# zgchen33/MCGaze

Hardware: AMD Instinct MI355X
Metric: clips/sec (7x3x224x224) (higher is better)
Workload: dtype f16x3; 1 GPU; full multiclue_gaze_r50 forward (R-50 + FPN + 4 decoder stages + gaze head), 64 clips/GPU x 7 frames x 3x224x224, 64 clips/step; clips_per_gpu=64, clip_length=7, global_clips=64, chunk_frames=0, parallelism=single GPU, trunk_streams=2

## Files before the change

include/mcgaze_hip.h:

```cpp
#ifndef MCGAZE_HIP_H
#define MCGAZE_HIP_H

#include <stddef.h>
#include <stdint.h>

#ifdef __cplusplus
extern "C" {
#endif

#define MCG_ABI_VERSION 19

enum { MCG_OK = 0, MCG_ERR_ARG = 1, MCG_ERR_HIP = 2, MCG_ERR_UNSUPPORTED = 3, MCG_ERR_WORKSPACE = 4 };
typedef enum { MCG_F32 = 0, MCG_BF16 = 1, MCG_F16X3 = 2, MCG_F16 = 3 } mcg_dtype;
#define MCG_ELEM_BYTES(dt) (((dt) == MCG_BF16 || (dt) == MCG_F16) ? 2 : 4)
typedef void* mcg_stream;

int mcg_abi_version(void);
const char* mcg_build_id(void);
const char* mcg_last_error(void);
int mcg_device_info(int* cu_count, size_t* hbm_bytes, char* arch, int arch_len);

int mcg_nchw_to_nhwc(mcg_stream s, mcg_dtype dt, const float* src, void* dst, int N, int C, int H, int W);
int mcg_nhwc_to_nchw(mcg_stream s, mcg_dtype dt, const void* src, float* dst, int N, int C, int H, int W);

enum { MCG_RES_NONE = 0, MCG_RES_ADD = 1, MCG_RES_UPSAMPLE_ADD = 2 };
enum {
  MCG_FLAG_STAGED_GEMM = 1,
  MCG_FLAG_NO_SPECIALISED = 2,
  MCG_FLAG_NO_ATTN_BLOCK = 4
};
typedef struct {
  const void* x;
  const void* w;
  const float* bias;
  const void* residual;
  void* y;
  int N, H, W, Cin, Cout, KH, KW, stride, pad;
  int relu;
  int residual_mode;
  int Hr, Wr;
  const void* x2;
  int Cin2, stride2, H2, W2;
  int tile;
  int flags;
  float wscale;
} mcg_conv_desc;
int mcg_conv2d(mcg_stream s, mcg_dtype dt, const mcg_conv_desc* d);

int mcg_bottleneck_x3(mcg_stream s, const float* x, const float* src2, const void* wstream, const float* bias, float* y, float* z,
                      int frames, int H, int W, int cm, int nsrc, int cn, void* trace);

size_t mcg_conv3x3_wino_x3_weight_bytes(int Cin, int Cout, int g);
int mcg_conv3x3_wino_x3(mcg_stream s, const float* x, const void* u, const float* bias, float* y, int frames, int H, int W,
                        int Cin, int Cout, int relu, int tile, float wscale, int g);

int mcg_pointwise_stream(mcg_stream s, mcg_dtype dt, const void* a, const void* wf, const float* bias, const void* res, void* y,
                         int M, int K, int N, int relu, int res_mode, int Ho, int Wo, int Hr, int Wr, float wscale,
                         const int* block_list, const int* block_count, int grid_cap);
int mcg_pointwise_dyn(mcg_stream s, mcg_dtype dt, const void* a, const void* wf, const float* bias, void* y, int M, float wscale, int grid_cap);
int mcg_pointwise_pair(mcg_stream s, mcg_dtype dt, const void* a1, const void* a2, const void* res, const void* w3f, const float* b3,
                       void* y, const void* w1f, const float* b1, void* z, int M, int K2, int C2, int grid_cap);

size_t mcg_stem_workspace_bytes(mcg_dtype dt, int N, int H, int W);
int mcg_stem_forward(mcg_stream s, mcg_dtype dt, const float* img, const void* w_stem, const float* bias,
                     void* y, int N, int H, int W, void* ws, size_t ws_bytes, int flags);

int mcg_roi_align(mcg_stream s, mcg_dtype dt, const void* const feats[4], const int feat_h[4], const int feat_w[4],
                  const int strides[4], int C, const float* boxes, int num_boxes, int boxes_per_frame,
                  void* out, int32_t* levels_out);
int mcg_roi_align_indexed(mcg_stream s, mcg_dtype dt, const void* const feats[4], const int feat_h[4], const int feat_w[4],
                          const int strides[4], int C, const float* boxes, int num_boxes, int boxes_per_frame,
                          const int32_t* frame_of, int pyramid_frames, void* out, int32_t* levels_out);

enum {
  MCG_SW_IN_PROJ_W = 0, MCG_SW_IN_PROJ_B, MCG_SW_OUT_PROJ_W, MCG_SW_OUT_PROJ_B, MCG_SW_ATTN_LN_G, MCG_SW_ATTN_LN_B,
  MCG_SW_DYN_W,
  MCG_SW_DYN_B,
  MCG_SW_NORM_IN_G, MCG_SW_NORM_IN_B, MCG_SW_NORM_OUT_G, MCG_SW_NORM_OUT_B,
  MCG_SW_FC_W, MCG_SW_FC_B, MCG_SW_FC_LN_G, MCG_SW_FC_LN_B, MCG_SW_IIC_LN_G, MCG_SW_IIC_LN_B,
  MCG_SW_FFN1_W, MCG_SW_FFN1_B, MCG_SW_FFN2_W, MCG_SW_FFN2_B, MCG_SW_FFN_LN_G, MCG_SW_FFN_LN_B,
  MCG_SW_CLS_FC_W, MCG_SW_CLS_LN_G, MCG_SW_CLS_LN_B,
  MCG_SW_REG_FC_W,
  MCG_SW_REG_LN_G,
  MCG_SW_REG_LN_B,
  MCG_SW_HEAD_CLS_W,
  MCG_SW_HEAD_CLS_B,
  MCG_SW_HEAD_REG_W,
  MCG_SW_HEAD_REG_B,
  MCG_SW_OUT_PROJ_WF, MCG_SW_CLS_FC_WF,
  MCG_SW_REG_FC_WF,
  MCG_SW_IN_PROJ_WF,
  MCG_SW_DYN_WF,
  MCG_SW_COUNT
};
enum {
  MCG_GW_FC_W = 0,
  MCG_GW_LN_G,
  MCG_GW_LN_B,
  MCG_GW_OUT_W,
  MCG_GW_OUT_B,
  MCG_GW_FUSE_W,
  MCG_GW_FUSE_B,
  MCG_GW_COUNT
};

size_t mcg_stage_workspace_bytes(mcg_dtype dt, int num_frames);
int mcg_stage_forward(mcg_stream s, mcg_dtype dt, const void* const weights[MCG_SW_COUNT], const void* roi_feat,
                      const void* obj_in, const float* boxes_in, int num_frames, int clip_length,
                      void* obj_out, float* boxes_out, float* cls_out, const float bbox_stds[4],
                      void* ws, size_t ws_bytes, int flags);
int mcg_stage_forward_ragged(mcg_stream s, mcg_dtype dt, const void* const weights[MCG_SW_COUNT], const void* roi_feat,
                             const void* obj_in, const float* boxes_in, int num_frames, const int* clip_start, int num_clips,
                             int max_clip_length, void* obj_out, float* boxes_out, float* cls_out, const float bbox_stds[4],
                             void* ws, size_t ws_bytes, int flags);

size_t mcg_gaze_head_workspace_bytes(mcg_dtype dt, int num_frames);
int mcg_gaze_head(mcg_stream s, mcg_dtype dt, const void* const weights[MCG_GW_COUNT], const void* obj,
                  int num_frames, float* gaze_out, void* ws, size_t ws_bytes);

typedef struct {
  const void* w;
  const float* bias;
  int cin, cout, k, stride, pad;
  const void* wf;
  float wscale;
  const void* wf4;
} mcg_conv_weights;

typedef struct {
  const void* wstream;
  const float* bias;
  int conv2_index;
  int cm, c, cn;
  int nsrc;
} mcg_fused_block;

typedef struct {
  int blocks[4];
  mcg_conv_weights stem;
  const mcg_conv_weights* convs;
  int num_convs;
  mcg_conv_weights lateral[4];
  mcg_conv_weights fpn_out[4];
  mcg_conv_weights c3_ds[4];
  const float* init_boxes;
  const void* init_feats;
  int num_stages;
  const void* const* stage_weights;
  const void* const* gaze_weights;
  float bbox_stds[4];
  const mcg_fused_block* fused;
  int num_fused;
} mcg_model_weights;

typedef struct mcg_engine mcg_engine;
int mcg_engine_create(mcg_engine** out, const mcg_model_weights* w, mcg_dtype dt);
void mcg_engine_destroy(mcg_engine* e);
int mcg_engine_set_option(mcg_engine* e, const char* name, int value);
int mcg_engine_range_audit(mcg_engine* e, unsigned long long* counts, const char** names, int capacity, int* n_out);
size_t mcg_engine_workspace_bytes(const mcg_engine* e, int num_frames, int H, int W, int chunk_frames);
int mcg_backbone_fpn_forward(mcg_engine* e, mcg_stream s, const float* img, int num_frames, int H, int W,
                             int chunk_frames, void* const pyramid[4], void* ws, size_t ws_bytes);
size_t mcg_trunk_workspace_bytes(const mcg_engine* e, int num_frames, int H, int W, int chunk_frames);
size_t mcg_decoder_workspace_bytes(const mcg_engine* e, int num_frames);
int mcg_decoder_forward(mcg_engine* e, mcg_stream s, const void* const pyramid[4], int num_frames, int clip_length, int H, int W,
                        const int* img_hw, float* gaze_out, float* boxes_out, float* scores_out, void* ws, size_t ws_bytes);
int mcg_decoder_forward_indexed(mcg_engine* e, mcg_stream s, const void* const pyramid[4], int pyramid_frames, const int32_t* frame_of,
                                int num_frames, int clip_length, int H, int W, const int* img_hw, float* gaze_out, float* boxes_out,
                                float* scores_out, void* ws, size_t ws_bytes);
int mcg_decoder_forward_ragged(mcg_engine* e, mcg_stream s, const void* const pyramid[4], int pyramid_frames, const int32_t* frame_of,
                               int num_frames, const int* clip_start, int num_clips, int max_clip_length, int H, int W, const int* img_hw,
                               float* gaze_out, float* boxes_out, float* scores_out, void* ws, size_t ws_bytes);
size_t mcg_deferred_pyramid_bytes(const mcg_engine* e, int num_frames, int H, int W);
int mcg_deferred_pyramid_levels(const mcg_engine* e, void* slot, int num_frames, int H, int W, void* levels[4], int* deferred);
int mcg_deferred_pyramid_state(const mcg_engine* e, void* slot, int num_frames, int H, int W, void** inner, int** flags, int** counts,
                               int** lists, int* blocks, int* lateral_deferred);
int mcg_inner_block_neighbours(int id, int H, int W, int out[9]);
int mcg_backbone_fpn_forward_deferred(mcg_engine* e, mcg_stream s, const float* img, int num_frames, int H, int W, int chunk_frames,
                                      void* slot, size_t slot_bytes, void* ws, size_t ws_bytes);
int mcg_decoder_forward_deferred(mcg_engine* e, mcg_stream s, void* slot, size_t slot_bytes, int num_frames, int clip_length, int H, int W,
                                 const int* img_hw, float* gaze_out, float* boxes_out, float* scores_out, void* ws, size_t ws_bytes);
int mcg_decoder_forward_deferred_ragged(mcg_engine* e, mcg_stream s, void* slot, size_t slot_bytes, int num_frames, const int* clip_start,
                                        int num_clips, int max_clip_length, int H, int W, const int* img_hw, float* gaze_out,
                                        float* boxes_out, float* scores_out, void* ws, size_t ws_bytes);
int mcg_clip_forward(mcg_engine* e, mcg_stream s, const float* img, int num_frames, int clip_length, int H, int W,
                     const int* img_hw, int chunk_frames, float* gaze_out, float* boxes_out, float* scores_out,
                     void* ws, size_t ws_bytes);
int mcg_clip_forward_ragged(mcg_engine* e, mcg_stream s, const float* img, int num_frames, const int* clip_start, int num_clips,
                            int max_clip_length, int H, int W, const int* img_hw, int chunk_frames, float* gaze_out, float* boxes_out,
                            float* scores_out, void* ws, size_t ws_bytes);
int mcg_pyramid_scatter_rows(mcg_stream s, mcg_dtype dt, const void* const src[4], void* const dst[4],
                             int num_frames, int store_rows, int H, int W, const int32_t* row_of);
int mcg_merge_windows(mcg_stream s, const float* gaze, const float* boxes, const float* scores, int num_frames, const float* scale,
                      int scale_per_frame, const int32_t* plan, int num_dst, int max_src, float* store, int store_rows,
                      float person_threshold);
int mcg_smooth_gaze(mcg_stream s, const float* store, int store_rows, const int32_t* plan, int num_out, double alpha, float* out);

typedef struct mcg_frame_desc {
  const void* src;
  int src_h, src_w, src_pitch;
  int crop_y, crop_x, crop_h, crop_w;
  int out_h, out_w;
} mcg_frame_desc;
int mcg_preprocess_frames(mcg_stream stream, const mcg_frame_desc* frames_dev, int num_frames, float* dst, int pad_h, int pad_w,
                          const float mean[3], const float stdinv[3], int to_rgb);
typedef struct mcg_image_desc {
  const void* src;
  int h, w, pitch;
} mcg_image_desc;
int mcg_preprocess_head_crops(mcg_stream s, const mcg_image_desc* images_dev, int num_images, const float* boxes_dev,
                              const int32_t* image_of_dev, int n, double expand, int scale_w, int scale_h, mcg_frame_desc* desc_out_dev,
                              int32_t* img_hw_dev, float* scale_factor_dev, int32_t* flags_dev, float* dst, int pad_h, int pad_w,
                              const float mean[3], const float stdinv[3], int to_rgb);
typedef struct mcg_yuv_coef {
  int y_off, cy, cub, cug, cvg, cvr;
} mcg_yuv_coef;
typedef struct mcg_nv12_image_desc {
  const void* y;
  const void* uv;
  int h, w, pitch_y, pitch_uv;
} mcg_nv12_image_desc;
typedef struct mcg_nv12_frame_desc {
  const void* src;
  int src_h, src_w, src_pitch;
  int crop_y, crop_x, crop_h, crop_w;
  int out_h, out_w;
  const void* uv;
  int uv_pitch;
} mcg_nv12_frame_desc;
int mcg_preprocess_frames_nv12(mcg_stream stream, const mcg_nv12_frame_desc* frames_dev, int num_frames, float* dst, int pad_h, int pad_w,
                               const float mean[3], const float stdinv[3], int to_rgb, const mcg_yuv_coef* coef);
int mcg_preprocess_head_crops_nv12(mcg_stream s, const mcg_nv12_image_desc* images_dev, int num_images, const float* boxes_dev,
                                   const int32_t* image_of_dev, int n, double expand, int scale_w, int scale_h,
                                   mcg_nv12_frame_desc* desc_out_dev, int32_t* img_hw_dev, float* scale_factor_dev, int32_t* flags_dev,
                                   float* dst, int pad_h, int pad_w, const float mean[3], const float stdinv[3], int to_rgb,
                                   const mcg_yuv_coef* coef);

typedef struct mcg_arrow_desc {
  int seg[3][2][2];
  int thickness;
  int x0, y0, x1, y1;
  int image, flag;
  int reserved;
} mcg_arrow_desc;
int mcg_draw_gaze_arrows(mcg_stream s, const mcg_image_desc* images_dev, int num_images, int max_h, int max_w, const float* boxes_dev,
                         const float* gaze_dev, int gaze_stride, const int32_t* image_of_dev, int n, double length, int min_thickness,
                         double thickness_ratio, double tip_length, const unsigned char* color, const unsigned char* colors_dev,
                         mcg_arrow_desc* plan_out_dev, int32_t* flags_dev);
int mcg_draw_gaze_arrows_nv12(mcg_stream s, const mcg_nv12_image_desc* images_dev, int num_images, int max_h, int max_w, const float* boxes_dev,
                              const float* gaze_dev, int gaze_stride, const int32_t* image_of_dev, int n, double length, int min_thickness,
                              double thickness_ratio, double tip_length, const unsigned char* yuv, const unsigned char* yuvs_dev,
                              mcg_arrow_desc* plan_out_dev, int32_t* flags_dev);

size_t mcg_detect_heads_workspace_bytes(int num_images, int num_anchors);
int mcg_detect_heads(mcg_stream s, const float* pred_dev, int num_images, int num_anchors, int num_classes, long long image_stride, int row_stride,
                     int in_h, int in_w, const int32_t* frame_hw_dev , double conf_thres, double iou_thres,
                     int only_class , int agnostic, int max_nms, int max_det,
                     float* boxes_dev , float* scores_dev , int32_t* classes_dev ,
                     int32_t* image_of_dev , int32_t* counts_dev , int32_t* flags_dev ,
                     void* ws_dev, size_t ws_bytes);

enum { MCG_LETTERBOX_U8 = 0, MCG_LETTERBOX_F16 = 1, MCG_LETTERBOX_F32 = 2 };
typedef struct mcg_letterbox_desc {
  mcg_frame_desc frame;
  int top, left;
} mcg_letterbox_desc;
typedef struct mcg_nv12_letterbox_desc {
  mcg_nv12_frame_desc frame;
  int top, left;
} mcg_nv12_letterbox_desc;
int mcg_letterbox_frames(mcg_stream stream, const mcg_letterbox_desc* frames_dev, int num_frames, void* dst, int out_h, int out_w, int out_type,
                         int swap_rb);
int mcg_letterbox_frames_nv12(mcg_stream stream, const mcg_nv12_letterbox_desc* frames_dev, int num_frames, void* dst, int out_h, int out_w,
                              int out_type, int swap_rb, const mcg_yuv_coef* coef);

typedef struct mcg_track_header {
  int32_t next_id;
  int32_t frames_seen;
  int32_t reserved[2];
} mcg_track_header;
typedef struct mcg_track_slot {
  float box[4];
  int32_t id;
  int32_t age;
  int32_t reserved[2];
} mcg_track_slot;
size_t mcg_track_state_bytes(int num_sequences, int slots);
int mcg_track_heads(mcg_stream s, const float* boxes_dev, long long frame_stride, const int32_t* counts_dev, int num_sequences, int num_frames,
                    int max_det, int slots, double match_iou, int max_age, void* state_dev,
                    float* slot_boxes_dev , int32_t* image_of_dev , int32_t* track_id_dev ,
                    int32_t* age_dev , int32_t* det_of_dev , int32_t* flags_dev );

int mcg_track_heads_motion(mcg_stream s, const float* boxes_dev, long long frame_stride, const int32_t* counts_dev, int num_sequences,
                           int num_frames, int max_det, int slots, double match_iou, int max_age, double velocity_gain, double coast_decay,
                           void* state_dev, float* slot_boxes_dev , int32_t* image_of_dev ,
                           int32_t* track_id_dev , int32_t* age_dev , int32_t* det_of_dev ,
                           int32_t* flags_dev , float* state_boxes_dev );

int mcg_live_slots(mcg_stream s, const void* state_dev, int num_cameras, int slots, int tick, int ring_depth, float* crop_boxes_dev,
                   int32_t* image_of_dev, int32_t* ring_id_dev, float* ring_box_dev, int32_t* matched_dev);
int mcg_live_gate(mcg_stream s, const int32_t* ring_id_dev, const float* ring_box_dev, int ring_depth, int num_cameras, int slots, int tick,
                  const int32_t* table_dev, int num_entries, int first_out, int num_out, const float* fused_dev, const float* others_dev,
                  float* fused_smooth_dev, float* others_smooth_dev, int32_t* track_id_dev, int32_t* valid_dev, float* head_box_dev,
                  int32_t* image_of_dev, int32_t* smooth_valid_dev);

int mcg_live_lanes(mcg_stream s, const void* state_dev, int num_cameras, int slots, int lanes, int tick, int ring_depth,
                   int32_t* lane_state_dev, float* crop_boxes_dev, int32_t* image_of_dev, int32_t* ring_id_dev, float* ring_box_dev,
                   int32_t* ring_col_dev, int32_t* lane_of_dev, int32_t* matched_dev, int32_t* overflow_dev);
int mcg_live_gate_lanes(mcg_stream s, const int32_t* ring_id_dev, const float* ring_box_dev, const int32_t* ring_col_dev, int ring_depth,
                        int num_cameras, int slots, int lanes, int tick, const int32_t* table_dev, int num_entries, int first_out, int num_out,
                        const float* fused_dev, const float* others_dev, float* fused_smooth_dev, float* others_smooth_dev,
                        int32_t* track_id_dev, int32_t* valid_dev, int32_t* camera_dev, int32_t* slot_dev, float* head_box_dev,
                        int32_t* image_of_dev, int32_t* smooth_valid_dev);

int mcg_gaze_targets(mcg_stream s, const float* boxes_dev, const float* gaze_dev, int gaze_stride, const int32_t* image_of_dev, int n,
                     const float* regions_dev, const int32_t* region_image_dev, int m, int region_period, double expand, double camera_cos2,
                     int32_t* kind_dev, int32_t* target_dev, float* t_dev, float* hit_dev, int32_t* mutual_dev, int32_t* flags_dev);

int mcg_gaze_dwell(mcg_stream s, const int32_t* person_dev, const int32_t* tag_dev, const int32_t* kind_dev, const int32_t* ident_dev,
                   const int32_t* mutual_dev, int num_frames, int columns, int frame0, int enter, int exit_frames, int32_t* state_dev,
                   int32_t* region_frames_dev, int num_regions, int32_t* dwell_dev, int32_t* ended_dev, int32_t* events_dev, int max_events,
                   int32_t* num_events_dev);

#define MCG_ATTEND_POLY_VERTS 32
int mcg_gaze_targets_poly(mcg_stream s, const float* boxes_dev, const float* gaze_dev, int gaze_stride, const int32_t* image_of_dev, int n,
                          const float* region_xy_dev, int num_vertices, const int32_t* region_start_dev, const int32_t* region_image_dev, int m,
                          int region_period, double expand, double camera_cos2, int32_t* kind_dev, int32_t* target_dev, float* t_dev,
                          float* hit_dev, int32_t* mutual_dev, int32_t* flags_dev);

typedef struct mcg_stroke_desc {
  int seg[3][2][2];
  int thickness;
  int x0, y0, x1, y1;
  int image, flag;
  int layer, count;
  unsigned color, color_active;
  int reserved;
} mcg_stroke_desc;
int mcg_draw_attention(mcg_stream s, const mcg_image_desc* images_dev, int num_images, int max_h, int max_w, const float* boxes_dev,
                       const float* gaze_dev, int gaze_stride, const int32_t* image_of_dev, int n, const int32_t* kind_dev, const int32_t* target_dev,
                       const float* hit_dev, const int32_t* mutual_dev, const float* region_xy_dev, int num_vertices,
                       const int32_t* region_start_dev, const int32_t* region_image_dev, int m, int region_period, const unsigned char* palette,
                       double length, int min_thickness, double thickness_ratio, double tip_length, int line_thickness, int region_thickness,
                       void* workspace_dev, size_t workspace_bytes, int32_t* flags_dev, int32_t* region_flags_dev, int32_t* region_active_dev);
int mcg_draw_attention_nv12(mcg_stream s, const mcg_nv12_image_desc* images_dev, int num_images, int max_h, int max_w, const float* boxes_dev,
                            const float* gaze_dev, int gaze_stride, const int32_t* image_of_dev, int n, const int32_t* kind_dev,
                            const int32_t* target_dev, const float* hit_dev, const int32_t* mutual_dev, const float* region_xy_dev, int num_vertices,
                            const int32_t* region_start_dev, const int32_t* region_image_dev, int m, int region_period, const unsigned char* palette,
                            double length, int min_thickness, double thickness_ratio, double tip_length, int line_thickness, int region_thickness,
                            void* workspace_dev, size_t workspace_bytes, int32_t* flags_dev, int32_t* region_flags_dev, int32_t* region_active_dev);

#define MCG_LABEL_CHARS 24
typedef struct mcg_label_desc {
  int x, y;
  int x0, y0, x1, y1;
  int image, flag;
  int len;
  unsigned color;
  unsigned char text[MCG_LABEL_CHARS];
} mcg_label_desc;
int mcg_format_labels(mcg_stream s, const int32_t* id_dev, const int32_t* value_dev, int n, int num, int den, unsigned char* text_out_dev);
int mcg_draw_labels(mcg_stream s, const mcg_image_desc* images_dev, int num_images, int max_h, int max_w, const float* boxes_dev,
                    const int32_t* image_of_dev, const unsigned char* text_dev, const int32_t* place_dev, int n, const unsigned char* font_dev,
                    int scale, int advance, int pad, const unsigned char* color, const unsigned char* colors_dev, const unsigned char* background,
                    mcg_label_desc* plan_out_dev, int32_t* flags_dev);
int mcg_draw_labels_nv12(mcg_stream s, const mcg_nv12_image_desc* images_dev, int num_images, int max_h, int max_w, const float* boxes_dev,
                         const int32_t* image_of_dev, const unsigned char* text_dev, const int32_t* place_dev, int n, const unsigned char* font_dev,
                         int scale, int advance, int pad, const unsigned char* yuv, const unsigned char* yuvs_dev, const unsigned char* background,
                         mcg_label_desc* plan_out_dev, int32_t* flags_dev);

int mcg_gaze_heat_add(mcg_stream s, const float* hit_dev, const int32_t* kind_dev, const int32_t* image_of_dev, const int32_t* flags_dev,
                      const int32_t* mask_dev, int n, int32_t* heat_dev, int32_t* peak_dev, int C, int GH, int GW, int cell_shift, int radius,
                      int kinds, int period, int decay_shift, void* workspace_dev, size_t workspace_bytes);
int mcg_draw_heat(mcg_stream s, const mcg_image_desc* images_dev, int num_images, int max_h, int max_w, const int32_t* heat_dev,
                  const int32_t* full_dev, int C, int GH, int GW, int cell_shift, int period, const unsigned char* lut_dev, int min_level);
int mcg_draw_heat_nv12(mcg_stream s, const mcg_nv12_image_desc* images_dev, int num_images, int max_h, int max_w, const int32_t* heat_dev,
                       const int32_t* full_dev, int C, int GH, int GW, int cell_shift, int period, const unsigned char* lut_dev, int min_level);

typedef struct mcg_anon_desc {
  int image, flag;
  int x0, y0, x1, y1;
  int cx2, cy2;
  int W, H;
  int shift, shape;
} mcg_anon_desc;
int mcg_anonymize_heads(mcg_stream s, const mcg_image_desc* images_dev, int num_images, int max_h, int max_w, const float* boxes_dev,
                        const int32_t* image_of_dev, int n, double expand, int shape, int cell_shift, int blocks, int mode,
                        const unsigned char* color, mcg_anon_desc* plan_out_dev, int32_t* flags_dev);
int mcg_anonymize_heads_nv12(mcg_stream s, const mcg_nv12_image_desc* images_dev, int num_images, int max_h, int max_w, const float* boxes_dev,
                             const int32_t* image_of_dev, int n, double expand, int shape, int cell_shift, int blocks, int mode,
                             const unsigned char* yuv, mcg_anon_desc* plan_out_dev, int32_t* flags_dev);

int mcg_engine_profile_start(mcg_engine* e, int capacity);
int mcg_engine_profile_stop(mcg_engine* e, int* count, float* ms, double* flops, double* algo_bytes, int* cfg, int* shape_mnk, int capacity);
int mcg_bench_backbone_forward(mcg_engine* e, mcg_stream s, const float* img, int num_frames, int H, int W, void* ws, size_t ws_bytes);
int mcg_bench_backbone_levels(const mcg_engine* e, void* ws, int num_frames, int H, int W, void* levels[4]);

#ifdef __cplusplus
}
#endif
#endif
```

mcgaze_amd/csrc/check_resources.py:

```python
#!/usr/bin/env python3
import re
import sys

RULES = {
    'wino_x3w_kernel': dict(scratch=0, vgpr_spill=0, unit='engine'),
    'wino_x3w_blocks_kernel': dict(scratch=0, vgpr_spill=0, unit='engine'),
    'gaze_targets_kernel': dict(scratch=0, vgpr_spill=0, unit='attend'),
    'gaze_targets_poly_kernel': dict(scratch=0, vgpr_spill=0, unit='attend'),
    'gaze_mutual_kernel': dict(scratch=0, vgpr_spill=0, unit='attend'),
    'gaze_dwell_kernel': dict(scratch=0, vgpr_spill=0, unit='dwell'),
    'gaze_dwell_events_kernel': dict(scratch=0, vgpr_spill=0, unit='dwell'),
    'label_raster_kernel': dict(scratch=0, vgpr_spill=0, unit='labels'),
    'heat_render_kernel': dict(scratch=0, vgpr_spill=0, unit='heat'),
    'anonymize_render_kernel': dict(scratch=0, vgpr_spill=0, unit='anonymize'),
}


def parse(path):
    kernels, cur = [], None
    for line in open(path, errors='replace'):
        m = re.search(r'remark: (?:\s*)Function Name: (\S+)', line)
        if m:
            cur = dict(name=m.group(1))
            kernels.append(cur)
            continue
        m = re.search(r'remark:\s+([A-Za-z \[\]/]+): (\S+) \[-Rpass-analysis', line)
        if m and cur is not None:
            cur[m.group(1).strip()] = m.group(2)
    return kernels


def main():
    path = sys.argv[1]
    kernels = parse(path)
    other = [l.rstrip() for l in open(path, errors='replace') if 'Rpass-analysis=kernel-resource-usage' not in l and not re.match(r'\s+\d* *\|', l) and l.strip()
             and not l.startswith('In file included from') and not re.match(r'\d+ (warning|remark)s? generated', l.strip())]
    for l in other:
        print(l, file=sys.stderr)
    bad = []
    import os
    unit = os.path.basename(path).split('.')[0]
    for prefix, lim in RULES.items():
        if lim.get('unit') == unit and not any(prefix in k['name'] and 'VGPRs Spill' in k and 'ScratchSize [bytes/lane]' in k for k in kernels):
            bad.append(f'{prefix}: no resource remarks found in {path} (expected -Rpass-analysis=kernel-resource-usage output for it)')
    for k in kernels:
        for prefix, lim in RULES.items():
            if prefix in k['name']:
                scratch = int(k.get('ScratchSize [bytes/lane]', '0'))
                spill = int(k.get('VGPRs Spill', '0'))
                if scratch > lim['scratch'] or spill > lim['vgpr_spill']:
                    bad.append(f"{k['name']}: scratch {scratch} B/lane, {spill} spilled VGPRs (limits {lim['scratch']}, {lim['vgpr_spill']})")
    if '--table' in sys.argv:
        print('| kernel | VGPRs | AGPRs | SGPRs | scratch B/lane | VGPR spill | waves/SIMD |\n|---|---|---|---|---|---|---|')
        for k in kernels:
            print(f"| `{k['name']}` | {k.get('VGPRs')} | {k.get('AGPRs')} | {k.get('TotalSGPRs')} | {k.get('ScratchSize [bytes/lane]')} | {k.get('VGPRs Spill')} | {k.get('Occupancy [waves/SIMD]')} |")
    if bad:
        print('check_resources: kernels that must not spill (RULES):\n  ' + '\n  '.join(bad), file=sys.stderr)
        return 1
    return 0


if __name__ == '__main__':
    sys.exit(main())
```

mcgaze_amd/csrc/engine.hip:

```cpp
#include "igemm.hpp"
#include "pw_pair.hpp"
#include "pw_single.hpp"
#include "bneck_x3.hpp"
#include "pw_single_x3.hpp"
#include "wino_x3.hpp"

#include <stdarg.h>
#include <stdlib.h>
#include <string.h>

#include <map>
#include <mutex>
#include <string>
#include <vector>

int launch_roi_align(hipStream_t s, mcg_dtype dt, const void* const feats[4], const int feat_h[4], const int feat_w[4],
                     const int strides[4], int C, const float* boxes, int num_boxes, int boxes_per_frame, const int32_t* frame_of,
                     int pyramid_frames, void* out, int32_t* levels_out);
int launch_init_queries(hipStream_t s, mcg_dtype dt, const float* init_boxes, const void* init_feats, const int* img_hw,
                        const int32_t* frame_of, int pyramid_frames, int H, int W, float* boxes, void* obj, int N);
bool roi_mark_supported(int H, int W);
int launch_defer_clear(hipStream_t s, int* p, int n);
int launch_roi_mark(hipStream_t s, const float* boxes, int num_boxes, int boxes_per_frame, int level, int H, int W, int stride, int* state,
                    int* list, int* count);
int launch_inner_mark(hipStream_t s, const int* out_list, const int* out_count, int H, int W, int nblk, int* state, int* list, int* count);

struct mcg_engine {
  mcg_dtype dt;
  int blocks[4];
  mcg_conv_weights stem;
  std::vector<mcg_conv_weights> convs;
  mcg_conv_weights lateral[4], fpn_out[4], c3_ds[4];
  std::vector<mcg_fused_block> fused;
  bool bneck_fused = true;
  bool bneck_blocked = true;
  int winograd = 1;
  int wino_tile = -1;
  int fpn_deferred = 1;
  int fpn_lateral_deferred = 1;
  static constexpr int kAuditCap = 256;
  unsigned long long* audit_dev = nullptr;
  std::vector<std::string> audit_names;
  const float* init_boxes;
  const void* init_feats;
  int num_stages;
  std::vector<const void*> stage_w;
  const void* gaze_w[MCG_GW_COUNT];
  float stds[4];
  static constexpr int kMaxSplit = 4, kCandidates = 8;
  struct StreamPool* pool = nullptr;
  hipStream_t* cand = nullptr;
  hipEvent_t ev_fork = nullptr, ev_join[kMaxSplit - 1] = {};
  McgCtx ctx;
  Prof prof;
  int trunk_streams = 2;
  int max_range_frames = 0;
  bool pw_single = true;
  bool pw_pair = true;
  std::mutex mu;
};
struct StreamPool {
  hipStream_t cand[mcg_engine::kCandidates] = {};
  hipEvent_t ev_probe[3] = {};
  std::map<hipStream_t, std::vector<int>> side_of;
  std::mutex mu;
  bool ok = false;
};
static StreamPool* stream_pool_for_current_device() {
  static std::mutex g_mu;
  static std::map<int, StreamPool*> g_pools;
  int dev = 0;
  if (hipGetDevice(&dev) != hipSuccess) return nullptr;
  std::lock_guard<std::mutex> lock(g_mu);
  auto it = g_pools.find(dev);
  if (it != g_pools.end()) return it->second;
  StreamPool* p = new StreamPool();
  bool ok = true;
  for (int i = 0; i < mcg_engine::kCandidates; ++i) ok = ok && hipStreamCreateWithFlags(&p->cand[i], hipStreamNonBlocking) == hipSuccess;
  for (int i = 0; i < 3; ++i) ok = ok && hipEventCreate(&p->ev_probe[i]) == hipSuccess;
  p->ok = ok;
  g_pools[dev] = p;
  return p;
}
__global__ void probe_spin_kernel(long long ticks) {
  const long long t0 = wall_clock64();
  while (wall_clock64() - t0 < ticks) {}
}
static const std::vector<int>& side_streams_for(mcg_engine* e, hipStream_t s) {
  StreamPool* p = e->pool;
  std::lock_guard<std::mutex> lock(p->mu);
  auto it = p->side_of.find(s);
  if (it != p->side_of.end()) return it->second;
  std::vector<int> good, rest;
  const long long ticks = 15000;
  for (int c = 0; c < mcg_engine::kCandidates; ++c) {
    bool concurrent = false;
    if (hipEventRecord(p->ev_probe[0], s) == hipSuccess) {
      hipLaunchKernelGGL(probe_spin_kernel, dim3(1), dim3(64), 0, s, ticks);
      hipLaunchKernelGGL(probe_spin_kernel, dim3(1), dim3(64), 0, p->cand[c], ticks);
      float ms = 0.f;
      if (hipEventRecord(p->ev_probe[1], s) == hipSuccess && hipEventRecord(p->ev_probe[2], p->cand[c]) == hipSuccess &&
          hipEventSynchronize(p->ev_probe[1]) == hipSuccess && hipEventSynchronize(p->ev_probe[2]) == hipSuccess &&
          hipEventElapsedTime(&ms, p->ev_probe[0], p->ev_probe[2]) == hipSuccess)
        concurrent = ms < 0.15f * 1.6f;
    }
    (concurrent ? good : rest).push_back(c);
  }
  (void)hipGetLastError();
  good.insert(good.end(), rest.begin(), rest.end());
  return p->side_of.emplace(s, good).first->second;
}
static int range_frame_cap(const mcg_engine* e, int H, int W) {
  const long long per_frame = (long long)(H / 4) * (W / 4) * 256 * (mcg_is16(e->dt) ? 2 : 4);
  long long cap = 0x7FFFFF00ll / (per_frame > 0 ? per_frame : 1);
  if (e->max_range_frames > 0 && e->max_range_frames < cap) cap = e->max_range_frames;
  return cap < 1 ? 1 : (cap > 0x7fffffff ? 0x7fffffff : (int)cap);
}
static const int kMinFramesPerRange = 56;
static int trunk_ranges(const mcg_engine* e, int frames) {
  int k = e->trunk_streams;
  if (k > mcg_engine::kMaxSplit) k = mcg_engine::kMaxSplit;
  while (k > 1 && frames / k < kMinFramesPerRange) --k;
  return k < 1 ? 1 : k;
}

static inline size_t al256(size_t b) { return (b + 255) / 256 * 256; }
static inline size_t esize(mcg_dtype dt) { return mcg_is16(dt) ? 2 : 4; }

extern "C" void mcg_engine_destroy(mcg_engine* e);
extern "C" int mcg_engine_create(mcg_engine** out, const mcg_model_weights* w, mcg_dtype dt) {
  MCG_CHECK_ARG(out && w, "mcg_engine_create: null pointer");
  MCG_CHECK_ARG(dt == MCG_F32 || dt == MCG_BF16 || dt == MCG_F16X3 || dt == MCG_F16, "mcg_engine_create: unknown dtype %d", (int)dt);
  int expect = 0;
  for (int l = 0; l < 4; ++l) {
    MCG_CHECK_ARG(w->blocks[l] > 0, "mcg_engine_create: blocks[%d]=%d", l, w->blocks[l]);
    expect += 3 * w->blocks[l] + 1;
  }
  MCG_CHECK_ARG(w->num_convs == expect && w->convs, "mcg_engine_create: expected %d bottleneck convs, got %d", expect, w->num_convs);
  MCG_CHECK_ARG(w->num_stages > 0 && w->stage_weights && w->gaze_weights && w->init_boxes && w->init_feats, "mcg_engine_create: decoder tables missing");
  for (int i = 0; i < w->num_convs; ++i)
    MCG_CHECK_ARG(w->convs[i].w && w->convs[i].bias, "mcg_engine_create: conv %d has a null pointer", i);
  mcg_engine* e = new mcg_engine();
  e->dt = dt;
  memcpy(e->blocks, w->blocks, sizeof(e->blocks));
  e->stem = w->stem;
  e->convs.assign(w->convs, w->convs + w->num_convs);
  memcpy(e->lateral, w->lateral, sizeof(e->lateral));
  memcpy(e->fpn_out, w->fpn_out, sizeof(e->fpn_out));
  memcpy(e->c3_ds, w->c3_ds, sizeof(e->c3_ds));
  if (w->fused && w->num_fused > 0 && dt == MCG_F16X3) e->fused.assign(w->fused, w->fused + w->num_fused);
  e->init_boxes = w->init_boxes;
  e->init_feats = w->init_feats;
  e->num_stages = w->num_stages;
  e->stage_w.assign(w->stage_weights, w->stage_weights + (size_t)w->num_stages * MCG_SW_COUNT);
  memcpy(e->gaze_w, w->gaze_weights, sizeof(e->gaze_w));
  memcpy(e->stds, w->bbox_stds, sizeof(e->stds));
  bool ok = hipEventCreateWithFlags(&e->ev_fork, hipEventDisableTiming) == hipSuccess;
  e->pool = stream_pool_for_current_device();
  ok = ok && e->pool && e->pool->ok;
  if (e->pool) e->cand = e->pool->cand;
  for (int i = 0; i < mcg_engine::kMaxSplit - 1; ++i) ok = ok && hipEventCreateWithFlags(&e->ev_join[i], hipEventDisableTiming) == hipSuccess;
  if (!ok) {
    mcg_engine_destroy(e);
    mcg_set_error("mcg_engine_create: could not create the side streams / events");
    return MCG_ERR_HIP;
  }
  *out = e;
  return MCG_OK;
}

extern "C" int mcg_engine_set_option(mcg_engine* e, const char* name, int value) {
  MCG_CHECK_ARG(e && name, "mcg_engine_set_option: null pointer");
  std::lock_guard<std::mutex> lock(e->mu);
  if (!strcmp(name, "trunk_streams")) { MCG_CHECK_ARG(value >= 1 && value <= mcg_engine::kMaxSplit, "trunk_streams must be 1..%d", mcg_engine::kMaxSplit); e->trunk_streams = value; }
  else if (!strcmp(name, "max_range_frames")) { MCG_CHECK_ARG(value >= 0, "max_range_frames must be >= 0"); e->max_range_frames = value; }
  else if (!strcmp(name, "tile")) e->ctx.tile = value > 0 ? value : -1;
  else if (!strcmp(name, "staged_gemm")) e->ctx.staged = value != 0;
  else if (!strcmp(name, "conv3x3_c64")) e->ctx.c64 = value != 0;
  else if (!strcmp(name, "stem_fused")) e->ctx.stem_fused = value != 0;
  else if (!strcmp(name, "decoder_chain")) e->ctx.chain = value != 0;
  else if (!strcmp(name, "decoder_attn_block")) e->ctx.attn_block = value != 0;
  else if (!strcmp(name, "pointwise_pair")) e->pw_pair = value != 0;
  else if (!strcmp(name, "pointwise_stream")) e->pw_single = value != 0;
  else if (!strcmp(name, "bottleneck_fused")) e->bneck_fused = value != 0;
  else if (!strcmp(name, "bottleneck_blocked")) e->bneck_blocked = value != 0;
  else if (!strcmp(name, "winograd")) { MCG_CHECK_ARG(value >= 0 && value <= 2, "winograd must be 0, 1 or 2"); e->winograd = value; }
  else if (!strcmp(name, "fpn_deferred")) e->fpn_deferred = value != 0;
  else if (!strcmp(name, "fpn_lateral_deferred")) e->fpn_lateral_deferred = value != 0;
  else if (!strcmp(name, "wino_tile")) { MCG_CHECK_ARG(value >= -1 && value <= 3, "wino_tile must be -1 (by grid size) .. 3"); e->wino_tile = value; }
  else if (!strcmp(name, "range_audit")) {
    MCG_CHECK_ARG(!mcg_is16(e->dt) || !value, "range_audit: f32-storage engines only (MCG_F32, MCG_F16X3)");
    if (value && !e->audit_dev) {
      if (hipMalloc((void**)&e->audit_dev, sizeof(unsigned long long) * 2 * mcg_engine::kAuditCap) != hipSuccess) { e->audit_dev = nullptr; mcg_set_error("range_audit: hipMalloc failed"); return MCG_ERR_HIP; }
    }
    if (value && hipMemset(e->audit_dev, 0, sizeof(unsigned long long) * 2 * mcg_engine::kAuditCap) != hipSuccess) { mcg_set_error("range_audit: hipMemset failed"); return MCG_ERR_HIP; }
    if (!value && e->audit_dev) { (void)hipFree(e->audit_dev); e->audit_dev = nullptr; }
    e->audit_names.clear();
  }
  else { mcg_set_error("mcg_engine_set_option: unknown option '%s'", name); return MCG_ERR_ARG; }
  return MCG_OK;
}

extern "C" int mcg_engine_profile_start(mcg_engine* e, int capacity) {
  MCG_CHECK_ARG(e, "mcg_engine_profile_start: null engine");
  std::lock_guard<std::mutex> lock(e->mu);
  if (e->prof.recs) { mcg_set_error("mcg_engine_profile_start: already armed"); return MCG_ERR_ARG; }
  MCG_CHECK_ARG(capacity > 0 && capacity <= (1 << 20), "mcg_engine_profile_start: bad capacity %d", capacity);
  e->prof.recs = new ProfRec[capacity];
  for (int i = 0; i < capacity; ++i) { e->prof.recs[i].a = nullptr; e->prof.recs[i].b = nullptr; }
  for (int i = 0; i < capacity; ++i) {
    if (hipEventCreate(&e->prof.recs[i].a) != hipSuccess || hipEventCreate(&e->prof.recs[i].b) != hipSuccess) {
      for (int j = 0; j <= i; ++j) {
        if (e->prof.recs[j].a) (void)hipEventDestroy(e->prof.recs[j].a);
        if (e->prof.recs[j].b) (void)hipEventDestroy(e->prof.recs[j].b);
      }
      delete[] e->prof.recs;
      e->prof = Prof();
      mcg_set_error("mcg_engine_profile_start: hipEventCreate failed");
      return MCG_ERR_HIP;
    }
  }
  e->prof.cap = capacity; e->prof.n = 0;
  e->ctx.prof = &e->prof;
  return MCG_OK;
}
extern "C" int mcg_engine_profile_stop(mcg_engine* e, int* count, float* ms, double* flops, double* bytes, int* cfg, int* shape, int capacity) {
  MCG_CHECK_ARG(e, "mcg_engine_profile_stop: null engine");
  std::lock_guard<std::mutex> lock(e->mu);
  if (!e->prof.recs) { mcg_set_error("mcg_engine_profile_stop: not armed"); return MCG_ERR_ARG; }
  const int n = e->prof.n;
  int rc = MCG_OK;
  for (int i = 0; i < n; ++i) {
    const ProfRec& r = e->prof.recs[i];
    float t = 0.f;
    if (hipEventSynchronize(r.b) != hipSuccess || hipEventElapsedTime(&t, r.a, r.b) != hipSuccess) rc = MCG_ERR_HIP;
    if (i < capacity) {
      if (ms) ms[i] = t;
      if (flops) flops[i] = r.flops;
      if (bytes) bytes[i] = r.bytes;
      if (cfg) cfg[i] = r.cfg;
      if (shape) { shape[3 * i] = r.shape[0]; shape[3 * i + 1] = r.shape[1]; shape[3 * i + 2] = r.shape[2]; }
    }
  }
  for (int i = 0; i < e->prof.cap; ++i) { (void)hipEventDestroy(e->prof.recs[i].a); (void)hipEventDestroy(e->prof.recs[i].b); }
  delete[] e->prof.recs;
  e->prof = Prof();
  e->ctx.prof = nullptr;
  if (count) *count = n < capacity ? n : capacity;
  if (rc != MCG_OK) mcg_set_error("mcg_engine_profile_stop: event query failed");
  return rc;
}
extern "C" void mcg_engine_destroy(mcg_engine* e) {
  if (!e) return;
  if (e->ev_fork) (void)hipEventDestroy(e->ev_fork);
  for (int i = 0; i < mcg_engine::kMaxSplit - 1; ++i)
    if (e->ev_join[i]) (void)hipEventDestroy(e->ev_join[i]);
  if (e->prof.recs) {
    for (int i = 0; i < e->prof.cap; ++i) { (void)hipEventDestroy(e->prof.recs[i].a); (void)hipEventDestroy(e->prof.recs[i].b); }
    delete[] e->prof.recs;
  }
  if (e->audit_dev) (void)hipFree(e->audit_dev);
  delete e;
}

__global__ void range_audit_kernel(const float* __restrict__ x, long long n, unsigned long long* __restrict__ cnt) {
  unsigned long long big = 0, bad = 0;
  for (long long i = (long long)blockIdx.x * blockDim.x + threadIdx.x; i < n; i += (long long)gridDim.x * blockDim.x) {
    const float v = x[i];
    if (!(fabsf(v) <= 3.4028235e38f)) ++bad;
    else if (fabsf(v) > 65504.f) ++big;
  }
  big = (unsigned long long)wave_sum((float)big) ;
  bad = (unsigned long long)wave_sum((float)bad);
  if ((threadIdx.x & 63) == 0) {
    if (big) atomicAdd(cnt, big);
    if (bad) atomicAdd(cnt + 1, bad);
  }
}
struct AuditCursor { mcg_engine* e; hipStream_t s; int idx; bool naming; };
__attribute__((format(printf, 4, 5))) static void audit_tensor(AuditCursor& a, const void* p, long long elements, const char* fmt, ...) {
  if (!a.e->audit_dev || a.idx >= mcg_engine::kAuditCap) return;
  if (a.naming) {
    char name[64];
    va_list ap;
    va_start(ap, fmt);
    vsnprintf(name, sizeof(name), fmt, ap);
    va_end(ap);
    a.e->audit_names.push_back(name);
  }
  const long long per_thread = 16;
  long long blocks = (elements + 256 * per_thread - 1) / (256 * per_thread);
  if (blocks > 4096) blocks = 4096;
  if (blocks < 1) blocks = 1;
  hipLaunchKernelGGL(range_audit_kernel, dim3((int)blocks), dim3(256), 0, a.s, (const float*)p, elements, a.e->audit_dev + 2 * a.idx);
  ++a.idx;
}

struct TrunkWs {
  char *stem_ws, *x0, *xa, *xb, *o1, *o2, *ds, *c[4], *l[4];
  size_t stem_bytes, big, total;
};
static TrunkWs trunk_layout(mcg_dtype dt, int n, int H, int W, char* base) {
  const size_t es = esize(dt);
  const size_t h2 = H / 4, w2 = W / 4;
  TrunkWs t;
  size_t off = 0;
  auto take = [&](size_t bytes) { char* p = base ? base + off : nullptr; off += al256(bytes); return p; };
  t.stem_bytes = mcg_stem_workspace_bytes(dt, n, H, W);
  t.stem_ws = take(t.stem_bytes);
  t.big = (size_t)n * h2 * w2 * 256 * es;
  t.x0 = take((size_t)n * h2 * w2 * 64 * es);
  t.xa = take(t.big); t.xb = take(t.big);
  t.o1 = take(t.big / 2); t.o2 = take(t.big / 2);
  t.ds = take(t.big);
  for (int i = 0; i < 4; ++i) {
    const size_t hi = (H / 4) >> i, wi = (W / 4) >> i;
    t.c[i] = take((size_t)n * hi * wi * (256u << i) * es);
    t.l[i] = take((size_t)n * hi * wi * 256 * es);
  }
  t.total = off;
  return t;
}

static int wino_kind(const mcg_engine* e, mcg_dtype dt, const mcg_conv_weights& cw, int n, int h, int w, int rm) {
  return (dt == MCG_F16X3 && e->winograd && e->ctx.tile < 0 && cw.k == 3 && cw.stride == 1 && cw.pad == 1 && rm == MCG_RES_NONE)
             ? ((cw.wf4 && e->winograd >= 2 && wino_x3_applicable(n, h, w, cw.cin, cw.cout, 4)) ? 4 : ((cw.wf && wino_x3_applicable(n, h, w, cw.cin, cw.cout, 2)) ? 2 : 0))
             : 0;
}
static WinoParams wino_params(const mcg_conv_weights& cw, int g, const void* x, int n, int h, int w, void* y, int relu) {
  WinoParams wp;
  memset(&wp, 0, sizeof(wp));
  wp.x = (const float*)x; wp.u = g == 4 ? cw.wf4 : cw.wf; wp.bias = cw.bias; wp.y = (float*)y;
  wp.H = h; wp.W = w; wp.frames = n; wp.Cin = cw.cin; wp.Cout = cw.cout; wp.relu = relu; wp.wscale = cw.wscale;
  return wp;
}
static ProfRec* prof_begin_wino(const McgCtx& ctx, hipStream_t s, const mcg_conv_weights& cw, long long M, bool book = true) {
  return prof_begin(ctx, s, 73, (int)M, cw.cout, 9 * cw.cin, book ? 2.0 * M * 9.0 * cw.cin * cw.cout : 0.0,
                    book ? 4.0 * ((double)M * (cw.cin + cw.cout) + 9.0 * cw.cin * cw.cout) : 0.0);
}
static int launch_done(ProfRec* rec, hipStream_t s, int rc, const char* what) {
  prof_end(rec, s);
  if (rc) { mcg_set_error("%s launch failed", what); return MCG_ERR_HIP; }
  return MCG_OK;
}
static mcg_conv_desc conv_desc(mcg_dtype dt, const mcg_conv_weights& cw, const void* x, int n, int h, int w, void* y, int relu,
                               const void* res, int res_mode, int hr, int wr) {
  mcg_conv_desc d;
  memset(&d, 0, sizeof(d));
  d.x = x; d.w = cw.w; d.bias = cw.bias; d.residual = res; d.y = y;
  d.N = n; d.H = h; d.W = w; d.Cin = cw.cin; d.Cout = cw.cout; d.KH = cw.k; d.KW = cw.k; d.stride = cw.stride; d.pad = cw.pad;
  d.relu = relu; d.residual_mode = res_mode; d.Hr = hr; d.Wr = wr;
  d.wscale = dt == MCG_F16X3 ? cw.wscale : 0.f;
  return d;
}
static int conv_call(const mcg_engine* e, hipStream_t s, mcg_dtype dt, const mcg_conv_weights& cw, const void* x, int n, int h, int w, void* y,
                     int relu, const void* res, int res_mode, int hr, int wr) {
  const long long M = (long long)n * h * w;
  const int rm = res ? res_mode : MCG_RES_NONE;
  const long long res_m = rm == MCG_RES_UPSAMPLE_ADD ? (long long)n * hr * wr : M;
  const bool x3 = dt == MCG_F16X3;
  if ((x3 || mcg_is16(dt)) && e->pw_single && e->ctx.tile < 0 && cw.wf && cw.bias && cw.k == 1 && cw.stride == 1 && cw.pad == 0 && M < 0x7fffffffll &&
      (x3 ? pw_single_x3_applicable(cw.cin, cw.cout, rm, M, res_m) : !e->ctx.staged && pw_single_applicable(cw.cin, cw.cout, rm, M, res_m))) {
    PwSingleParams pp;
    memset(&pp, 0, sizeof(pp));
    pp.a = x; pp.res = res; pp.wf = cw.wf; pp.bias = cw.bias; pp.y = y;
    pp.M = (int)M; pp.relu = relu; pp.Ho = h; pp.Wo = w; pp.wscale = x3 ? cw.wscale : 0.f;
    if (rm == MCG_RES_UPSAMPLE_ADD) { pp.Hr = hr; pp.Wr = wr; pp.rscale_h = (float)hr / (float)h; pp.rscale_w = (float)wr / (float)w; }
    ProfRec* rec = prof_begin(e->ctx, s, x3 ? 71 : 61, pp.M, cw.cout, cw.cin, 2.0 * M * cw.cin * cw.cout,
                              (double)esize(dt) * ((double)M * (cw.cin + cw.cout) + (rm == MCG_RES_NONE ? 0.0 : (double)res_m) * cw.cout + (double)cw.cin * cw.cout));
    const int rmode = rm == MCG_RES_NONE ? 0 : (rm == MCG_RES_ADD ? 1 : 2);
    return launch_done(rec, s, x3 ? launch_pw_single_x3(s, pp, cw.cout, rmode) : launch_pw_single(s, pp, cw.cin, cw.cout, rmode, dt),
                       x3 ? "pw_single_x3" : "pw_single");
  }
  const int wg = wino_kind(e, dt, cw, n, h, w, rm);
  if (wg) {
    ProfRec* rec = prof_begin_wino(e->ctx, s, cw, M);
    return launch_done(rec, s, launch_wino_x3(s, wino_params(cw, wg, x, n, h, w, y, relu), e->wino_tile, wg), "wino_x3");
  }
  const mcg_conv_desc d = conv_desc(dt, cw, x, n, h, w, y, relu, res, res_mode, hr, wr);
  return conv2d_ctx(s, dt, &d, e->ctx);
}

struct TrunkCursor {
  const void* x;
  int h, w, ci;
  char *o1, *o2;
  bool o1_ready;
  bool x_blocked;
};
static const mcg_fused_block* fused_tail_at(const mcg_engine* e, int ci, int b) {
  if (!(e->dt == MCG_F16X3 && e->bneck_fused && e->ctx.tile < 0) || ci + 2 >= (int)e->convs.size()) return nullptr;
  const mcg_fused_block* f = nullptr;
  for (const mcg_fused_block& q : e->fused)
    if (q.conv2_index == ci + 1) f = &q;
  if (!f) return nullptr;
  const bool ds = b == 0;
  const mcg_conv_weights &d2 = e->convs[ci + 1], &d3 = e->convs[ci + 2];
  const int kk = ds ? e->convs[ci + 3].cin : 0, ss = ds ? e->convs[ci + 3].stride : 1;
  const int cn_i = ci + (ds ? 4 : 3);
  const bool nx = f->cn == 0 || (cn_i < (int)e->convs.size() && e->convs[cn_i].k == 1 && e->convs[cn_i].stride == 1 && e->convs[cn_i].cout == f->cn && e->convs[cn_i].cin == f->c);
  return (d2.k == 3 && d2.stride == 1 && d2.pad == 1 && d2.cin == f->cm && d2.cout == f->cm && d3.cout == f->c && f->nsrc == (ds ? 2 : 1) && nx &&
          bneck_x3_applicable(f->cm, f->c, f->cn, f->nsrc, kk, ss)) ? f : nullptr;
}
static int fused_tail_step(const mcg_engine* e, hipStream_t s, const TrunkWs& t, AuditCursor& au, TrunkCursor& c, const mcg_fused_block* fb,
                           int n, int l, int b, void* y) {
  const bool has_ds = b == 0;
  const int k2 = has_ds ? e->convs[c.ci + 3].cin : 0;
  BneckParams bp;
  memset(&bp, 0, sizeof(bp));
  bp.x = (const float*)c.o1; bp.res = (const float*)c.x; bp.wstream = (const char*)fb->wstream; bp.bias = fb->bias;
  bp.y = (float*)y; bp.z = (float*)c.o2; bp.H = c.h; bp.W = c.w;
  const long long blk_bytes = (long long)n * ((c.h + bnx::TH - 1) / bnx::TH) * ((c.w + bnx::TW - 1) / bnx::TW) * bnx::NPIX * fb->c * (long long)esize(e->dt);
  const mcg_fused_block* fnext = (b + 1 < e->blocks[l]) ? fused_tail_at(e, c.ci + (has_ds ? 4 : 3), b + 1) : nullptr;
  bp.res_blocked = c.x_blocked ? 1 : 0;
  bp.y_blocked = (e->bneck_blocked && !e->audit_dev && y != (void*)t.c[l] && fb->cn > 0 && fnext && fnext->nsrc == 1 && fnext->c == fb->c &&
                  blk_bytes <= (long long)t.big) ? 1 : 0;
  const double M = (double)n * c.h * c.w;
  ProfRec* rec = prof_begin(e->ctx, s, 70, n * c.h * c.w, fb->c + fb->cn, 9 * fb->cm + fb->cm + k2 + fb->c,
                            2.0 * M * (9.0 * fb->cm * fb->cm + (double)(fb->cm + k2) * fb->c + (double)fb->c * fb->cn),
                            4.0 * (M * (fb->cm + (has_ds ? k2 : fb->c) + fb->c + fb->cn) + 9.0 * fb->cm * fb->cm + (double)(fb->cm + k2) * fb->c + (double)fb->c * fb->cn));
  MCG_TRY(launch_done(rec, s, launch_bneck_x3(s, bp, n, fb->cm, fb->nsrc, fb->cn), "bneck_x3"));
  audit_tensor(au, y, (long long)n * c.h * c.w * fb->c, "layer%d.%d.out (fused tail)", l + 1, b);
  if (fb->cn > 0) {
    audit_tensor(au, c.o2, (long long)n * c.h * c.w * fb->cn, "layer%d.%d.next_conv1 (fused tail)", l + 1, b);
    std::swap(c.o1, c.o2);
    c.o1_ready = true;
  }
  c.x_blocked = bp.y_blocked != 0;
  return MCG_OK;
}
static const mcg_conv_weights* pw_pair_next(const mcg_engine* e, int ci, int l, int b, long long M) {
  const bool has_ds = b == 0;
  const mcg_conv_weights& c3 = e->convs[ci + 2];
  const mcg_conv_weights* c3w = has_ds ? (e->c3_ds[l].w ? &e->c3_ds[l] : nullptr) : &c3;
  const int ci_next = ci + (has_ds ? 4 : 3);
  const mcg_conv_weights* c1n = ci_next < (int)e->convs.size() ? &e->convs[ci_next] : nullptr;
  const int k2 = has_ds ? e->convs[ci + 3].cin : 0;
  return (mcg_is16(e->dt) && e->pw_pair && l == 0 && c3w && c1n && c3w->wf && c1n->wf && c3w->bias && c1n->bias && c1n->k == 1 && c1n->stride == 1 &&
          c1n->cin == c3.cout && pw_pair_applicable(c3.cin, k2, has_ds ? e->convs[ci + 3].stride : 1, c3.cout, c1n->cout, M) && M < 0x7fffffffll)
             ? c1n : nullptr;
}
static int pw_pair_step(const mcg_engine* e, hipStream_t s, TrunkCursor& c, const mcg_conv_weights& c1n, int n, int l, int b, void* y, int ho, int wo) {
  const bool has_ds = b == 0;
  const mcg_conv_weights& c3 = e->convs[c.ci + 2];
  const mcg_conv_weights& c3w = has_ds ? e->c3_ds[l] : c3;
  PwPairParams pp;
  memset(&pp, 0, sizeof(pp));
  pp.a1 = c.o2; pp.K1 = c3.cin;
  if (has_ds) { pp.a2 = c.x; pp.K2 = e->convs[c.ci + 3].cin; pp.stride2 = e->convs[c.ci + 3].stride; pp.H2 = c.h; pp.W2 = c.w; }
  else pp.res = c.x;
  pp.w3f = c3w.wf; pp.b3 = c3w.bias; pp.y = y;
  pp.w1f = c1n.wf; pp.b1 = c1n.bias; pp.z = c.o1;
  pp.M = n * ho * wo; pp.C = c3.cout; pp.C2 = c1n.cout; pp.Ho = ho; pp.Wo = wo;
  ProfRec* rec = prof_begin(e->ctx, s, 60, pp.M, pp.C + pp.C2, pp.K1 + pp.K2, 2.0 * pp.M * ((double)(pp.K1 + pp.K2) * pp.C + (double)pp.C * pp.C2),
                            2.0 * ((double)pp.M * (pp.K1 + pp.K2 + (has_ds ? 0 : pp.C) + pp.C + pp.C2) + (double)(pp.K1 + pp.K2) * pp.C + (double)pp.C * pp.C2));
  MCG_TRY(launch_done(rec, s, launch_pw_pair(s, pp, e->dt), "pw_pair"));
  c.o1_ready = true;
  return MCG_OK;
}
static int conv3_step(const mcg_engine* e, hipStream_t s, const TrunkWs& t, AuditCursor& au, const TrunkCursor& c, int n, int l, int b, void* y,
                      int ho, int wo) {
  const mcg_conv_weights& c3 = e->convs[c.ci + 2];
  if (b == 0 && e->c3_ds[l].w) {
    const mcg_conv_weights& ds = e->convs[c.ci + 3];
    mcg_conv_desc d = conv_desc(e->dt, e->c3_ds[l], c.o2, n, ho, wo, y, 1, nullptr, MCG_RES_NONE, 0, 0);
    d.Cin = c3.cin;
    d.x2 = c.x; d.Cin2 = ds.cin; d.stride2 = ds.stride; d.H2 = c.h; d.W2 = c.w;
    MCG_TRY(conv2d_ctx(s, e->dt, &d, e->ctx));
  } else {
    const void* identity = c.x;
    if (b == 0) {
      MCG_TRY(conv_call(e, s, e->dt, e->convs[c.ci + 3], c.x, n, c.h, c.w, t.ds, 0, nullptr, MCG_RES_NONE, 0, 0));
      identity = t.ds;
    }
    MCG_TRY(conv_call(e, s, e->dt, c3, c.o2, n, ho, wo, y, 1, identity, MCG_RES_ADD, 0, 0));
  }
  audit_tensor(au, y, (long long)n * ho * wo * c3.cout, "layer%d.%d.out", l + 1, b);
  return MCG_OK;
}

struct TrunkKeep { char *inner, *c2, *l1; };
static int trunk_chunk(mcg_engine* e, hipStream_t s, const float* img, int f0, int n, int H, int W, void* const pyr[4], char* wsbase,
                       bool backbone_only = false, const TrunkKeep tk = TrunkKeep{nullptr, nullptr, nullptr}) {
  const mcg_dtype dt = e->dt;
  const size_t es = esize(dt);
  TrunkWs t = trunk_layout(dt, n, H, W, wsbase);
  char* const inner0 = tk.inner;
  if (inner0) t.l[0] = inner0 + (size_t)f0 * (H / 4) * (W / 4) * 256 * es;
  const bool lateral_deferred = inner0 && tk.c2 && tk.l1;
  if (lateral_deferred) {
    t.c[0] = tk.c2 + (size_t)f0 * (H / 4) * (W / 4) * 256 * es;
    t.l[1] = tk.l1 + (size_t)f0 * (H / 8) * (W / 8) * 256 * es;
  }
  MCG_TRY(stem_forward_ctx(s, dt, img + (size_t)f0 * 3 * H * W, e->stem.w, e->stem.bias, t.x0, n, H, W, t.stem_ws, t.stem_bytes, e->ctx));
  AuditCursor au{e, s, 0, e->audit_dev != nullptr && e->audit_names.empty()};
  audit_tensor(au, t.x0, (long long)n * (H / 4) * (W / 4) * 64, "stem");
  TrunkCursor c{t.x0, H / 4, W / 4, 0, t.o1, t.o2, false, false};
  for (int l = 0; l < 4; ++l) {
    for (int b = 0; b < e->blocks[l]; ++b) {
      const mcg_conv_weights &c1 = e->convs[c.ci], &c2 = e->convs[c.ci + 1];
      const int ho = (c.h + 2 * c2.pad - c2.k) / c2.stride + 1, wo = (c.w + 2 * c2.pad - c2.k) / c2.stride + 1;
      void* y = (b == e->blocks[l] - 1) ? (void*)t.c[l] : (c.x == t.xa ? (void*)t.xb : (void*)t.xa);
      if (!c.o1_ready) {
        MCG_TRY(conv_call(e, s, dt, c1, c.x, n, c.h, c.w, c.o1, 1, nullptr, MCG_RES_NONE, 0, 0));
        audit_tensor(au, c.o1, (long long)n * c.h * c.w * c1.cout, "layer%d.%d.conv1", l + 1, b);
      }
      c.o1_ready = false;
      const mcg_fused_block* fb = fused_tail_at(e, c.ci, b);
      if (c.x_blocked && !(fb && fb->nsrc == 1)) { mcg_set_error("trunk: a blocked tensor reached a kernel that does not read that layout"); return MCG_ERR_UNSUPPORTED; }
      if (fb) {
        MCG_TRY(fused_tail_step(e, s, t, au, c, fb, n, l, b, y));
      } else {
        MCG_TRY(conv_call(e, s, dt, c2, c.o1, n, c.h, c.w, c.o2, 1, nullptr, MCG_RES_NONE, 0, 0));
        audit_tensor(au, c.o2, (long long)n * ho * wo * c2.cout, "layer%d.%d.conv2", l + 1, b);
        const mcg_conv_weights* c1n = pw_pair_next(e, c.ci, l, b, (long long)n * ho * wo);
        MCG_TRY(c1n ? pw_pair_step(e, s, c, *c1n, n, l, b, y, ho, wo) : conv3_step(e, s, t, au, c, n, l, b, y, ho, wo));
      }
      c.x = y; c.h = ho; c.w = wo;
      c.ci += b == 0 ? 4 : 3;
    }
  }
  if (backbone_only) return MCG_OK;
  int hs[4], wsz[4];
  for (int i = 0; i < 4; ++i) { hs[i] = (H / 4) >> i; wsz[i] = (W / 4) >> i; }
  for (int i = 3; i >= (lateral_deferred ? 1 : 0); --i) {
    const void* res = i == 3 ? nullptr : t.l[i + 1];
    MCG_TRY(conv_call(e, s, dt, e->lateral[i], t.c[i], n, hs[i], wsz[i], t.l[i], 0, res, res ? MCG_RES_UPSAMPLE_ADD : MCG_RES_NONE,
                      i == 3 ? 0 : hs[i + 1], i == 3 ? 0 : wsz[i + 1]));
    audit_tensor(au, t.l[i], (long long)n * hs[i] * wsz[i] * 256, "fpn.lateral%d (+ top-down)", i);
  }
  for (int i = inner0 ? 1 : 0; i < 4; ++i) {
    char* dst = (char*)pyr[i] + (size_t)f0 * hs[i] * wsz[i] * 256 * es;
    MCG_TRY(conv_call(e, s, dt, e->fpn_out[i], t.l[i], n, hs[i], wsz[i], dst, 0, nullptr, MCG_RES_NONE, 0, 0));
    audit_tensor(au, dst, (long long)n * hs[i] * wsz[i] * 256, "fpn.P%d", i + 2);
  }
  return MCG_OK;
}

extern "C" int mcg_engine_range_audit(mcg_engine* e, unsigned long long* counts, const char** names, int capacity, int* n_out) {
  MCG_CHECK_ARG(e && counts && n_out && capacity > 0, "mcg_engine_range_audit: bad argument");
  std::lock_guard<std::mutex> lock(e->mu);
  if (!e->audit_dev) { mcg_set_error("mcg_engine_range_audit: the range_audit option is off"); return MCG_ERR_ARG; }
  const int n = (int)e->audit_names.size() < capacity ? (int)e->audit_names.size() : capacity;
  if (hipDeviceSynchronize() != hipSuccess ||
      hipMemcpy(counts, e->audit_dev, sizeof(unsigned long long) * 2 * n, hipMemcpyDeviceToHost) != hipSuccess ||
      hipMemset(e->audit_dev, 0, sizeof(unsigned long long) * 2 * mcg_engine::kAuditCap) != hipSuccess) {
    mcg_set_error("mcg_engine_range_audit: device read failed");
    return MCG_ERR_HIP;
  }
  if (names) for (int i = 0; i < n; ++i) names[i] = e->audit_names[i].c_str();
  *n_out = n;
  return MCG_OK;
}

struct DecWs {
  char *roi, *obj_a, *obj_b, *stage_ws, *gaze_ws;
  float *boxes_a, *boxes_b, *cls;
  size_t stage_bytes, gaze_bytes, total;
};
static DecWs dec_layout(mcg_dtype dt, int N, char* base) {
  const size_t es = esize(dt), R = (size_t)N * 3;
  DecWs c;
  memset(&c, 0, sizeof(c));
  size_t off = 0;
  auto take = [&](size_t bytes) { char* p = base ? base + off : nullptr; off += al256(bytes); return p; };
  c.roi = take(R * 49 * 256 * es);
  c.obj_a = take(R * 256 * es); c.obj_b = take(R * 256 * es);
  c.boxes_a = (float*)take(R * 4 * 4); c.boxes_b = (float*)take(R * 4 * 4); c.cls = (float*)take(R * 4);
  c.stage_bytes = mcg_stage_workspace_bytes(dt, N); c.stage_ws = take(c.stage_bytes);
  c.gaze_bytes = mcg_gaze_head_workspace_bytes(dt, N); c.gaze_ws = take(c.gaze_bytes);
  c.total = off;
  return c;
}
static bool check_shape_ok(int N, int H, int W) { return N > 0 && H >= 32 && W >= 32 && H % 32 == 0 && W % 32 == 0; }
static size_t pyramid_bytes(mcg_dtype dt, int N, int H, int W, int level) {
  return al256((size_t)N * ((H / 4) >> level) * ((W / 4) >> level) * 256 * esize(dt));
}

struct DeferSlot {
  void* p[4];
  char* inner;
  int *state, *count, *list;
  int nblk;
  bool deferred;
  bool lateral;
  char *c2, *l1;
  int *istate, *icount, *ilist;
  size_t total;
};
static bool fpn_deferred_on(const mcg_engine* e, int N, int H, int W) {
  const mcg_conv_weights& cw = e->fpn_out[0];
  const int h = H / 4, w = W / 4;
  return e->fpn_deferred && e->dt == MCG_F16X3 && !e->audit_dev && e->num_stages > 0 && wino_kind(e, e->dt, cw, N, h, w, MCG_RES_NONE) == 2 &&
         wino_x3_blocks_applicable(N, h, w, cw.cin, cw.cout) && roi_mark_supported(h, w);
}
static bool fpn_lateral_deferred_on(const mcg_engine* e, int N, int H, int W) {
  const mcg_conv_weights& cw = e->lateral[0];
  const int h = H / 4, w = W / 4;
  return e->fpn_lateral_deferred && fpn_deferred_on(e, N, H, W) && e->pw_single && e->ctx.tile < 0 && cw.wf && cw.bias && cw.k == 1 && cw.stride == 1 &&
         cw.pad == 0 && h % 2 == 0 && w % 2 == 0 &&
         pw_single_x3_blocks_applicable(cw.cin, cw.cout, h, w, (long long)N * h * w, (long long)N * (h / 2) * (w / 2));
}
static DeferSlot defer_layout(const mcg_engine* e, int N, int H, int W, char* base) {
  DeferSlot d;
  memset(&d, 0, sizeof(d));
  size_t off = 0;
  auto take = [&](size_t bytes) { char* p = base ? base + off : nullptr; off += al256(bytes); return p; };
  for (int i = 0; i < 4; ++i) d.p[i] = take(pyramid_bytes(e->dt, N, H, W, i));
  d.deferred = fpn_deferred_on(e, N, H, W);
  if (d.deferred) {
    d.inner = take((size_t)N * (H / 4) * (W / 4) * 256 * esize(e->dt));
    d.nblk = N * wino_x3_blocks_per_frame(H / 4, W / 4);
    d.lateral = fpn_lateral_deferred_on(e, N, H, W);
    const size_t per = (size_t)d.nblk + e->num_stages;
    d.state = (int*)take(sizeof(int) * per * (d.lateral ? 2 : 1));
    d.count = d.state ? d.state + d.nblk : nullptr;
    d.list = (int*)take(sizeof(int) * (size_t)d.nblk * e->num_stages);
    if (d.lateral) {
      d.istate = d.state ? d.state + per : nullptr;
      d.icount = d.istate ? d.istate + d.nblk : nullptr;
      d.ilist = (int*)take(sizeof(int) * (size_t)d.nblk * e->num_stages);
      d.c2 = take((size_t)N * (H / 4) * (W / 4) * 256 * esize(e->dt));
      d.l1 = take((size_t)N * (H / 8) * (W / 8) * 256 * esize(e->dt));
    }
  }
  d.total = off;
  return d;
}

extern "C" size_t mcg_trunk_workspace_bytes(const mcg_engine* e, int N, int H, int W, int chunk) {
  if (!e || N <= 0) return 0;
  if (chunk <= 0 || chunk > N) chunk = N;
  if (chunk < N) return trunk_layout(e->dt, chunk, H, W, nullptr).total;
  size_t total = 0;
  const int cap = range_frame_cap(e, H, W);
  for (int k = 1; k <= mcg_engine::kMaxSplit; ++k) {
    const int per = (N + k - 1) / k < cap ? (N + k - 1) / k : cap;
    const size_t t = (size_t)k * al256(trunk_layout(e->dt, per, H, W, nullptr).total);
    if (t > total) total = t;
  }
  return total;
}
extern "C" size_t mcg_decoder_workspace_bytes(const mcg_engine* e, int N) {
  if (!e || N <= 0) return 0;
  return dec_layout(e->dt, N, nullptr).total;
}
extern "C" size_t mcg_engine_workspace_bytes(const mcg_engine* e, int N, int H, int W, int chunk) {
  if (!e || N <= 0) return 0;
  return mcg_trunk_workspace_bytes(e, N, H, W, chunk) + mcg_decoder_workspace_bytes(e, N) + defer_layout(e, N, H, W, nullptr).total;
}
extern "C" size_t mcg_deferred_pyramid_bytes(const mcg_engine* e, int N, int H, int W) {
  if (!e || N <= 0 || check_shape_ok(N, H, W) == false) return 0;
  return defer_layout(e, N, H, W, nullptr).total;
}

static int check_shape(int N, int H, int W) {
  MCG_CHECK_ARG(N > 0, "num_frames must be positive (got %d)", N);
  MCG_CHECK_ARG(H >= 32 && W >= 32 && H % 32 == 0 && W % 32 == 0, "frame size %dx%d must be a multiple of 32 (Pad(size_divisor=32))", H, W);
  return MCG_OK;
}

static int trunk_forward(mcg_engine* e, mcg_stream s_, const float* img, int N, int H, int W, int chunk,
                         void* const pyramid[4], void* ws, size_t ws_bytes, bool backbone_only, const TrunkKeep tk = TrunkKeep{nullptr, nullptr, nullptr}) {
  MCG_CHECK_ARG(e && img && (pyramid || backbone_only) && ws, "mcg_backbone_fpn_forward: null pointer");
  MCG_TRY(check_shape(N, H, W));
  std::lock_guard<std::mutex> lock(e->mu);
  if (chunk <= 0 || chunk > N) chunk = N;
  const size_t need = mcg_trunk_workspace_bytes(e, N, H, W, chunk);
  if (ws_bytes < need) { mcg_set_error("mcg_backbone_fpn_forward: workspace too small (%zu < %zu)", ws_bytes, need); return MCG_ERR_WORKSPACE; }
  const int k = chunk < N ? 1 : trunk_ranges(e, N), cap = range_frame_cap(e, H, W);
  const int per = chunk < N ? chunk : ((N + k - 1) / k < cap ? (N + k - 1) / k : cap);
  const hipStream_t s = (hipStream_t)s_;
  hipStream_t si[mcg_engine::kMaxSplit] = {s};
  if (k > 1) {
    const std::vector<int>& sides = side_streams_for(e, s);
    for (int i = 1; i < k; ++i) si[i] = e->cand[sides[i - 1]];
    if (hipEventRecord(e->ev_fork, s) != hipSuccess) { mcg_set_error("mcg_backbone_fpn_forward: hipEventRecord failed"); return MCG_ERR_HIP; }
    for (int i = 1; i < k; ++i)
      if (hipStreamWaitEvent(si[i], e->ev_fork, 0) != hipSuccess) { mcg_set_error("mcg_backbone_fpn_forward: hipStreamWaitEvent failed"); return MCG_ERR_HIP; }
  }
  const size_t part_ws = k > 1 ? al256(trunk_layout(e->dt, per, H, W, nullptr).total) : 0;
  int rc = MCG_OK;
  for (int f0 = 0, i = 0; f0 < N && rc == MCG_OK; f0 += per, i = (i + 1) % k)
    rc = trunk_chunk(e, si[i], img, f0, (N - f0) < per ? (N - f0) : per, H, W, pyramid, (char*)ws + (size_t)i * part_ws, backbone_only, tk);
  for (int i = 1; i < k; ++i) {
    if (hipEventRecord(e->ev_join[i - 1], si[i]) != hipSuccess || hipStreamWaitEvent(s, e->ev_join[i - 1], 0) != hipSuccess) {
      mcg_set_error("mcg_backbone_fpn_forward: join failed");
      rc = rc == MCG_OK ? MCG_ERR_HIP : rc;
    }
  }
  return rc;
}

extern "C" int mcg_bottleneck_x3(mcg_stream s, const float* x, const float* src2, const void* wstream, const float* bias, float* y, float* z,
                                 int frames, int H, int W, int cm, int nsrc, int cn, void* trace) {
  MCG_CHECK_ARG(x && src2 && wstream && bias && y && (z || cn == 0), "mcg_bottleneck_x3: null pointer");
  MCG_CHECK_ARG(frames > 0 && H > 0 && W > 0, "mcg_bottleneck_x3: empty problem");
  MCG_CHECK_ARG(bneck_x3_applicable(cm, 4 * cm, cn, nsrc, 64, 1), "mcg_bottleneck_x3: unsupported shape (cm=%d nsrc=%d cn=%d)", cm, nsrc, cn);
  BneckParams bp;
  memset(&bp, 0, sizeof(bp));
  bp.x = x; bp.res = src2; bp.wstream = (const char*)wstream; bp.bias = bias; bp.y = y; bp.z = z; bp.H = H; bp.W = W; bp.trace = (unsigned long long*)trace;
  if (launch_bneck_x3((hipStream_t)s, bp, frames, cm, nsrc, cn)) { mcg_set_error("mcg_bottleneck_x3: launch failed"); return MCG_ERR_HIP; }
  return MCG_OK;
}

extern "C" size_t mcg_conv3x3_wino_x3_weight_bytes(int Cin, int Cout, int g) {
  return (Cin > 0 && Cout > 0 && Cin % 32 == 0 && Cout % wnx::UNT == 0 && (g == 2 || g == 4)) ? wino_x3_weight_bytes(Cin, Cout, g) : 0;
}
extern "C" int mcg_conv3x3_wino_x3(mcg_stream s, const float* x, const void* u, const float* bias, float* y, int frames, int H, int W,
                                   int Cin, int Cout, int relu, int tile, float wscale, int g) {
  MCG_CHECK_ARG(x && u && y, "mcg_conv3x3_wino_x3: null pointer");
  MCG_CHECK_ARG(tile >= 0 && tile <= 4, "mcg_conv3x3_wino_x3: tile must be 0 (by grid size) .. 4");
  if (!wino_x3_applicable(frames, H, W, Cin, Cout, g)) {
    mcg_set_error("mcg_conv3x3_wino_x3: unsupported shape (frames=%d %dx%d, %d -> %d channels, F(%d,3)): Cin %% 32, Cout %% 128, W <= 62 (F(4,3): W %% 4 == 0, W >= 16), a tile's window within its buffer", frames, H, W, Cin, Cout, g);
    return MCG_ERR_UNSUPPORTED;
  }
  WinoParams wp;
  memset(&wp, 0, sizeof(wp));
  wp.x = x; wp.u = u; wp.bias = bias; wp.y = y; wp.H = H; wp.W = W; wp.frames = frames; wp.Cin = Cin; wp.Cout = Cout; wp.relu = relu;
  wp.wscale = wscale;
  if (launch_wino_x3((hipStream_t)s, wp, tile - 1, g)) { mcg_set_error("mcg_conv3x3_wino_x3: launch failed"); return MCG_ERR_HIP; }
  return MCG_OK;
}

extern "C" int mcg_pointwise_stream(mcg_stream s, mcg_dtype dt, const void* a, const void* wf, const float* bias, const void* res, void* y,
                                    int M, int K, int N, int relu, int res_mode, int Ho, int Wo, int Hr, int Wr, float wscale,
                                    const int* block_list, const int* block_count, int grid_cap) {
  MCG_CHECK_ARG(a && wf && bias && y, "mcg_pointwise_stream: null pointer");
  MCG_CHECK_ARG(M > 0 && grid_cap >= 0, "mcg_pointwise_stream: M must be positive and grid_cap >= 0 (M=%d grid_cap=%d)", M, grid_cap);
  MCG_CHECK_ARG(res_mode >= MCG_RES_NONE && res_mode <= MCG_RES_UPSAMPLE_ADD && (res != nullptr) == (res_mode != MCG_RES_NONE),
                "mcg_pointwise_stream: res_mode %d needs %s residual", res_mode, res_mode == MCG_RES_NONE ? "no" : "a");
  MCG_CHECK_ARG((block_list != nullptr) == (block_count != nullptr), "mcg_pointwise_stream: block_list and block_count come together");
  const bool x3 = dt == MCG_F16X3, up = res_mode == MCG_RES_UPSAMPLE_ADD;
  if (up) MCG_CHECK_ARG(Ho > 0 && Wo > 0 && Hr > 0 && Wr > 0 && M % ((long long)Ho * Wo) == 0,
                        "mcg_pointwise_stream: upsample residual: M = frames * Ho * Wo (M=%d, %dx%d from %dx%d)", M, Ho, Wo, Hr, Wr);
  const long long res_rows = up ? M / ((long long)Ho * Wo) * Hr * Wr : M;
  bool ok = x3 ? pw_single_x3_dispatched(K, N, M, res_rows) : mcg_is16(dt) && pw_single_dispatched(K, N, res_mode, M, res_rows);
  if (block_list) ok = x3 && up && pw_single_x3_blocks_applicable(K, N, Ho, Wo, M, res_rows);
  if (!ok) {
    mcg_set_error("mcg_pointwise_stream: unsupported (dtype %d, %d -> %d channels, res_mode %d, M=%d%s): see include/mcgaze_hip.h for the table", (int)dt, K, N,
                  res_mode, M, block_list ? ", block list" : "");
    return MCG_ERR_UNSUPPORTED;
  }
  PwSingleParams pp;
  memset(&pp, 0, sizeof(pp));
  pp.a = a; pp.res = res; pp.wf = wf; pp.bias = bias; pp.y = y;
  pp.M = M; pp.relu = relu; pp.Ho = up ? Ho : 1; pp.Wo = up ? Wo : 1; pp.wscale = x3 ? wscale : 0.f;
  if (up) { pp.Hr = Hr; pp.Wr = Wr; pp.rscale_h = (float)Hr / (float)Ho; pp.rscale_w = (float)Wr / (float)Wo; }
  const int rc = block_list ? launch_pw_single_x3_blocks((hipStream_t)s, pp, block_list, block_count, M / 64, grid_cap)
                 : x3       ? launch_pw_single_x3((hipStream_t)s, pp, N, res_mode, grid_cap)
                            : launch_pw_single((hipStream_t)s, pp, K, N, res_mode, dt, grid_cap);
  if (rc) { mcg_set_error("mcg_pointwise_stream: launch failed"); return MCG_ERR_HIP; }
  return MCG_OK;
}

extern "C" int mcg_pointwise_pair(mcg_stream s, mcg_dtype dt, const void* a1, const void* a2, const void* res, const void* w3f, const float* b3,
                                  void* y, const void* w1f, const float* b1, void* z, int M, int K2, int C2, int grid_cap) {
  MCG_CHECK_ARG(a1 && w3f && b3 && y && w1f && b1 && z, "mcg_pointwise_pair: null pointer");
  MCG_CHECK_ARG(M > 0 && grid_cap >= 0, "mcg_pointwise_pair: M must be positive and grid_cap >= 0 (M=%d grid_cap=%d)", M, grid_cap);
  MCG_CHECK_ARG((a2 != nullptr) == (K2 != 0), "mcg_pointwise_pair: a second source comes with K2 = 64, none with K2 = 0");
  if (!mcg_is16(dt) || !pw_pair_applicable(64, K2, 1, 256, C2, M) || (K2 != 0 && res)) {
    mcg_set_error("mcg_pointwise_pair: unsupported (dtype %d, K2=%d, C2=%d, M=%d%s): bf16 / fp16, K2 0 or 64, C2 64 or 128, a residual only without a second source",
                  (int)dt, K2, C2, M, res ? ", residual" : "");
    return MCG_ERR_UNSUPPORTED;
  }
  PwPairParams pp;
  memset(&pp, 0, sizeof(pp));
  pp.a1 = a1; pp.K1 = 64; pp.a2 = a2; pp.K2 = K2; pp.stride2 = 1; pp.res = res;
  pp.w3f = w3f; pp.b3 = b3; pp.y = y; pp.w1f = w1f; pp.b1 = b1; pp.z = z;
  pp.M = M; pp.C = 256; pp.C2 = C2; pp.Ho = 1; pp.Wo = M; pp.H2 = 1; pp.W2 = M;
  if (launch_pw_pair((hipStream_t)s, pp, dt, grid_cap)) { mcg_set_error("mcg_pointwise_pair: launch failed"); return MCG_ERR_HIP; }
  return MCG_OK;
}

extern "C" int mcg_backbone_fpn_forward(mcg_engine* e, mcg_stream s, const float* img, int N, int H, int W, int chunk,
                                        void* const pyramid[4], void* ws, size_t ws_bytes) {
  return trunk_forward(e, s, img, N, H, W, chunk, pyramid, ws, ws_bytes, false);
}
extern "C" int mcg_bench_backbone_forward(mcg_engine* e, mcg_stream s, const float* img, int N, int H, int W, void* ws, size_t ws_bytes) {
  return trunk_forward(e, s, img, N, H, W, 0, nullptr, ws, ws_bytes, true);
}

extern "C" int mcg_bench_backbone_levels(const mcg_engine* e, void* ws, int N, int H, int W, void* levels[4]) {
  MCG_CHECK_ARG(e && ws && levels, "mcg_bench_backbone_levels: null pointer");
  MCG_TRY(check_shape(N, H, W));
  MCG_CHECK_ARG(trunk_ranges(e, N) == 1 && N <= range_frame_cap(e, H, W), "mcg_bench_backbone_levels: the batch runs as several frame ranges (set trunk_streams = 1)");
  const TrunkWs t = trunk_layout(e->dt, N, H, W, (char*)ws);
  for (int i = 0; i < 4; ++i) levels[i] = t.c[i];
  return MCG_OK;
}

static int defer_stage_forward(const mcg_engine* e, hipStream_t s, const DeferSlot& d, int st, const float* boxes, int N, int h, int w) {
  const mcg_conv_weights& cw = e->fpn_out[0];
  int* list = d.list + (size_t)st * d.nblk;
  MCG_TRY(launch_roi_mark(s, boxes, N * 3, 3, 0, h, w, 4, d.state, list, d.count + st));
  if (d.lateral) {
    const mcg_conv_weights& lw = e->lateral[0];
    int* ilist = d.ilist + (size_t)st * d.nblk;
    MCG_TRY(launch_inner_mark(s, list, d.count + st, h, w, d.nblk, d.istate, ilist, d.icount + st));
    const long long M = (long long)N * h * w, res_m = (long long)N * (h / 2) * (w / 2);
    PwSingleParams pp;
    memset(&pp, 0, sizeof(pp));
    pp.a = d.c2; pp.res = d.l1; pp.wf = lw.wf; pp.bias = lw.bias; pp.y = d.inner;
    pp.M = (int)M; pp.relu = 0; pp.Ho = h; pp.Wo = w; pp.wscale = lw.wscale;
    pp.Hr = h / 2; pp.Wr = w / 2; pp.rscale_h = (float)pp.Hr / (float)h; pp.rscale_w = (float)pp.Wr / (float)w;
    const bool book = st == 0;
    ProfRec* lrec = prof_begin(e->ctx, s, 71, pp.M, lw.cout, lw.cin, book ? 2.0 * M * lw.cin * lw.cout : 0.0,
                               book ? 4.0 * ((double)M * (lw.cin + lw.cout) + (double)res_m * lw.cout + (double)lw.cin * lw.cout) : 0.0);
    MCG_TRY(launch_done(lrec, s, launch_pw_single_x3_blocks(s, pp, ilist, d.icount + st, d.nblk), "pw_single_x3 block"));
  }
  ProfRec* rec = prof_begin_wino(e->ctx, s, cw, (long long)N * h * w, st == 0);
  return launch_done(rec, s, launch_wino_x3_blocks(s, wino_params(cw, 2, d.inner, N, h, w, d.p[0], 0), list, d.count + st, d.nblk), "wino_x3 block");
}

static int decoder_forward(mcg_engine* e, hipStream_t s, const void* const pyramid[4], int pyramid_frames, const int32_t* frame_of, int N,
                           const ClipTable& ct, int H, int W, const int* img_hw, float* gaze_out, float* boxes_out, float* scores_out, void* ws,
                           size_t ws_bytes, const DeferSlot* d = nullptr) {
  MCG_CHECK_ARG(e && pyramid && gaze_out && boxes_out && scores_out && ws, "mcg_decoder_forward: null pointer");
  MCG_TRY(check_shape(N, H, W));
  MCG_TRY(check_clips("mcg_decoder_forward", N, ct));
  DecWs c = dec_layout(e->dt, N, (char*)ws);
  if (ws_bytes < c.total) { mcg_set_error("mcg_decoder_forward: workspace too small (%zu < %zu)", ws_bytes, c.total); return MCG_ERR_WORKSPACE; }
  MCG_TRY(launch_init_queries(s, e->dt, e->init_boxes, e->init_feats, img_hw, frame_of, pyramid_frames, H, W, c.boxes_a, c.obj_a, N));
  int fh[4], fw[4];
  const int strides[4] = {4, 8, 16, 32};
  for (int i = 0; i < 4; ++i) { fh[i] = (H / 4) >> i; fw[i] = (W / 4) >> i; }
  char* obj_in = c.obj_a; char* obj_out = c.obj_b;
  float* b_in = c.boxes_a; float* b_out = c.boxes_b;
  const bool defer = d && d->deferred;
  if (defer) MCG_TRY(launch_defer_clear(s, d->state, (d->nblk + e->num_stages) * (d->lateral ? 2 : 1)));
  for (int st = 0; st < e->num_stages; ++st) {
    if (defer) MCG_TRY(defer_stage_forward(e, s, *d, st, b_in, N, fh[0], fw[0]));
    MCG_TRY(launch_roi_align(s, e->dt, pyramid, fh, fw, strides, 256, b_in, N * 3, 3, frame_of, pyramid_frames, c.roi, nullptr));
    float* bdst = (st == e->num_stages - 1) ? boxes_out : b_out;
    MCG_TRY(stage_forward_ctx(s, e->dt, &e->stage_w[(size_t)st * MCG_SW_COUNT], c.roi, obj_in, b_in, N, ct, obj_out, bdst,
                              c.cls, e->stds, c.stage_ws, c.stage_bytes, e->ctx));
    char* t = obj_in; obj_in = obj_out; obj_out = t;
    if (st != e->num_stages - 1) { float* tb = b_in; b_in = b_out; b_out = tb; }
  }
  MCG_TRY(gaze_head_ctx(s, e->dt, e->gaze_w, obj_in, N, gaze_out, c.gaze_ws, c.gaze_bytes, e->ctx, c.cls, scores_out));
  return MCG_OK;
}

extern "C" int mcg_decoder_forward(mcg_engine* e, mcg_stream s_, const void* const pyramid[4], int N, int clip_length, int H, int W,
                                   const int* img_hw, float* gaze_out, float* boxes_out, float* scores_out, void* ws, size_t ws_bytes) {
  return decoder_forward(e, (hipStream_t)s_, pyramid, N, nullptr, N, ClipTable::uniform(N, clip_length), H, W, img_hw, gaze_out, boxes_out, scores_out, ws,
                         ws_bytes);
}

extern "C" int mcg_decoder_forward_indexed(mcg_engine* e, mcg_stream s_, const void* const pyramid[4], int pyramid_frames, const int32_t* frame_of,
                                           int N, int clip_length, int H, int W, const int* img_hw, float* gaze_out, float* boxes_out,
                                           float* scores_out, void* ws, size_t ws_bytes) {
  MCG_CHECK_ARG(frame_of, "mcg_decoder_forward_indexed: null frame_of (mcg_decoder_forward is the plain path)");
  MCG_CHECK_ARG(pyramid_frames > 0, "mcg_decoder_forward_indexed: empty pyramid store (pyramid_frames=%d)", pyramid_frames);
  return decoder_forward(e, (hipStream_t)s_, pyramid, pyramid_frames, frame_of, N, ClipTable::uniform(N, clip_length), H, W, img_hw, gaze_out, boxes_out,
                         scores_out, ws, ws_bytes);
}

extern "C" int mcg_decoder_forward_ragged(mcg_engine* e, mcg_stream s_, const void* const pyramid[4], int pyramid_frames, const int32_t* frame_of,
                                          int N, const int* clip_start, int num_clips, int max_clip_length, int H, int W, const int* img_hw,
                                          float* gaze_out, float* boxes_out, float* scores_out, void* ws, size_t ws_bytes) {
  MCG_CHECK_ARG(clip_start, "mcg_decoder_forward_ragged: null clip_start (mcg_decoder_forward is the equal-length path)");
  MCG_CHECK_ARG(pyramid_frames > 0, "mcg_decoder_forward_ragged: empty pyramid store (pyramid_frames=%d)", pyramid_frames);
  MCG_CHECK_ARG(frame_of || pyramid_frames == N, "mcg_decoder_forward_ragged: without frame_of the pyramid holds one row per frame (%d rows, %d frames)",
                pyramid_frames, N);
  return decoder_forward(e, (hipStream_t)s_, pyramid, pyramid_frames, frame_of, N, ClipTable{clip_start, num_clips, max_clip_length}, H, W, img_hw,
                         gaze_out, boxes_out, scores_out, ws, ws_bytes);
}

extern "C" int mcg_deferred_pyramid_levels(const mcg_engine* e, void* slot, int N, int H, int W, void* levels[4], int* deferred) {
  MCG_CHECK_ARG(e && slot && levels, "mcg_deferred_pyramid_levels: null pointer");
  MCG_TRY(check_shape(N, H, W));
  const DeferSlot d = defer_layout(e, N, H, W, (char*)slot);
  for (int i = 0; i < 4; ++i) levels[i] = d.p[i];
  if (deferred) *deferred = d.deferred ? 1 : 0;
  return MCG_OK;
}

extern "C" int mcg_backbone_fpn_forward_deferred(mcg_engine* e, mcg_stream s, const float* img, int N, int H, int W, int chunk, void* slot,
                                                 size_t slot_bytes, void* ws, size_t ws_bytes) {
  MCG_CHECK_ARG(e && slot, "mcg_backbone_fpn_forward_deferred: null pointer");
  MCG_TRY(check_shape(N, H, W));
  const DeferSlot d = defer_layout(e, N, H, W, (char*)slot);
  if (slot_bytes < d.total) { mcg_set_error("mcg_backbone_fpn_forward_deferred: slot too small (%zu < %zu)", slot_bytes, d.total); return MCG_ERR_WORKSPACE; }
  return trunk_forward(e, s, img, N, H, W, chunk, d.p, ws, ws_bytes, false,
                       TrunkKeep{d.deferred ? d.inner : nullptr, d.lateral ? d.c2 : nullptr, d.lateral ? d.l1 : nullptr});
}

extern "C" int mcg_deferred_pyramid_state(const mcg_engine* e, void* slot, int N, int H, int W, void** inner, int** flags, int** counts, int** lists,
                                          int* blocks, int* lateral_deferred) {
  MCG_CHECK_ARG(e && slot, "mcg_deferred_pyramid_state: null pointer");
  MCG_TRY(check_shape(N, H, W));
  const DeferSlot d = defer_layout(e, N, H, W, (char*)slot);
  if (inner) *inner = d.inner;
  if (flags) *flags = d.istate;
  if (counts) *counts = d.icount;
  if (lists) *lists = d.ilist;
  if (blocks) *blocks = d.nblk;
  if (lateral_deferred) *lateral_deferred = d.lateral ? 1 : 0;
  return MCG_OK;
}

static int decoder_forward_deferred(mcg_engine* e, mcg_stream s, void* slot, size_t slot_bytes, int N, const ClipTable& ct, int H, int W,
                                    const int* img_hw, float* gaze_out, float* boxes_out, float* scores_out, void* ws, size_t ws_bytes) {
  MCG_CHECK_ARG(e && slot, "mcg_decoder_forward_deferred: null pointer");
  MCG_TRY(check_shape(N, H, W));
  const DeferSlot d = defer_layout(e, N, H, W, (char*)slot);
  if (slot_bytes < d.total) { mcg_set_error("mcg_decoder_forward_deferred: slot too small (%zu < %zu)", slot_bytes, d.total); return MCG_ERR_WORKSPACE; }
  return decoder_forward(e, (hipStream_t)s, d.p, N, nullptr, N, ct, H, W, img_hw, gaze_out, boxes_out, scores_out, ws, ws_bytes, &d);
}

extern "C" int mcg_decoder_forward_deferred(mcg_engine* e, mcg_stream s, void* slot, size_t slot_bytes, int N, int clip_length, int H, int W,
                                            const int* img_hw, float* gaze_out, float* boxes_out, float* scores_out, void* ws, size_t ws_bytes) {
  return decoder_forward_deferred(e, s, slot, slot_bytes, N, ClipTable::uniform(N, clip_length), H, W, img_hw, gaze_out, boxes_out, scores_out, ws, ws_bytes);
}

extern "C" int mcg_decoder_forward_deferred_ragged(mcg_engine* e, mcg_stream s, void* slot, size_t slot_bytes, int N, const int* clip_start,
                                                   int num_clips, int max_clip_length, int H, int W, const int* img_hw, float* gaze_out,
                                                   float* boxes_out, float* scores_out, void* ws, size_t ws_bytes) {
  MCG_CHECK_ARG(clip_start, "mcg_decoder_forward_deferred_ragged: null clip_start (mcg_decoder_forward_deferred is the equal-length path)");
  return decoder_forward_deferred(e, s, slot, slot_bytes, N, ClipTable{clip_start, num_clips, max_clip_length}, H, W, img_hw, gaze_out, boxes_out,
                                  scores_out, ws, ws_bytes);
}

static int clip_forward(mcg_engine* e, mcg_stream s_, const float* img, int N, const ClipTable& ct, int H, int W, const int* img_hw, int chunk,
                        float* gaze_out, float* boxes_out, float* scores_out, void* ws, size_t ws_bytes) {
  MCG_CHECK_ARG(e && img && gaze_out && boxes_out && scores_out && ws, "mcg_clip_forward: null pointer");
  MCG_TRY(check_shape(N, H, W));
  MCG_TRY(check_clips("mcg_clip_forward", N, ct));
  const size_t need = mcg_engine_workspace_bytes(e, N, H, W, chunk);
  if (ws_bytes < need) { mcg_set_error("mcg_clip_forward: workspace too small (%zu < %zu)", ws_bytes, need); return MCG_ERR_WORKSPACE; }
  char* base = (char*)ws;
  const size_t trunk_bytes = mcg_trunk_workspace_bytes(e, N, H, W, chunk);
  const size_t slot_bytes = defer_layout(e, N, H, W, nullptr).total;
  const size_t off = trunk_bytes + slot_bytes;
  MCG_TRY(mcg_backbone_fpn_forward_deferred(e, s_, img, N, H, W, chunk, base + trunk_bytes, slot_bytes, base, trunk_bytes));
  return decoder_forward_deferred(e, s_, base + trunk_bytes, slot_bytes, N, ct, H, W, img_hw, gaze_out, boxes_out, scores_out, base + off,
                                  ws_bytes - off);
}

extern "C" int mcg_clip_forward(mcg_engine* e, mcg_stream s_, const float* img, int N, int clip_length, int H, int W,
                                const int* img_hw, int chunk, float* gaze_out, float* boxes_out, float* scores_out,
                                void* ws, size_t ws_bytes) {
  return clip_forward(e, s_, img, N, ClipTable::uniform(N, clip_length), H, W, img_hw, chunk, gaze_out, boxes_out, scores_out, ws, ws_bytes);
}

extern "C" int mcg_clip_forward_ragged(mcg_engine* e, mcg_stream s_, const float* img, int N, const int* clip_start, int num_clips,
                                       int max_clip_length, int H, int W, const int* img_hw, int chunk, float* gaze_out, float* boxes_out,
                                       float* scores_out, void* ws, size_t ws_bytes) {
  MCG_CHECK_ARG(clip_start, "mcg_clip_forward_ragged: null clip_start (mcg_clip_forward is the equal-length path)");
  return clip_forward(e, s_, img, N, ClipTable{clip_start, num_clips, max_clip_length}, H, W, img_hw, chunk, gaze_out, boxes_out, scores_out, ws,
                      ws_bytes);
}
```

mcgaze_amd/csrc/roi_align.hip:

```cpp
#include "common.hpp"
#include "roi_sample.hpp"

struct RoiLevels {
  const void* feat[4];
  int h[4], w[4];
  float scale[4];
};

template <typename T>
__global__ __launch_bounds__(256) void roi_align_kernel(RoiLevels lv, int C, const float* __restrict__ boxes, int boxes_per_frame,
                                                        const int32_t* __restrict__ frame_of, int pyramid_frames,
                                                        T* __restrict__ out, int32_t* __restrict__ levels_out, float finest_scale) {
  constexpr int EPC = Elem<T>::kPerChunk;
  constexpr int P = 7, S = 2, NS = P * S;
  __shared__ int s_lo[2][NS], s_hi[2][NS];
  __shared__ float s_l[2][NS], s_h[2][NS];
  __shared__ int s_valid[2][NS];
  const int box = blockIdx.x, tid = threadIdx.x;
  const float x1 = boxes[box * 4 + 0], y1 = boxes[box * 4 + 1], x2 = boxes[box * 4 + 2], y2 = boxes[box * 4 + 3];
  const int level = roi_level(x1, y1, x2, y2, finest_scale);
  const int H = lv.h[level], W = lv.w[level];
  const float ss = lv.scale[level];
  if (tid < 2 * NS) {
    const int axis = tid / NS, i = tid % NS;
    int lo, hi, valid;
    float l;
    roi_axis_sample<P, S>(axis == 0 ? y1 : x1, axis == 0 ? y2 : x2, ss, axis == 0 ? H : W, i, lo, hi, l, valid);
    s_lo[axis][i] = lo; s_hi[axis][i] = hi; s_l[axis][i] = l; s_h[axis][i] = 1.f - l; s_valid[axis][i] = valid;
  }
  if (tid == 0) {
    if (levels_out) levels_out[box] = level;
  }
  __syncthreads();
  int frame = box / boxes_per_frame;
  bool bad_row = false;
  if (frame_of) {
    frame = __builtin_amdgcn_readfirstlane(frame_of[frame]);
    bad_row = frame < 0 || frame >= pyramid_frames;
    if (bad_row) frame = 0;
  }
  const T* __restrict__ F = (const T*)lv.feat[level] + (long long)frame * H * W * C;
  const int groups = C / EPC, bins_per_pass = 256 / groups;
  const int cg = tid % groups, slot = tid / groups;
  if (bad_row) {
    float nan[EPC];
#pragma unroll
    for (int e = 0; e < EPC; ++e) nan[e] = __builtin_nanf("");
    for (int bin = slot; bin < P * P; bin += bins_per_pass)
      *(uint4*)(out + ((long long)box * (P * P) + bin) * C + cg * EPC) = f32_to_chunk(nan, (T*)nullptr);
    return;
  }
  for (int bin = slot; bin < P * P; bin += bins_per_pass) {
    const int ph = bin / P, pw = bin % P;
    float acc[EPC];
#pragma unroll
    for (int e = 0; e < EPC; ++e) acc[e] = 0.f;
#pragma unroll
    for (int iy = 0; iy < S; ++iy) {
      const int yi = ph * S + iy;
#pragma unroll
      for (int ix = 0; ix < S; ++ix) {
        const int xi = pw * S + ix;
        if (!(s_valid[0][yi] && s_valid[1][xi])) continue;
        const int yl = s_lo[0][yi], yh = s_hi[0][yi], xl = s_lo[1][xi], xh = s_hi[1][xi];
        const float ly = s_l[0][yi], hy = s_h[0][yi], lx = s_l[1][xi], hx = s_h[1][xi];
        const float w1 = hy * hx, w2 = hy * lx, w3 = ly * hx, w4 = ly * lx;
        float v1[EPC], v2[EPC], v3[EPC], v4[EPC];
        chunk_to_f32(*(const uint4*)(F + ((long long)yl * W + xl) * C + cg * EPC), v1, (T*)nullptr);
        chunk_to_f32(*(const uint4*)(F + ((long long)yl * W + xh) * C + cg * EPC), v2, (T*)nullptr);
        chunk_to_f32(*(const uint4*)(F + ((long long)yh * W + xl) * C + cg * EPC), v3, (T*)nullptr);
        chunk_to_f32(*(const uint4*)(F + ((long long)yh * W + xh) * C + cg * EPC), v4, (T*)nullptr);
#pragma unroll
        for (int e = 0; e < EPC; ++e) acc[e] += w1 * v1[e] + w2 * v2[e] + w3 * v3[e] + w4 * v4[e];
      }
    }
#pragma unroll
    for (int e = 0; e < EPC; ++e) acc[e] *= (1.0f / (float)(S * S));
    *(uint4*)(out + ((long long)box * (P * P) + bin) * C + cg * EPC) = f32_to_chunk(acc, (T*)nullptr);
  }
}

constexpr int kMarkMaxBlocks = 64;
__global__ __launch_bounds__(256) void roi_mark_kernel(const float* __restrict__ boxes, int boxes_per_frame, int level_deferred, int H, int W,
                                                       float ss, int* __restrict__ state, int* __restrict__ list, int* __restrict__ count,
                                                       float finest_scale) {
  constexpr int P = 7, S = 2, NS = P * S;
  __shared__ int s_hit[2][kMarkMaxBlocks];
  const int box = blockIdx.x, tid = threadIdx.x;
  const float x1 = boxes[box * 4 + 0], y1 = boxes[box * 4 + 1], x2 = boxes[box * 4 + 2], y2 = boxes[box * 4 + 3];
  if (roi_level(x1, y1, x2, y2, finest_scale) != level_deferred) return;
  const int by_n = (H + 7) / 8, bx_n = (W + 7) / 8;
  if (tid < 2 * kMarkMaxBlocks) s_hit[tid / kMarkMaxBlocks][tid % kMarkMaxBlocks] = 0;
  __syncthreads();
  if (tid < 2 * NS) {
    const int axis = tid / NS, i = tid % NS;
    int lo, hi, valid;
    float l;
    roi_axis_sample<P, S>(axis == 0 ? y1 : x1, axis == 0 ? y2 : x2, ss, axis == 0 ? H : W, i, lo, hi, l, valid);
    if (valid) { s_hit[axis][lo >> 3] = 1; s_hit[axis][hi >> 3] = 1; }
  }
  __syncthreads();
  const int frame = box / boxes_per_frame;
  for (int t = tid; t < by_n * bx_n; t += 256) {
    const int by = t / bx_n, bx = t - by * bx_n;
    if (s_hit[0][by] && s_hit[1][bx]) {
      const int id = frame * (by_n * bx_n) + t;
      if (atomicCAS(&state[id], 0, 1) == 0) list[atomicAdd(count, 1)] = id;
    }
  }
}
__host__ __device__ inline int inner_neighbour(int id, int k, int by_n, int bx_n) {
  const int bpf = by_n * bx_n, f = id / bpf, rem = id - f * bpf, by = rem / bx_n + k / 3 - 1, bx = rem % bx_n + k % 3 - 1;
  return (by < 0 || by >= by_n || bx < 0 || bx >= bx_n) ? -1 : f * bpf + by * bx_n + bx;
}
__global__ __launch_bounds__(256) void inner_mark_kernel(const int* __restrict__ out_list, const int* __restrict__ out_count, int by_n, int bx_n,
                                                         int nblk, int* __restrict__ state, int* __restrict__ list, int* __restrict__ count) {
  const int n = min(*out_count, nblk) * 9;
  for (int t = blockIdx.x * blockDim.x + threadIdx.x; t < n; t += gridDim.x * blockDim.x) {
    const int src = out_list[t / 9];
    if (src < 0 || src >= nblk) continue;
    const int id = inner_neighbour(src, t % 9, by_n, bx_n);
    if (id >= 0 && atomicCAS(&state[id], 0, 1) == 0) list[atomicAdd(count, 1)] = id;
  }
}
int launch_inner_mark(hipStream_t s, const int* out_list, const int* out_count, int H, int W, int nblk, int* state, int* list, int* count) {
  const long long threads = (long long)nblk * 9;
  const int blocks = (int)((threads + 255) / 256 < 1024 ? (threads + 255) / 256 : 1024);
  hipLaunchKernelGGL(inner_mark_kernel, dim3(blocks > 0 ? blocks : 1), dim3(256), 0, s, out_list, out_count, (H + 7) / 8, (W + 7) / 8, nblk, state,
                     list, count);
  MCG_CHECK_LAUNCH("inner_mark");
  return MCG_OK;
}
extern "C" int mcg_inner_block_neighbours(int id, int H, int W, int out[9]) {
  int n = 0;
  for (int k = 0; k < 9; ++k) {
    const int v = inner_neighbour(id, k, (H + 7) / 8, (W + 7) / 8);
    if (v >= 0) out[n++] = v;
  }
  return n;
}
__global__ void defer_clear_kernel(int* __restrict__ p, int n) {
  for (int i = blockIdx.x * blockDim.x + threadIdx.x; i < n; i += gridDim.x * blockDim.x) p[i] = 0;
}
bool roi_mark_supported(int H, int W) { return (H + 7) / 8 <= kMarkMaxBlocks && (W + 7) / 8 <= kMarkMaxBlocks; }
int launch_defer_clear(hipStream_t s, int* p, int n) {
  const int blocks = (n + 255) / 256 < 1024 ? (n + 255) / 256 : 1024;
  hipLaunchKernelGGL(defer_clear_kernel, dim3(blocks > 0 ? blocks : 1), dim3(256), 0, s, p, n);
  MCG_CHECK_LAUNCH("defer_clear");
  return MCG_OK;
}
int launch_roi_mark(hipStream_t s, const float* boxes, int num_boxes, int boxes_per_frame, int level, int H, int W, int stride, int* state,
                    int* list, int* count) {
  MCG_CHECK_ARG(roi_mark_supported(H, W), "roi_mark: deferred level of %dx%d pixels exceeds %d blocks per axis", H, W, kMarkMaxBlocks);
  hipLaunchKernelGGL(roi_mark_kernel, dim3(num_boxes), dim3(256), 0, s, boxes, boxes_per_frame, level, H, W, 1.0f / (float)stride, state, list,
                     count, 56.f);
  MCG_CHECK_LAUNCH("roi_mark");
  return MCG_OK;
}

int launch_roi_align(hipStream_t s, mcg_dtype dt, const void* const feats[4], const int feat_h[4], const int feat_w[4],
                     const int strides[4], int C, const float* boxes, int num_boxes, int boxes_per_frame, const int32_t* frame_of,
                     int pyramid_frames, void* out, int32_t* levels_out) {
  RoiLevels lv;
  for (int i = 0; i < 4; ++i) {
    lv.feat[i] = feats[i]; lv.h[i] = feat_h[i]; lv.w[i] = feat_w[i];
    lv.scale[i] = 1.0f / (float)strides[i];
  }
  const int epc = mcg_is16(dt) ? 8 : 4;
  MCG_CHECK_ARG(C % epc == 0 && C / epc <= 256 && 256 % (C / epc) == 0, "roi_align: unsupported channel count %d", C);
  dispatch_elem(dt, [&](auto e) {
    hipLaunchKernelGGL(roi_align_kernel<decltype(e)>, dim3(num_boxes), dim3(256), 0, s, lv, C, boxes, boxes_per_frame, frame_of, pyramid_frames, (decltype(e)*)out, levels_out, 56.f);
  });
  MCG_CHECK_LAUNCH("roi_align");
  return MCG_OK;
}

extern "C" int mcg_roi_align(mcg_stream s, mcg_dtype dt, const void* const feats[4], const int feat_h[4], const int feat_w[4],
                             const int strides[4], int C, const float* boxes, int num_boxes, int boxes_per_frame,
                             void* out, int32_t* levels_out) {
  MCG_CHECK_ARG(feats && feat_h && feat_w && strides && boxes && out, "mcg_roi_align: null pointer");
  MCG_CHECK_ARG(num_boxes > 0 && boxes_per_frame > 0, "mcg_roi_align: empty box set");
  for (int i = 0; i < 4; ++i) MCG_CHECK_ARG(feats[i] && feat_h[i] > 0 && feat_w[i] > 0 && strides[i] > 0, "mcg_roi_align: bad level %d", i);
  return launch_roi_align((hipStream_t)s, dt, feats, feat_h, feat_w, strides, C, boxes, num_boxes, boxes_per_frame, nullptr, 0, out, levels_out);
}

extern "C" int mcg_roi_align_indexed(mcg_stream s, mcg_dtype dt, const void* const feats[4], const int feat_h[4], const int feat_w[4],
                                     const int strides[4], int C, const float* boxes, int num_boxes, int boxes_per_frame,
                                     const int32_t* frame_of, int pyramid_frames, void* out, int32_t* levels_out) {
  MCG_CHECK_ARG(feats && feat_h && feat_w && strides && boxes && out && frame_of, "mcg_roi_align_indexed: null pointer");
  MCG_CHECK_ARG(num_boxes > 0 && boxes_per_frame > 0 && pyramid_frames > 0, "mcg_roi_align_indexed: empty box set or pyramid");
  for (int i = 0; i < 4; ++i) MCG_CHECK_ARG(feats[i] && feat_h[i] > 0 && feat_w[i] > 0 && strides[i] > 0, "mcg_roi_align_indexed: bad level %d", i);
  return launch_roi_align((hipStream_t)s, dt, feats, feat_h, feat_w, strides, C, boxes, num_boxes, boxes_per_frame, frame_of, pyramid_frames,
                          out, levels_out);
}
```

mcgaze_amd/csrc/roi_sample.hpp:

```cpp
#pragma once

__device__ __forceinline__ int roi_level(float x1, float y1, float x2, float y2, float finest_scale) {
  const float sc = sqrtf((x2 - x1) * (y2 - y1));
  int level = (int)fminf(fmaxf(floorf(log2f(sc / finest_scale + 1e-6f)), 0.f), 3.f);
  if (!(sc == sc)) level = 0;
  return level;
}

template <int P, int S>
__device__ __forceinline__ void roi_axis_sample(float a1, float a2, float ss, int L, int i, int& lo_out, int& hi_out, float& l_out, int& valid_out) {
  const float start = a1 * ss - 0.5f, end = a2 * ss - 0.5f;
  const float bin = (end - start) / (float)P;
  float c = start + (float)(i / S) * bin + ((float)(i % S) + 0.5f) * bin / (float)S;
  const int valid = c >= -1.0f && c <= (float)L;
  c = fmaxf(c, 0.f);
  int lo = (int)c, hi;
  if (lo >= L - 1) {
    lo = hi = L - 1;
    c = (float)lo;
  } else {
    hi = lo + 1;
  }
  lo_out = lo; hi_out = hi; l_out = c - (float)lo; valid_out = valid;
}
```

mcgaze_amd/csrc/wino_x3.hpp:

```cpp
#pragma once
#include "igemm_dma.hpp"

namespace wnx {
constexpr int KS = 16;
constexpr int UNT = 128;
constexpr int ustage(int g) { return (g + 2) * 4 * 2 * 1024; }
constexpr int wcap(int g, int ct) { return (g == 4 && ct == 4) ? 32 * 1024 : 48 * 1024; }
constexpr int W_LDS = 4 * 64 * 128 * 4;
}

struct WinoParams {
  const float* x;
  const void* u;
  const float* bias;
  float* y;
  int H, W, PW, frames, Cin, Cout, relu;
  int total_pairs, n_tiles;
  int tpf, gpf;
  float wscale;
  const int* blk_list;
  const int* blk_count;
  int bxn, bpf;
};

namespace wnx {
__device__ __forceinline__ void tile_range(const WinoParams& p, int mt, int MT, int& q0, int& q_end) {
  if (p.tpf > 0) {
    const int f = mt / p.tpf, t = mt - f * p.tpf;
    q0 = f * p.gpf + t * MT;
    q_end = min(q0 + MT, (f + 1) * p.gpf);
  } else {
    q0 = mt * MT;
    q_end = min(q0 + MT, p.total_pairs);
  }
}
__device__ __forceinline__ int slot_of(const WinoParams& p, int q) { const int R = q / p.PW; return R + R / p.H + 1; }
__device__ __forceinline__ uint32_t row_base(const WinoParams& p, int f, int y) { return (uint32_t)(((long long)(f * p.H + y) * p.W) * p.Cin * 4); }
struct WinRow { bool ok; uint32_t base; };
__device__ __forceinline__ WinRow win_row(const WinoParams& p, int sg) {
  const int H1 = p.H + 1, f = sg / H1, r = sg - f * H1;
  return {r != 0 && f < p.frames, row_base(p, f, r - 1)};
}
template <int G>
__device__ __forceinline__ void win_lane(int lane, int pc, int& x, int& c) {
  const int l_ph = lane >> 5, l_i = (lane >> 2) & 7, l_cs = lane & 3;
  const int b = pc / (G / 2), hph = pc - b * (G / 2);
  x = (8 * b + l_i) * G + 2 * hph + l_ph - 1;
  c = l_cs ^ ((2 * b + (l_i >> 2)) & 3);
}
__device__ __forceinline__ uint32_t win_voff(const WinoParams& p, int x, int c) {
  return (unsigned)x < (unsigned)p.W ? (uint32_t)((x * p.Cin + 4 * c) * 4) : MCG_OOB_OFFSET;
}
template <int G>
__device__ __forceinline__ const char* a_addr(const char* win, int jrow, int rowb, int xg, int toff, int chunk) {
  const int wx = G * xg + toff;
  const int pp = wx / G, ph = wx - pp * G, swz = (pp >> 2) & 3;
  const int off = jrow * rowb + (pp >> 3) * (G * 512) + ph * 512 + (pp & 7) * 64;
  return win + off + ((chunk ^ swz) << 4);
}
__device__ __forceinline__ void f23_position(int nu, int (&toff)[2], float& sgn) {
  toff[0] = nu == 0 ? 0 : 1; toff[1] = nu == 3 ? 3 : 2;
  sgn = nu == 1 ? 1.f : -1.f;
}
__device__ __forceinline__ void f23_chunk(const uint4& d0, const uint4& d1, float sgn, float* v) {
  const uint32_t e0[4] = {d0.x, d0.y, d0.z, d0.w};
  const uint32_t e1[4] = {d1.x, d1.y, d1.z, d1.w};
#pragma unroll
  for (int e = 0; e < 4; ++e) v[e] = fmaf(sgn, __uint_as_float(e1[e]), __uint_as_float(e0[e]));
}
__device__ __forceinline__ void f23_fragment(const uint4 (&d)[2][2], float sgn, bf16x8& ah, bf16x8& al) {
  float v[8];
#pragma unroll
  for (int c = 0; c < 2; ++c) f23_chunk(d[0][c], d[1][c], sgn, v + 4 * c);
  const uint4 v0 = make_uint4(__float_as_uint(v[0]), __float_as_uint(v[1]), __float_as_uint(v[2]), __float_as_uint(v[3]));
  const uint4 v1 = make_uint4(__float_as_uint(v[4]), __float_as_uint(v[5]), __float_as_uint(v[6]), __float_as_uint(v[7]));
  split_f32x8(v0, v1, ah, al);
}
template <int PP, int NT>
__device__ __forceinline__ void stage_acc(float* C, int nu, int rt, int ct, int lane, const f32x16& a) {
#pragma unroll
  for (int r = 0; r < 16; ++r) C[(nu * PP + rt * 32 + mfma32_row(r, lane)) * NT + ct * 32 + (lane & 31)] = a[r];
}
template <int G, int PP, int NT>
__device__ __forceinline__ void epilogue_item(const WinoParams& p, const float* C, int prl, int ch4, int n0, float wsc, int R, int xo, bool valid) {
  constexpr int NV = G + 2;
  if (!valid) return;
  float4 bv = make_float4(0.f, 0.f, 0.f, 0.f);
  if (p.bias) bv = *(const float4*)(p.bias + n0 + ch4);
  float4 m[NV];
#pragma unroll
  for (int v = 0; v < NV; ++v) m[v] = *(const float4*)(C + (v * PP + prl) * NT + ch4);
  float4 y[G];
  if constexpr (G == 2) {
    y[0] = make_float4(((m[0].x + m[1].x) + m[2].x) * wsc + bv.x, ((m[0].y + m[1].y) + m[2].y) * wsc + bv.y, ((m[0].z + m[1].z) + m[2].z) * wsc + bv.z, ((m[0].w + m[1].w) + m[2].w) * wsc + bv.w);
    y[1] = make_float4(((m[1].x - m[2].x) - m[3].x) * wsc + bv.x, ((m[1].y - m[2].y) - m[3].y) * wsc + bv.y, ((m[1].z - m[2].z) - m[3].z) * wsc + bv.z, ((m[1].w - m[2].w) - m[3].w) * wsc + bv.w);
  } else {
#define MCG_W4(F)                                                                                                            \
    {                                                                                                                    \
      const float s12 = m[1].F + m[2].F, d12 = m[1].F - m[2].F, s34 = m[3].F + m[4].F, d34 = m[3].F - m[4].F;            \
      y[0].F = ((m[0].F + s12) + s34) * wsc + bv.F;                                                                      \
      y[1].F = fmaf(2.f, d34, d12) * wsc + bv.F;                                                                         \
      y[2].F = fmaf(4.f, s34, s12) * wsc + bv.F;                                                                         \
      y[3].F = (fmaf(8.f, d34, d12) + m[5].F) * wsc + bv.F;                                                              \
    }
    MCG_W4(x) MCG_W4(y) MCG_W4(z) MCG_W4(w)
#undef MCG_W4
  }
  float* yp = p.y + ((long long)R * p.W + xo) * p.Cout + n0 + ch4;
#pragma unroll
  for (int j = 0; j < G; ++j) {
    if (xo + j >= p.W) break;
    float4 o = y[j];
    if (p.relu) { o.x = fmaxf(o.x, 0.f); o.y = fmaxf(o.y, 0.f); o.z = fmaxf(o.z, 0.f); o.w = fmaxf(o.w, 0.f); }
    *(float4*)(yp + (long long)j * p.Cout) = o;
  }
}
}

template <int NB, int RH, int RT, int CT, int G>
__global__ __launch_bounds__(64 * (G + 2) * RH, 1) void wino_x3_kernel(const WinoParams p) {
  using namespace wnx;
  constexpr int NV = G + 2, NW = NV * RH, NTHREADS = 64 * NW, MT = 32 * RH * RT, NT = 32 * CT;
  constexpr int ROWB = NB * 1024, WIN_CAP = wcap(G, CT), USTAGE = ustage(G);
  constexpr int BSTAGE = NV * CT * 2 * 1024;
  constexpr int BPW = 2 * NV * CT / NW;
  constexpr int MAXP = (WIN_CAP / 1024 + NW - 1) / NW;
  constexpr int NTERM = G == 2 ? 2 : 4;
  static_assert((2 * NV * CT) % NW == 0 && UNT % NT == 0 && (G == 2 || G == 4), "tile shape");
  extern __shared__ __attribute__((aligned(16))) char smem[];
  char* const s_win = smem;
  char* const s_b = smem + 2 * WIN_CAP;
  const int tid = threadIdx.x, lane = tid & 63;
  const int wave = __builtin_amdgcn_readfirstlane(tid >> 6);
  const int nu = wave % NV, rh = wave / NV;
  const int logical = xcd_remap(blockIdx.x, gridDim.x);
  const int mt = logical / p.n_tiles, ntile = logical - mt * p.n_tiles;
  int q0, q_end;
  tile_range(p, mt, MT, q0, q_end);
  const int q_last = q_end - 1;
  const int sig_b = __builtin_amdgcn_readfirstlane(slot_of(p, q0) - 1);
  const int NP = __builtin_amdgcn_readfirstlane((slot_of(p, q_last) - sig_b + 2) * NB);
  const int NSL = p.Cin / KS, KT = 3 * NSL;

  const int n0 = ntile * NT;
  const u32x4 srd_x = make_srd(p.x);
  const u32x4 srd_u = make_srd((const char*)p.u + (size_t)(n0 / UNT) * KT * USTAGE + (size_t)((n0 % UNT) / 32) * 2048);
  const uint32_t lds_win = (uint32_t)(uintptr_t)(__attribute__((address_space(3))) char*)s_win;
  const uint32_t lds_b = (uint32_t)(uintptr_t)(__attribute__((address_space(3))) char*)s_b;

  uint32_t prow[MAXP];
  int pblk[MAXP];
  bool pok[MAXP], prowok[MAXP];
  static_for<MAXP>([&](auto nc) {
    constexpr int n = decltype(nc)::value;
    const int pi = wave + NW * n, j = pi / NB, b = pi - j * NB;
    const WinRow row = win_row(p, sig_b + j);
    pok[n] = pi < NP;
    prowok[n] = __builtin_amdgcn_readfirstlane(row.ok ? 1 : 0) != 0;
    prow[n] = __builtin_amdgcn_readfirstlane(row.base);
    pblk[n] = b;
  });
  auto piece_voff = [&](int pc) -> uint32_t {
    int x, c;
    win_lane<G>(lane, pc, x, c);
    return win_voff(p, x, c);
  };
  auto issue_window = [&](int cs, uint32_t dst) {
    static_for<MAXP>([&](auto nc) {
      constexpr int n = decltype(nc)::value;
      if (pok[n]) {
        const uint32_t v = prowok[n] ? piece_voff(pblk[n]) : MCG_OOB_OFFSET;
        lds_dma16<0>(v, srd_x, prow[n] + (uint32_t)cs * (KS * 4), dst + (uint32_t)(wave + NW * n) * 1024u);
      }
    });
  };
  const uint32_t b_voff = (uint32_t)lane * 16u;
  auto issue_b = [&](int k, uint32_t dst) {
    static_for<BPW>([&](auto ic) {
      constexpr int i = decltype(ic)::value;
      const int pc = wave * BPW + i, pnu = pc / (2 * CT), rest = pc - pnu * (2 * CT);
      lds_dma16<i * 1024>(b_voff, srd_u, (uint32_t)k * USTAGE + (uint32_t)pnu * 8192u + (uint32_t)rest * 1024u, dst + (uint32_t)wave * (BPW * 1024u));
    });
  };

  int toff[NTERM];
  float tco[NTERM];
  if constexpr (G == 2) {
    tco[0] = 1.f;
    f23_position(nu, toff, tco[1]);
  } else {
    const int o4[6][4] = {{0, 2, 4, 4}, {1, 2, 3, 4}, {1, 2, 3, 4}, {1, 2, 3, 4}, {1, 2, 3, 4}, {1, 3, 5, 5}};
    const float c4[6][4] = {{4.f, -5.f, 1.f, 0.f}, {-4.f, -4.f, 1.f, 1.f}, {4.f, -4.f, -1.f, 1.f}, {-2.f, -1.f, 2.f, 1.f}, {2.f, -1.f, -2.f, 1.f}, {4.f, -5.f, 1.f, 0.f}};
#pragma unroll
    for (int t = 0; t < 4; ++t) {
      toff[t] = o4[0][t]; tco[t] = c4[0][t];
#pragma unroll
      for (int v = 1; v < 6; ++v)
        if (nu == v) { toff[t] = o4[v][t]; tco[t] = c4[v][t]; }
    }
  }
  const int pl = lane & 31, h = lane >> 5;
  const char* ap[RT][NTERM][2];
#pragma unroll
  for (int rt = 0; rt < RT; ++rt) {
    const int q = min(q0 + (RT * rh + rt) * 32 + pl, q_last);
    const int xg = q - q / p.PW * p.PW;
    const int jrow = slot_of(p, q) - sig_b - 1;
#pragma unroll
    for (int t = 0; t < NTERM; ++t)
#pragma unroll
      for (int ch = 0; ch < 2; ++ch) ap[rt][t][ch] = a_addr<G>(s_win, jrow, ROWB, xg, toff[t], 2 * h + ch);
  }
  const char* const bp = s_b + nu * (CT * 2 * 1024) + lane * 16;

  f32x16 acc[RT][CT];
#pragma unroll
  for (int i = 0; i < RT; ++i)
#pragma unroll
    for (int j = 0; j < CT; ++j)
#pragma unroll
      for (int r = 0; r < 16; ++r) acc[i][j][r] = 0.f;

  struct Raw { uint4 d[RT][NTERM][2]; };
  auto load_raw = [&](auto wbc, auto kyc, Raw& r) {
    constexpr int AOFF = decltype(wbc)::value * WIN_CAP + decltype(kyc)::value * ROWB;
#pragma unroll
    for (int rt = 0; rt < RT; ++rt)
#pragma unroll
      for (int t = 0; t < NTERM; ++t) { r.d[rt][t][0] = *(const uint4*)(ap[rt][t][0] + AOFF); r.d[rt][t][1] = *(const uint4*)(ap[rt][t][1] + AOFF); }
  };
  auto transform = [&](const Raw& r, bf16x8 (&ah)[RT], bf16x8 (&al)[RT]) {
#pragma unroll
    for (int rt = 0; rt < RT; ++rt) {
      if constexpr (G == 2) {
        f23_fragment(r.d[rt], tco[1], ah[rt], al[rt]);
      } else {
        float v[8];
#pragma unroll
        for (int c = 0; c < 2; ++c) {
          const uint32_t e0[4] = {r.d[rt][0][c].x, r.d[rt][0][c].y, r.d[rt][0][c].z, r.d[rt][0][c].w};
          const uint32_t e1[4] = {r.d[rt][1][c].x, r.d[rt][1][c].y, r.d[rt][1][c].z, r.d[rt][1][c].w};
          const uint32_t e2[4] = {r.d[rt][2][c].x, r.d[rt][2][c].y, r.d[rt][2][c].z, r.d[rt][2][c].w};
          const uint32_t e3[4] = {r.d[rt][3][c].x, r.d[rt][3][c].y, r.d[rt][3][c].z, r.d[rt][3][c].w};
#pragma unroll
          for (int e = 0; e < 4; ++e)
            v[4 * c + e] = fmaf(tco[3], __uint_as_float(e3[e]), fmaf(tco[2], __uint_as_float(e2[e]), fmaf(tco[1], __uint_as_float(e1[e]), tco[0] * __uint_as_float(e0[e]))));
        }
        const uint4 v0 = make_uint4(__float_as_uint(v[0]), __float_as_uint(v[1]), __float_as_uint(v[2]), __float_as_uint(v[3]));
        const uint4 v1 = make_uint4(__float_as_uint(v[4]), __float_as_uint(v[5]), __float_as_uint(v[6]), __float_as_uint(v[7]));
        split_f32x8(v0, v1, ah[rt], al[rt]);
      }
    }
  };

  issue_window(0, lds_win);
  issue_b(0, lds_b);
  bf16x8 fh[2][RT], fl[2][RT];
  asm volatile("s_waitcnt vmcnt(0)" ::: "memory");
  __builtin_amdgcn_s_barrier();
  {
    Raw r0;
    load_raw(std::integral_constant<int, 0>{}, std::integral_constant<int, 0>{}, r0);
    transform(r0, fh[0], fl[0]);
  }
  constexpr int NM1 = RT * CT;
  constexpr int PVALU = (G == 2 ? 32 : 56) * RT, VPM = (PVALU + 2 * NM1 - 1) / (2 * NM1);
#pragma nounroll
  for (int s2 = 0; s2 < NSL / 2; ++s2) {
    static_for<6>([&](auto uc) {
      constexpr int U = decltype(uc)::value, KY = U % 3, SL = U & 1, WB = U / 3;
      constexpr int U1 = (U + 1) % 6, KY1 = U1 % 3, WB1 = U1 / 3;
      constexpr int BOFF = SL * BSTAGE;
      const int k = 6 * s2 + U, cs = 2 * s2 + WB;
      asm volatile("s_waitcnt vmcnt(0) lgkmcnt(0)" ::: "memory");
      __builtin_amdgcn_s_barrier();
      bf16x8 bh[CT], bl[CT];
#pragma unroll
      for (int ct = 0; ct < CT; ++ct) {
        bh[ct] = __builtin_bit_cast(bf16x8, *(const uint4*)(bp + BOFF + ct * 2048));
        bl[ct] = __builtin_bit_cast(bf16x8, *(const uint4*)(bp + BOFF + ct * 2048 + 1024));
      }
      Raw raw;
      load_raw(std::integral_constant<int, WB1>{}, std::integral_constant<int, KY1>{}, raw);
      __builtin_amdgcn_sched_barrier(0);
      const uint32_t kn = (uint32_t)min(k + 1, KT - 1) * USTAGE, bdst = lds_b + (SL ^ 1) * BSTAGE + (uint32_t)wave * (BPW * 1024u);
      static_for<NM1>([&](auto mc) {
        constexpr int M = decltype(mc)::value, I = M / CT, J = M % CT;
        acc[I][J] = x3_mfma(fl[SL][I], bh[J], acc[I][J]);
        if constexpr (M < BPW) {
          const int pc = wave * BPW + M, pnu = pc / (2 * CT), rest = pc - pnu * (2 * CT);
          lds_dma16<M * 1024>(b_voff, srd_u, kn + (uint32_t)pnu * 8192u + (uint32_t)rest * 1024u, bdst);
        }
        __builtin_amdgcn_sched_barrier(0);
      });
      if constexpr (NM1 < BPW) {
        static_for<BPW - NM1>([&](auto mc) {
          constexpr int M = NM1 + decltype(mc)::value;
          const int pc = wave * BPW + M, pnu = pc / (2 * CT), rest = pc - pnu * (2 * CT);
          lds_dma16<M * 1024>(b_voff, srd_u, kn + (uint32_t)pnu * 8192u + (uint32_t)rest * 1024u, bdst);
        });
      }
      if (KY == 0 && cs + 1 < NSL) issue_window(cs + 1, lds_win + (WB ^ 1) * WIN_CAP);
      transform(raw, fh[SL ^ 1], fl[SL ^ 1]);
#pragma unroll
      for (int i2 = 0; i2 < RT; ++i2)
#pragma unroll
        for (int j2 = 0; j2 < CT; ++j2) acc[i2][j2] = x3_mfma(fh[SL][i2], bl[j2], acc[i2][j2]);
#pragma unroll
      for (int i2 = 0; i2 < RT; ++i2)
#pragma unroll
        for (int j2 = 0; j2 < CT; ++j2) acc[i2][j2] = x3_mfma(fh[SL][i2], bh[j2], acc[i2][j2]);
      static_for<2 * NM1 - 1>([&](auto) {
        __builtin_amdgcn_sched_group_barrier(0x008, 1, 0);
        __builtin_amdgcn_sched_group_barrier(0x002, VPM, 0);
      });
      __builtin_amdgcn_sched_group_barrier(0x008, 1, 0);
      __builtin_amdgcn_sched_group_barrier(0x002, 8, 0);
    });
  }
  asm volatile("s_waitcnt vmcnt(0) lgkmcnt(0)" ::: "memory");
  __syncthreads();

  constexpr int PP = 32 * RT, CPR = NT / 4;
  static_assert(NV * PP * NT * 4 <= 2 * WIN_CAP + 2 * BSTAGE, "epilogue staging");
  float* const C = (float*)smem;
  const float wsc = p.wscale > 0.f ? p.wscale : 1.f;
#pragma unroll 1
  for (int pass = 0; pass < RH; ++pass) {
    if (rh == pass) {
#pragma unroll
      for (int rt = 0; rt < RT; ++rt)
#pragma unroll
        for (int ct = 0; ct < CT; ++ct) stage_acc<PP, NT>(C, nu, rt, ct, lane, acc[rt][ct]);
    }
    __syncthreads();
    for (int item = tid; item < PP * CPR; item += NTHREADS) {
      const int prl = item / CPR, ch4 = (item - prl * CPR) * 4;
      const int q = q0 + pass * PP + prl, R = q / p.PW;
      epilogue_item<G, PP, NT>(p, C, prl, ch4, n0, wsc, R, G * (q - R * p.PW), q < q_end);
    }
    __syncthreads();
  }
}

typedef uint32_t u32x4v __attribute__((ext_vector_type(4)));
template <int IMM>
__device__ __forceinline__ void buf_load16(u32x4v& dst, uint32_t voffset, const u32x4& srd, uint32_t soffset_uniform) {
  asm volatile("buffer_load_dwordx4 %0, %1, %2, %3 offen offset:%4" : "=&v"(dst) : "v"(voffset), "s"(srd), "s"(soffset_uniform), "n"(IMM) : "memory");
}
template <int NB, bool BLK>
__device__ __forceinline__ void wino_x3w_tile(const WinoParams& p, const int logical) {
  using namespace wnx;
  constexpr int G = 2, NW = 4, RT = 4, CT = 4, MT = 128, NT = 128;
  constexpr int ROWB = NB * 1024, WIN_CAP = 48 * 1024, USTAGE = ustage(2);
  constexpr int MAXP = WIN_CAP / 1024 / NW;
  constexpr int HB = MAXP / 2;
  constexpr int BWR = 10;
  static_assert(!BLK || (NB == 1 && RT * BWR <= NW * MAXP), "block tile: one piece per window row, every block's rows in the window");
  extern __shared__ __attribute__((aligned(16))) char smem[];
  char* const s_win = smem;
  const int tid = threadIdx.x, lane = tid & 63;
  const int wave = __builtin_amdgcn_readfirstlane(tid >> 6);
  const int nu = wave;
  const int mt = logical / p.n_tiles, ntile = logical - mt * p.n_tiles;
  int q0 = 0, q_end = 0;
  int bf[RT], by0[RT], bxg[RT];
  uint32_t bokm = 0;
  if constexpr (BLK) {
    const int cnt = __builtin_amdgcn_readfirstlane(*p.blk_count);
#pragma unroll
    for (int rt = 0; rt < RT; ++rt) {
      const int e = RT * mt + rt;
      if (e < cnt) bokm |= 1u << rt;
      const int id = __builtin_amdgcn_readfirstlane(p.blk_list[e < cnt ? e : RT * mt]);
      const int f = id / p.bpf, r = id - f * p.bpf, by = r / p.bxn;
      bf[rt] = f; by0[rt] = 8 * by; bxg[rt] = 4 * (r - by * p.bxn);
    }
  } else {
    tile_range(p, mt, MT, q0, q_end);
  }
  auto pick = [&](const int (&a)[RT], int i) { return i == 0 ? a[0] : (i == 1 ? a[1] : (i == 2 ? a[2] : a[3])); };
  const int q_last = q_end - 1;
  const int sig_b = BLK ? 0 : __builtin_amdgcn_readfirstlane(slot_of(p, q0) - 1);
  const int NP = BLK ? RT * BWR : __builtin_amdgcn_readfirstlane((slot_of(p, q_last) - sig_b + 2) * NB);
  const int NSL = p.Cin / KS, KT = 3 * NSL;
  const int n0 = ntile * NT;
  const u32x4 srd_x = make_srd(p.x);
  const u32x4 srd_u = make_srd((const char*)p.u + (size_t)(n0 / UNT) * KT * USTAGE);
  const uint32_t lds_win = (uint32_t)(uintptr_t)(__attribute__((address_space(3))) char*)s_win;

  uint32_t prow[MAXP];
  int pxo[MAXP];
  uint32_t pokm = 0, prowokm = 0;
  static_for<MAXP>([&](auto nc) {
    constexpr int n = decltype(nc)::value;
    const int pi = wave + NW * n;
    if constexpr (BLK) {
      const int rb = min(pi / BWR, RT - 1), y = pick(by0, rb) + pi - BWR * rb - 1, f = pick(bf, rb);
      const bool rowok = y >= 0 && y < p.H;
      if (pi < NP && ((bokm >> rb) & 1)) pokm |= 1u << n;
      if (rowok) prowokm |= 1u << n;
      prow[n] = __builtin_amdgcn_readfirstlane(row_base(p, f, rowok ? y : 0));
      pxo[n] = __builtin_amdgcn_readfirstlane(2 * pick(bxg, rb));
    } else {
      const WinRow row = win_row(p, sig_b + pi / NB);
      if (pi < NP) pokm |= 1u << n;
      if (row.ok) prowokm |= 1u << n;
      prow[n] = __builtin_amdgcn_readfirstlane(row.base);
      pxo[n] = 0;
    }
  });
  pokm = __builtin_amdgcn_readfirstlane(pokm);
  prowokm = __builtin_amdgcn_readfirstlane(prowokm);
  int l_x, l_c;
  win_lane<G>(lane, wave & (NB - 1), l_x, l_c);
  const uint32_t w_voff = BLK ? (uint32_t)(4 * l_c * 4) : win_voff(p, l_x, l_c);
  auto piece_voff = [&](auto nc) -> uint32_t {
    constexpr int n = decltype(nc)::value;
    if (!(prowokm & (1u << n))) return MCG_OOB_OFFSET;
    if constexpr (BLK) {
      const int x = pxo[n] + l_x;
      return (unsigned)x < (unsigned)p.W ? (uint32_t)(x * p.Cin * 4) + w_voff : MCG_OOB_OFFSET;
    } else {
      return w_voff;
    }
  };
  auto issue_window = [&](auto hc, int cs, uint32_t dst) {
    constexpr int h0 = decltype(hc)::value * HB;
    static_for<HB>([&](auto nc) {
      constexpr int n = h0 + decltype(nc)::value;
      if (pokm & (1u << n)) {
        const uint32_t v = piece_voff(std::integral_constant<int, n>{});
        lds_dma16<0>(v, srd_x, prow[n] + (uint32_t)cs * (KS * 4), dst + (uint32_t)(wave + NW * n) * 1024u);
      }
    });
  };
  const uint32_t b_voff = (uint32_t)lane * 16u + (uint32_t)nu * 8192u;
  u32x4v bh[2][CT], bl[2][CT];
  auto issue_b1 = [&](auto slc, auto jc, uint32_t koff) {
    constexpr int SLX = decltype(slc)::value, J = decltype(jc)::value;
    if constexpr (J & 1) buf_load16<(J & 3) * 1024>(bl[SLX][J >> 1], b_voff, srd_u, koff + (J >> 2) * 4096u);
    else buf_load16<(J & 3) * 1024>(bh[SLX][J >> 1], b_voff, srd_u, koff + (J >> 2) * 4096u);
  };

  int toff[2];
  float tsg;
  f23_position(nu, toff, tsg);
  const int pl = lane & 31, h = lane >> 5;
  const char* ap[RT][2][2];
#pragma unroll
  for (int rt = 0; rt < RT; ++rt) {
    int jrow, xg;
    if constexpr (BLK) {
      jrow = BWR * rt + (pl >> 2);
      xg = pl & 3;
    } else {
      const int q = min(q0 + rt * 32 + pl, q_last);
      xg = q - q / p.PW * p.PW;
      jrow = slot_of(p, q) - sig_b - 1;
    }
#pragma unroll
    for (int t = 0; t < 2; ++t)
#pragma unroll
      for (int ch = 0; ch < 2; ++ch) ap[rt][t][ch] = a_addr<G>(s_win, jrow, ROWB, xg, toff[t], 2 * h + ch);
  }

  f32x16 acc[RT][CT];
#pragma unroll
  for (int i = 0; i < RT; ++i)
#pragma unroll
    for (int j = 0; j < CT; ++j)
#pragma unroll
      for (int r = 0; r < 16; ++r) acc[i][j][r] = 0.f;

  struct Raw { uint4 d[RT][2][2]; };
  auto load_raw = [&](auto wbc, auto kyc, Raw& r) {
    constexpr int AOFF = decltype(wbc)::value * WIN_CAP + decltype(kyc)::value * ROWB;
#pragma unroll
    for (int rt = 0; rt < RT; ++rt)
#pragma unroll
      for (int t = 0; t < 2; ++t) { r.d[rt][t][0] = *(const uint4*)(ap[rt][t][0] + AOFF); r.d[rt][t][1] = *(const uint4*)(ap[rt][t][1] + AOFF); }
  };

  issue_window(std::integral_constant<int, 0>{}, 0, lds_win);
  issue_window(std::integral_constant<int, 1>{}, 0, lds_win);
  static_for<8>([&](auto jc) { issue_b1(std::integral_constant<int, 0>{}, jc, 0u); });
  if (NSL > 1) issue_window(std::integral_constant<int, 0>{}, 1, lds_win + WIN_CAP);
  bf16x8 fh[2][RT], fl[2][RT];
  asm volatile("s_waitcnt vmcnt(0)" ::: "memory");
  __builtin_amdgcn_s_barrier();
  {
    Raw r0;
    load_raw(std::integral_constant<int, 0>{}, std::integral_constant<int, 0>{}, r0);
#pragma unroll
    for (int rt = 0; rt < RT; ++rt) f23_fragment(r0.d[rt], tsg, fh[0][rt], fl[0][rt]);
  }
  constexpr int NM1 = RT * CT;
  uint32_t nh[RT][4], nl[RT][4];
#pragma nounroll
  for (int s2 = 0; s2 < NSL / 2; ++s2) {
    static_for<6>([&](auto uc) {
      constexpr int U = decltype(uc)::value, KY = U % 3, SL = U & 1, WB = U / 3;
      constexpr int U1 = (U + 1) % 6, KY1 = U1 % 3, WB1 = U1 / 3;
      const int k = 6 * s2 + U, cs = 2 * s2 + WB;
      asm volatile("s_waitcnt vmcnt(0)"
                   : "+v"(bh[SL][0]), "+v"(bh[SL][1]), "+v"(bh[SL][2]), "+v"(bh[SL][3]), "+v"(bl[SL][0]), "+v"(bl[SL][1]), "+v"(bl[SL][2]), "+v"(bl[SL][3])
                   :
                   : "memory");
      if constexpr (KY == 2) __builtin_amdgcn_s_barrier();
      Raw raw;
      load_raw(std::integral_constant<int, WB1>{}, std::integral_constant<int, KY1>{}, raw);
      __builtin_amdgcn_sched_barrier(0);
      const uint32_t kn = (uint32_t)min(k + 1, KT - 1) * USTAGE;
      auto vmem_slot = [&](auto vc) {
        constexpr int V = decltype(vc)::value;
        if constexpr (V < 8) {
          issue_b1(std::integral_constant<int, SL ^ 1>{}, std::integral_constant<int, V>{}, kn);
        } else if constexpr (KY != 1 && V < 8 + HB) {
          constexpr int n = (KY == 0 ? HB : 0) + (V - 8);
          const int csn = KY == 0 ? cs + 1 : cs + 2;
          if (csn < NSL && (pokm & (1u << n))) {
            const uint32_t v = piece_voff(std::integral_constant<int, n>{});
            lds_dma16<0>(v, srd_x, prow[n] + (uint32_t)csn * (KS * 4), lds_win + (KY == 0 ? (WB ^ 1) : WB) * WIN_CAP + (uint32_t)(wave + NW * n) * 1024u);
          }
        }
      };
      static_for<NM1>([&](auto mc) {
        constexpr int M = decltype(mc)::value, I = M / CT, J = M % CT;
        acc[I][J] = x3_mfma(fl[SL][I], __builtin_bit_cast(bf16x8, bh[SL][J]), acc[I][J]);
        if constexpr (M % 3 == 0) {
          __builtin_amdgcn_sched_barrier(0);
          vmem_slot(std::integral_constant<int, M / 3>{});
          __builtin_amdgcn_sched_barrier(0);
        }
      });
      __builtin_amdgcn_sched_barrier(0);
      static_for<8>([&](auto qc) {
        constexpr int Q = decltype(qc)::value, I = Q & 3, TERM3 = Q >> 2;
        constexpr int XR = Q >> 1, XC = Q & 1;
        {
          float v[4];
          f23_chunk(raw.d[XR][0][XC], raw.d[XR][1][XC], tsg, v);
          split_pair(v[0], v[1], nh[XR][2 * XC], nl[XR][2 * XC]);
          split_pair(v[2], v[3], nh[XR][2 * XC + 1], nl[XR][2 * XC + 1]);
        }
#pragma unroll
        for (int j2 = 0; j2 < CT; ++j2)
          acc[I][j2] = x3_mfma(fh[SL][I], __builtin_bit_cast(bf16x8, TERM3 ? bh[SL][j2] : bl[SL][j2]), acc[I][j2]);
        asm volatile("" : "+v"(nh[XR][2 * XC]), "+v"(nh[XR][2 * XC + 1]), "+v"(nl[XR][2 * XC]), "+v"(nl[XR][2 * XC + 1]));
        static_for<4>([&](auto) {
          __builtin_amdgcn_sched_group_barrier(0x008, 1, 0);
          __builtin_amdgcn_sched_group_barrier(0x002, 4, 0);
        });
        __builtin_amdgcn_sched_barrier(0);
        vmem_slot(std::integral_constant<int, 6 + Q>{});
        __builtin_amdgcn_sched_barrier(0);
      });
#pragma unroll
      for (int rt = 0; rt < RT; ++rt) {
        fh[SL ^ 1][rt] = __builtin_bit_cast(bf16x8, make_uint4(nh[rt][0], nh[rt][1], nh[rt][2], nh[rt][3]));
        fl[SL ^ 1][rt] = __builtin_bit_cast(bf16x8, make_uint4(nl[rt][0], nl[rt][1], nl[rt][2], nl[rt][3]));
      }
    });
  }
  asm volatile("s_waitcnt vmcnt(0) lgkmcnt(0)"
               : "+v"(bh[0][0]), "+v"(bh[0][1]), "+v"(bh[0][2]), "+v"(bh[0][3]), "+v"(bl[0][0]), "+v"(bl[0][1]), "+v"(bl[0][2]), "+v"(bl[0][3]),
                 "+v"(bh[1][0]), "+v"(bh[1][1]), "+v"(bh[1][2]), "+v"(bh[1][3]), "+v"(bl[1][0]), "+v"(bl[1][1]), "+v"(bl[1][2]), "+v"(bl[1][3])
               :
               : "memory");
  __syncthreads();

  constexpr int PP = 64, CPR = NT / 4;
  float* const C = (float*)smem;
  const float wsc = p.wscale > 0.f ? p.wscale : 1.f;
#pragma unroll
  for (int pass = 0; pass < 2; ++pass) {
#pragma unroll
    for (int rt = 0; rt < 2; ++rt)
#pragma unroll
      for (int ct = 0; ct < CT; ++ct) stage_acc<PP, NT>(C, nu, rt, ct, lane, acc[2 * pass + rt][ct]);
    __syncthreads();
    for (int item = tid; item < PP * CPR; item += 256) {
      const int prl = item / CPR, ch4 = (item - prl * CPR) * 4;
      if constexpr (BLK) {
        const int rt = 2 * pass + (prl >> 5), pl = prl & 31;
        const int y = pick(by0, rt) + (pl >> 2), xo = G * (pick(bxg, rt) + (pl & 3));
        epilogue_item<G, PP, NT>(p, C, prl, ch4, n0, wsc, pick(bf, rt) * p.H + y, xo, ((bokm >> rt) & 1) && y < p.H && xo < p.W);
      } else {
        const int q = q0 + pass * PP + prl, R = q / p.PW;
        epilogue_item<G, PP, NT>(p, C, prl, ch4, n0, wsc, R, G * (q - R * p.PW), q < q_end);
      }
    }
    __syncthreads();
  }
}
template <int NB>
__global__ __launch_bounds__(256, 1) void wino_x3w_kernel(const WinoParams p) {
  wino_x3w_tile<NB, false>(p, xcd_remap(blockIdx.x, gridDim.x));
}
__global__ __launch_bounds__(256, 1) void wino_x3w_blocks_kernel(const WinoParams p) {
  const int units = __builtin_amdgcn_readfirstlane(((*p.blk_count + 3) >> 2) * p.n_tiles);
  const int padded = p.n_tiles == 2 ? (units + 15) & ~15 : units;
  for (int u = blockIdx.x; u < padded; u += gridDim.x) {
    int logical = u;
    if (p.n_tiles == 2) { const int x = u & 7, j = u >> 3; logical = (j & 1) + 2 * (x + 8 * (j >> 1)); }
    if (logical < units) wino_x3w_tile<1, true>(p, logical);
  }
}

static inline int wino_x3_tile_groups(int g, int shape) { return g == 2 ? ((shape == 0 || shape == 3) ? 128 : (shape == 1 ? 64 : 32)) : (shape == 0 ? 64 : 32); }
static inline int wino_x3_tile_channels(int shape) { return (shape == 0 || shape == 3) ? 128 : 64; }
static inline int wino_x3_pieces(int W, int g) { return (g * ((W + g - 1) / g) + 2 + 8 * g - 1) / (8 * g) * (g / 2); }
static inline int wino_x3_max_rows(int H, int W, int mt, int g, bool cross) {
  const int PW = (W + g - 1) / g;
  int rows = (PW - 1 + mt - 1) / PW + 1;
  if (!cross && rows > H) rows = H;
  const int nz = cross ? (rows >= 2 ? (rows - 2) / H + 1 : 0) : 0;
  return rows + nz + 2;
}
static inline int wino_x3_nb_template(int pieces) { return pieces <= 1 ? 1 : (pieces <= 2 ? 2 : 4); }
static inline bool wino_x3_operands_ok(int frames, int H, int W, int Cin, int Cout) {
  const long long px = (long long)frames * H * W;
  return Cin % 32 == 0 && Cout % wnx::UNT == 0 && H >= 1 && W >= 2 && frames >= 1 && px * Cin * 4 < MCG_DMA_MAX_BYTES &&
         px * Cout * 4 < MCG_DMA_MAX_BYTES && px < 0x7fffffffLL;
}
static inline int wino_x3_mode(int frames, int H, int W, int Cin, int Cout, int g) {
  if (!wino_x3_operands_ok(frames, H, W, Cin, Cout) || (g != 2 && g != 4)) return 0;
  if (g == 4 && (W % 4 != 0 || W < 16)) return 0;
  const int pcs = wino_x3_pieces(W, g);
  if (pcs > 4) return 0;
  const int nb = wino_x3_nb_template(pcs);
  const int mt = wino_x3_tile_groups(g, 0), cap = wnx::wcap(g, 4);
  if (wino_x3_max_rows(H, W, mt, g, true) * nb * 1024 <= cap) return 1;
  if (wino_x3_max_rows(H, W, mt, g, false) * nb * 1024 <= cap) return 2;
  return 0;
}
static inline bool wino_x3_applicable(int frames, int H, int W, int Cin, int Cout, int g = 2) { return wino_x3_mode(frames, H, W, Cin, Cout, g) != 0; }
static inline size_t wino_x3_weight_bytes(int Cin, int Cout, int g = 2) { return (size_t)(Cout / wnx::UNT) * (3 * Cin / wnx::KS) * wnx::ustage(g); }

template <int NB, int RH, int RT, int CT, int G>
static inline int launch_wino_x3_t(hipStream_t s, const WinoParams& p, int grid) {
  constexpr int kLds = 2 * wnx::wcap(G, CT) + 2 * ((G + 2) * CT * 2 * 1024);
  if (kernel_ready<wino_x3_kernel<NB, RH, RT, CT, G>>(kLds)) return 1;
  hipLaunchKernelGGL((wino_x3_kernel<NB, RH, RT, CT, G>), dim3(grid), dim3(64 * (G + 2) * RH), kLds, s, p);
  return hipGetLastError() == hipSuccess ? 0 : 1;
}
template <int NB>
static inline int launch_wino_x3w(hipStream_t s, const WinoParams& p, int grid) {
  if (kernel_ready<wino_x3w_kernel<NB>>(wnx::W_LDS)) return 1;
  hipLaunchKernelGGL((wino_x3w_kernel<NB>), dim3(grid), dim3(256), wnx::W_LDS, s, p);
  return hipGetLastError() == hipSuccess ? 0 : 1;
}
template <int NB>
static inline int launch_wino_x3_nb(hipStream_t s, const WinoParams& p, int g, int shape, int grid) {
  if (g == 2 && shape == 3) return launch_wino_x3w<NB>(s, p, grid);
  if (g == 4) return shape == 0 ? launch_wino_x3_t<NB, 2, 1, 4, 4>(s, p, grid) : launch_wino_x3_t<NB, 1, 1, 2, 4>(s, p, grid);
  if (shape == 0) return launch_wino_x3_t<NB, 2, 2, 4, 2>(s, p, grid);
  if (shape == 1) return launch_wino_x3_t<NB, 2, 1, 2, 2>(s, p, grid);
  return launch_wino_x3_t<NB, 1, 1, 2, 2>(s, p, grid);
}
static inline bool wino_x3_blocks_applicable(int frames, int H, int W, int Cin, int Cout) { return wino_x3_operands_ok(frames, H, W, Cin, Cout); }
static inline int wino_x3_blocks_per_frame(int H, int W) { return ((H + 7) / 8) * ((W + 7) / 8); }
static inline int launch_wino_x3_blocks(hipStream_t s, WinoParams p, const int* list, const int* count, int max_blocks) {
  int cus;
  if (kernel_ready<wino_x3w_blocks_kernel>(wnx::W_LDS, &cus)) return 1;
  p.PW = (p.W + 1) / 2;
  p.n_tiles = p.Cout / 128;
  p.bxn = (p.W + 7) / 8;
  p.bpf = wino_x3_blocks_per_frame(p.H, p.W);
  p.blk_list = list; p.blk_count = count;
  const int units = (max_blocks + 3) / 4 * p.n_tiles;
  const int grid = units < cus ? units : cus / 16 * 16;
  hipLaunchKernelGGL(wino_x3w_blocks_kernel, dim3(grid > 0 ? grid : 1), dim3(256), wnx::W_LDS, s, p);
  return hipGetLastError() == hipSuccess ? 0 : 1;
}
static const int kWinoMinGrid = 130;
static inline int launch_wino_x3(hipStream_t s, WinoParams p, int shape = -1, int g = 2) {
  const int mode = wino_x3_mode(p.frames, p.H, p.W, p.Cin, p.Cout, g);
  if (mode == 0) return 1;
  p.PW = (p.W + g - 1) / g;
  p.gpf = p.H * p.PW;
  p.total_pairs = p.frames * p.gpf;
  auto mtiles = [&](int sh) {
    const int mt = wino_x3_tile_groups(g, sh);
    return mode == 2 ? p.frames * ((p.gpf + mt - 1) / mt) : (p.total_pairs + mt - 1) / mt;
  };
  auto grid_of = [&](int sh) { return mtiles(sh) * (p.Cout / wino_x3_tile_channels(sh)); };
  if (shape < 0) shape = grid_of(0) >= kWinoMinGrid ? (g == 2 ? 3 : 0) : ((g == 2 && grid_of(1) >= kWinoMinGrid) ? 1 : 2);
  if (g == 4 && (shape == 1 || shape == 3)) shape = 2;
  p.n_tiles = p.Cout / wino_x3_tile_channels(shape);
  p.tpf = mode == 2 ? (p.gpf + wino_x3_tile_groups(g, shape) - 1) / wino_x3_tile_groups(g, shape) : 0;
  const int grid = grid_of(shape);
  const int nb = wino_x3_nb_template(wino_x3_pieces(p.W, g));
  if (nb == 1) return launch_wino_x3_nb<1>(s, p, g, shape, grid);
  if (nb == 2) return launch_wino_x3_nb<2>(s, p, g, shape, grid);
  return launch_wino_x3_nb<4>(s, p, g, shape, grid);
}
```

mcgaze_amd/lib.py:

```python
import ctypes as C
import os

_HERE = os.path.dirname(os.path.abspath(__file__))
LIB_PATH = os.environ.get('MCGAZE_LIB') or os.path.join(_HERE, 'libmcgaze_hip.so')

MCG_OK = 0
MCG_F32, MCG_BF16, MCG_F16X3, MCG_F16 = 0, 1, 2, 3
ABI_VERSION = 19
RES_NONE, RES_ADD, RES_UPSAMPLE_ADD = 0, 1, 2
FLAG_STAGED_GEMM, FLAG_NO_SPECIALISED, FLAG_NO_ATTN_BLOCK = 1, 2, 4

STAGE_KEYS = [
    'IN_PROJ_W', 'IN_PROJ_B', 'OUT_PROJ_W', 'OUT_PROJ_B', 'ATTN_LN_G', 'ATTN_LN_B', 'DYN_W', 'DYN_B',
    'NORM_IN_G', 'NORM_IN_B', 'NORM_OUT_G', 'NORM_OUT_B', 'FC_W', 'FC_B', 'FC_LN_G', 'FC_LN_B', 'IIC_LN_G', 'IIC_LN_B',
    'FFN1_W', 'FFN1_B', 'FFN2_W', 'FFN2_B', 'FFN_LN_G', 'FFN_LN_B', 'CLS_FC_W', 'CLS_LN_G', 'CLS_LN_B',
    'REG_FC_W', 'REG_LN_G', 'REG_LN_B', 'HEAD_CLS_W', 'HEAD_CLS_B', 'HEAD_REG_W', 'HEAD_REG_B', 'OUT_PROJ_WF', 'CLS_FC_WF', 'REG_FC_WF', 'IN_PROJ_WF', 'DYN_WF']
GAZE_KEYS = ['FC_W', 'LN_G', 'LN_B', 'OUT_W', 'OUT_B', 'FUSE_W', 'FUSE_B']
SW_COUNT, GW_COUNT = len(STAGE_KEYS), len(GAZE_KEYS)

EXPORTS = ['mcg_abi_version', 'mcg_build_id', 'mcg_last_error', 'mcg_device_info', 'mcg_nchw_to_nhwc', 'mcg_nhwc_to_nchw', 'mcg_conv2d',
           'mcg_stem_workspace_bytes', 'mcg_stem_forward', 'mcg_roi_align', 'mcg_stage_workspace_bytes', 'mcg_stage_forward',
           'mcg_gaze_head_workspace_bytes', 'mcg_gaze_head', 'mcg_engine_create', 'mcg_engine_destroy',
           'mcg_engine_workspace_bytes', 'mcg_trunk_workspace_bytes', 'mcg_decoder_workspace_bytes', 'mcg_backbone_fpn_forward',
           'mcg_decoder_forward', 'mcg_clip_forward', 'mcg_preprocess_frames', 'mcg_engine_set_option', 'mcg_engine_profile_start',
           'mcg_engine_profile_stop', 'mcg_bench_backbone_forward', 'mcg_bottleneck_x3', 'mcg_bench_backbone_levels', 'mcg_conv3x3_wino_x3',
           'mcg_conv3x3_wino_x3_weight_bytes', 'mcg_engine_range_audit', 'mcg_roi_align_indexed', 'mcg_decoder_forward_indexed',
           'mcg_deferred_pyramid_bytes', 'mcg_deferred_pyramid_levels', 'mcg_backbone_fpn_forward_deferred', 'mcg_decoder_forward_deferred',
           'mcg_stage_forward_ragged', 'mcg_decoder_forward_ragged', 'mcg_decoder_forward_deferred_ragged', 'mcg_clip_forward_ragged',
           'mcg_pyramid_scatter_rows', 'mcg_preprocess_head_crops', 'mcg_merge_windows', 'mcg_smooth_gaze', 'mcg_preprocess_frames_nv12',
           'mcg_preprocess_head_crops_nv12', 'mcg_draw_gaze_arrows', 'mcg_draw_gaze_arrows_nv12',
           'mcg_detect_heads_workspace_bytes', 'mcg_detect_heads', 'mcg_letterbox_frames', 'mcg_letterbox_frames_nv12',
           'mcg_track_state_bytes', 'mcg_track_heads', 'mcg_track_heads_motion', 'mcg_live_slots', 'mcg_live_gate', 'mcg_live_lanes', 'mcg_live_gate_lanes',
           'mcg_deferred_pyramid_state', 'mcg_inner_block_neighbours', 'mcg_gaze_targets', 'mcg_gaze_dwell', 'mcg_gaze_targets_poly',
           'mcg_pointwise_stream', 'mcg_pointwise_dyn', 'mcg_pointwise_pair', 'mcg_draw_attention', 'mcg_draw_attention_nv12',
           'mcg_format_labels', 'mcg_draw_labels', 'mcg_draw_labels_nv12', 'mcg_gaze_heat_add', 'mcg_draw_heat', 'mcg_draw_heat_nv12',
           'mcg_anonymize_heads', 'mcg_anonymize_heads_nv12']
LABEL_CHARS = 24
LETTERBOX_U8, LETTERBOX_F16, LETTERBOX_F32 = 0, 1, 2


class ConvDesc(C.Structure):
    _fields_ = [('x', C.c_void_p), ('w', C.c_void_p), ('bias', C.c_void_p), ('residual', C.c_void_p), ('y', C.c_void_p),
                ('N', C.c_int), ('H', C.c_int), ('W', C.c_int), ('Cin', C.c_int), ('Cout', C.c_int), ('KH', C.c_int),
                ('KW', C.c_int), ('stride', C.c_int), ('pad', C.c_int), ('relu', C.c_int), ('residual_mode', C.c_int),
                ('Hr', C.c_int), ('Wr', C.c_int), ('x2', C.c_void_p), ('Cin2', C.c_int), ('stride2', C.c_int), ('H2', C.c_int),
                ('W2', C.c_int), ('tile', C.c_int), ('flags', C.c_int), ('wscale', C.c_float)]


class ConvWeights(C.Structure):
    _fields_ = [('w', C.c_void_p), ('bias', C.c_void_p), ('cin', C.c_int), ('cout', C.c_int), ('k', C.c_int),
                ('stride', C.c_int), ('pad', C.c_int), ('wf', C.c_void_p), ('wscale', C.c_float), ('wf4', C.c_void_p)]


class FusedBlock(C.Structure):
    _fields_ = [('wstream', C.c_void_p), ('bias', C.c_void_p), ('conv2_index', C.c_int), ('cm', C.c_int), ('c', C.c_int), ('cn', C.c_int),
                ('nsrc', C.c_int)]


class ModelWeights(C.Structure):
    _fields_ = [('blocks', C.c_int * 4), ('stem', ConvWeights), ('convs', C.POINTER(ConvWeights)), ('num_convs', C.c_int),
                ('lateral', ConvWeights * 4), ('fpn_out', ConvWeights * 4), ('c3_ds', ConvWeights * 4), ('init_boxes', C.c_void_p),
                ('init_feats', C.c_void_p), ('num_stages', C.c_int), ('stage_weights', C.POINTER(C.c_void_p)),
                ('gaze_weights', C.POINTER(C.c_void_p)), ('bbox_stds', C.c_float * 4), ('fused', C.POINTER(FusedBlock)), ('num_fused', C.c_int)]


class FrameDesc(C.Structure):
    _fields_ = [('src', C.c_void_p), ('src_h', C.c_int), ('src_w', C.c_int), ('src_pitch', C.c_int), ('crop_y', C.c_int),
                ('crop_x', C.c_int), ('crop_h', C.c_int), ('crop_w', C.c_int), ('out_h', C.c_int), ('out_w', C.c_int)]


class ImageDesc(C.Structure):
    _fields_ = [('src', C.c_void_p), ('h', C.c_int), ('w', C.c_int), ('pitch', C.c_int)]


class YuvCoef(C.Structure):
    _fields_ = [(n, C.c_int) for n in ('y_off', 'cy', 'cub', 'cug', 'cvg', 'cvr')]


class Nv12ImageDesc(C.Structure):
    _fields_ = [('y', C.c_void_p), ('uv', C.c_void_p), ('h', C.c_int), ('w', C.c_int), ('pitch_y', C.c_int), ('pitch_uv', C.c_int)]


class Nv12FrameDesc(C.Structure):
    _fields_ = FrameDesc._fields_ + [('uv', C.c_void_p), ('uv_pitch', C.c_int)]


class LetterboxDesc(C.Structure):
    _fields_ = [('frame', FrameDesc), ('top', C.c_int), ('left', C.c_int)]


class Nv12LetterboxDesc(C.Structure):
    _fields_ = [('frame', Nv12FrameDesc), ('top', C.c_int), ('left', C.c_int)]


class ArrowDesc(C.Structure):
    _fields_ = [('seg', C.c_int * 2 * 2 * 3), ('thickness', C.c_int), ('x0', C.c_int), ('y0', C.c_int), ('x1', C.c_int), ('y1', C.c_int),
                ('image', C.c_int), ('flag', C.c_int), ('reserved', C.c_int)]


class StrokeDesc(C.Structure):
    _fields_ = [('seg', C.c_int * 2 * 2 * 3), ('thickness', C.c_int), ('x0', C.c_int), ('y0', C.c_int), ('x1', C.c_int), ('y1', C.c_int),
                ('image', C.c_int), ('flag', C.c_int), ('layer', C.c_int), ('count', C.c_int), ('color', C.c_uint), ('color_active', C.c_uint),
                ('reserved', C.c_int)]


class LabelDesc(C.Structure):
    _fields_ = [(n, C.c_int) for n in ('x', 'y', 'x0', 'y0', 'x1', 'y1', 'image', 'flag', 'len')] + [('color', C.c_uint), ('text', C.c_ubyte * LABEL_CHARS)]


class AnonDesc(C.Structure):
    _fields_ = [(n, C.c_int) for n in ('image', 'flag', 'x0', 'y0', 'x1', 'y1', 'cx2', 'cy2', 'W', 'H', 'shift', 'shape')]


class McgError(RuntimeError):
    pass


_lib = None


def load():
    global _lib
    if _lib is not None:
        return _lib
    if not os.path.exists(LIB_PATH):
        raise McgError(f'{LIB_PATH} not found: build it with `python -c "import __graft_entry__ as g; g.build()"` '
                       f'(or `make -C mcgaze_amd/csrc`); mcgaze_amd has no CPU fallback')
    lib = C.CDLL(LIB_PATH)
    vp, i, sz = C.c_void_p, C.c_int, C.c_size_t
    lib.mcg_abi_version.restype = i
    lib.mcg_last_error.restype = C.c_char_p
    lib.mcg_build_id.restype = C.c_char_p
    lib.mcg_device_info.argtypes = [C.POINTER(i), C.POINTER(sz), C.c_char_p, i]
    lib.mcg_nchw_to_nhwc.argtypes = [vp, i, vp, vp, i, i, i, i]
    lib.mcg_nhwc_to_nchw.argtypes = [vp, i, vp, vp, i, i, i, i]
    lib.mcg_conv2d.argtypes = [vp, i, C.POINTER(ConvDesc)]
    lib.mcg_stem_workspace_bytes.restype = sz
    lib.mcg_stem_workspace_bytes.argtypes = [i, i, i, i]
    lib.mcg_stem_forward.argtypes = [vp, i, vp, vp, vp, vp, i, i, i, vp, sz, i]
    lib.mcg_roi_align.argtypes = [vp, i, C.POINTER(vp), C.POINTER(i), C.POINTER(i), C.POINTER(i), i, vp, i, i, vp, vp]
    lib.mcg_roi_align_indexed.argtypes = [vp, i, C.POINTER(vp), C.POINTER(i), C.POINTER(i), C.POINTER(i), i, vp, i, i, vp, i, vp, vp]
    lib.mcg_stage_workspace_bytes.restype = sz
    lib.mcg_stage_workspace_bytes.argtypes = [i, i]
    lib.mcg_stage_forward.argtypes = [vp, i, C.POINTER(vp), vp, vp, vp, i, i, vp, vp, vp, C.POINTER(C.c_float), vp, sz, i]
    lib.mcg_gaze_head_workspace_bytes.restype = sz
    lib.mcg_gaze_head_workspace_bytes.argtypes = [i, i]
    lib.mcg_gaze_head.argtypes = [vp, i, C.POINTER(vp), vp, i, vp, vp, sz]
    lib.mcg_engine_create.argtypes = [C.POINTER(vp), C.POINTER(ModelWeights), i]
    lib.mcg_engine_destroy.argtypes = [vp]
    lib.mcg_engine_destroy.restype = None
    lib.mcg_engine_workspace_bytes.restype = sz
    lib.mcg_engine_workspace_bytes.argtypes = [vp, i, i, i, i]
    lib.mcg_trunk_workspace_bytes.restype = sz
    lib.mcg_trunk_workspace_bytes.argtypes = [vp, i, i, i, i]
    lib.mcg_decoder_workspace_bytes.restype = sz
    lib.mcg_decoder_workspace_bytes.argtypes = [vp, i]
    lib.mcg_decoder_forward.argtypes = [vp, vp, C.POINTER(vp), i, i, i, i, vp, vp, vp, vp, vp, sz]
    lib.mcg_decoder_forward_indexed.argtypes = [vp, vp, C.POINTER(vp), i, vp, i, i, i, i, vp, vp, vp, vp, vp, sz]
    lib.mcg_backbone_fpn_forward.argtypes = [vp, vp, vp, i, i, i, i, C.POINTER(vp), vp, sz]
    lib.mcg_deferred_pyramid_bytes.restype = sz
    lib.mcg_deferred_pyramid_bytes.argtypes = [vp, i, i, i]
    lib.mcg_deferred_pyramid_levels.argtypes = [vp, vp, i, i, i, C.POINTER(vp), C.POINTER(i)]
    lib.mcg_deferred_pyramid_state.argtypes = [vp, vp, i, i, i, C.POINTER(vp), C.POINTER(vp), C.POINTER(vp), C.POINTER(vp), C.POINTER(i), C.POINTER(i)]
    lib.mcg_inner_block_neighbours.argtypes = [i, i, i, C.POINTER(i)]
    lib.mcg_backbone_fpn_forward_deferred.argtypes = [vp, vp, vp, i, i, i, i, vp, sz, vp, sz]
    lib.mcg_decoder_forward_deferred.argtypes = [vp, vp, vp, sz, i, i, i, i, vp, vp, vp, vp, vp, sz]
    lib.mcg_clip_forward.argtypes = [vp, vp, vp, i, i, i, i, vp, i, vp, vp, vp, vp, sz]
    lib.mcg_stage_forward_ragged.argtypes = [vp, i, C.POINTER(vp), vp, vp, vp, i, vp, i, i, vp, vp, vp, C.POINTER(C.c_float), vp, sz, i]
    lib.mcg_decoder_forward_ragged.argtypes = [vp, vp, C.POINTER(vp), i, vp, i, vp, i, i, i, i, vp, vp, vp, vp, vp, sz]
    lib.mcg_decoder_forward_deferred_ragged.argtypes = [vp, vp, vp, sz, i, vp, i, i, i, i, vp, vp, vp, vp, vp, sz]
    lib.mcg_clip_forward_ragged.argtypes = [vp, vp, vp, i, vp, i, i, i, i, vp, i, vp, vp, vp, vp, sz]
    lib.mcg_pyramid_scatter_rows.argtypes = [vp, i, C.POINTER(vp), C.POINTER(vp), i, i, i, i, vp]
    lib.mcg_merge_windows.argtypes = [vp, vp, vp, vp, i, vp, i, vp, i, i, vp, i, C.c_float]
    lib.mcg_smooth_gaze.argtypes = [vp, vp, i, vp, i, C.c_double, vp]
    lib.mcg_preprocess_frames.argtypes =[vp, vp, i, vp, i, i, C.POINTER(C.c_float), C.POINTER(C.c_float), i]
    lib.mcg_preprocess_head_crops.argtypes = [vp, vp, i, vp, vp, i, C.c_double, i, i, vp, vp, vp, vp, vp, i, i, C.POINTER(C.c_float), C.POINTER(C.c_float), i]
    lib.mcg_preprocess_frames_nv12.argtypes = lib.mcg_preprocess_frames.argtypes + [C.POINTER(YuvCoef)]
    lib.mcg_preprocess_head_crops_nv12.argtypes = lib.mcg_preprocess_head_crops.argtypes + [C.POINTER(YuvCoef)]
    u8p = C.POINTER(C.c_ubyte)
    lib.mcg_draw_gaze_arrows.argtypes = [vp, vp, i, i, i, vp, vp, i, vp, i, C.c_double, i, C.c_double, C.c_double, u8p, vp, vp, vp]
    lib.mcg_draw_gaze_arrows_nv12.argtypes = lib.mcg_draw_gaze_arrows.argtypes
    lib.mcg_detect_heads_workspace_bytes.restype = sz
    lib.mcg_detect_heads_workspace_bytes.argtypes = [i, i]
    lib.mcg_detect_heads.argtypes = [vp, vp, i, i, i, C.c_longlong, i, i, i, vp, C.c_double, C.c_double, i, i, i, i, vp, vp, vp, vp, vp, vp, vp, sz]
    lib.mcg_letterbox_frames.argtypes = [vp, vp, i, vp, i, i, i, i]
    lib.mcg_letterbox_frames_nv12.argtypes = lib.mcg_letterbox_frames.argtypes + [C.POINTER(YuvCoef)]
    lib.mcg_track_state_bytes.restype = sz
    lib.mcg_track_state_bytes.argtypes = [i, i]
    lib.mcg_track_heads.argtypes = [vp, vp, C.c_longlong, vp, i, i, i, i, C.c_double, i, vp, vp, vp, vp, vp, vp, vp]
    lib.mcg_track_heads_motion.argtypes = [vp, vp, C.c_longlong, vp, i, i, i, i, C.c_double, i, C.c_double, C.c_double, vp, vp, vp, vp, vp, vp, vp, vp]
    lib.mcg_live_slots.argtypes = [vp, vp, i, i, i, i, vp, vp, vp, vp, vp]
    lib.mcg_live_gate.argtypes = [vp, vp, vp, i, i, i, i, vp, i, i, i, vp, vp, vp, vp, vp, vp, vp, vp, vp]
    lib.mcg_live_lanes.argtypes = [vp, vp, i, i, i, i, i, vp, vp, vp, vp, vp, vp, vp, vp, vp]
    lib.mcg_live_gate_lanes.argtypes = [vp, vp, vp, vp, i, i, i, i, i, vp, i, i, i, vp, vp, vp, vp, vp, vp, vp, vp, vp, vp, vp]
    lib.mcg_gaze_targets.argtypes = [vp, vp, vp, i, vp, i, vp, vp, i, i, C.c_double, C.c_double, vp, vp, vp, vp, vp, vp]
    lib.mcg_gaze_targets_poly.argtypes = [vp, vp, vp, i, vp, i, vp, i, vp, vp, i, i, C.c_double, C.c_double, vp, vp, vp, vp, vp, vp]
    lib.mcg_draw_attention.argtypes = [vp, vp, i, i, i, vp, vp, i, vp, i, vp, vp, vp, vp, vp, i, vp, vp, i, i, u8p, C.c_double, i, C.c_double, C.c_double,
                                       i, i, vp, sz, vp, vp, vp]
    lib.mcg_draw_attention_nv12.argtypes = lib.mcg_draw_attention.argtypes
    lib.mcg_format_labels.argtypes = [vp, vp, vp, i, i, i, vp]
    lib.mcg_draw_labels.argtypes = [vp, vp, i, i, i, vp, vp, vp, vp, i, vp, i, i, i, u8p, vp, u8p, vp, vp]
    lib.mcg_draw_labels_nv12.argtypes = lib.mcg_draw_labels.argtypes
    lib.mcg_gaze_heat_add.argtypes = [vp, vp, vp, vp, vp, vp, i, vp, vp, i, i, i, i, i, i, i, i, vp, sz]
    lib.mcg_draw_heat.argtypes = [vp, vp, i, i, i, vp, vp, i, i, i, i, i, vp, i]
    lib.mcg_draw_heat_nv12.argtypes = lib.mcg_draw_heat.argtypes
    lib.mcg_anonymize_heads.argtypes = [vp, vp, i, i, i, vp, vp, i, C.c_double, i, i, i, i, u8p, vp, vp]
    lib.mcg_anonymize_heads_nv12.argtypes = lib.mcg_anonymize_heads.argtypes
    lib.mcg_gaze_dwell.argtypes =[vp, vp, vp, vp, vp, vp, i, i, i, i, i, vp, vp, i, vp, vp, vp, i, vp]
    lib.mcg_engine_set_option.argtypes = [vp, C.c_char_p, i]
    lib.mcg_engine_profile_start.argtypes = [vp, i]
    lib.mcg_engine_profile_stop.argtypes = [vp, C.POINTER(i), C.POINTER(C.c_float), C.POINTER(C.c_double), C.POINTER(C.c_double), C.POINTER(i), C.POINTER(i), i]
    lib.mcg_bench_backbone_forward.argtypes = [vp, vp, vp, i, i, i, vp, sz]
    lib.mcg_bench_backbone_levels.argtypes = [vp, vp, i, i, i, C.POINTER(vp)]
    lib.mcg_bottleneck_x3.argtypes = [vp, vp, vp, vp, vp, vp, vp, i, i, i, i, i, i, vp]
    lib.mcg_conv3x3_wino_x3.argtypes = [vp, vp, vp, vp, vp, i, i, i, i, i, i, i, C.c_float, i]
    lib.mcg_conv3x3_wino_x3_weight_bytes.restype = sz
    lib.mcg_pointwise_stream.argtypes = [vp, i, vp, vp, vp, vp, vp, i, i, i, i, i, i, i, i, i, C.c_float, vp, vp, i]
    lib.mcg_pointwise_dyn.argtypes = [vp, i, vp, vp, vp, vp, i, C.c_float, i]
    lib.mcg_pointwise_pair.argtypes = [vp, i, vp, vp, vp, vp, vp, vp, vp, vp, vp, i, i, i, i]
    lib.mcg_engine_range_audit.argtypes = [vp, C.POINTER(C.c_ulonglong), C.POINTER(C.c_char_p), i, C.POINTER(i)]
    lib.mcg_conv3x3_wino_x3_weight_bytes.argtypes = [i, i, i]
    for name in EXPORTS:
        fn = getattr(lib, name)
        if fn.restype is C.c_int and name not in ('mcg_abi_version',):
            fn.restype = i
    if lib.mcg_abi_version() != ABI_VERSION:
        raise McgError(f'ABI mismatch: library reports {lib.mcg_abi_version()}, binding expects {ABI_VERSION}')
    _lib = lib
    return lib


def build_id():
    return load().mcg_build_id().decode()


def source_id():
    import hashlib
    src = os.path.join(_HERE, 'csrc')
    names = sorted(n for n in os.listdir(src) if n.endswith('.hip') or n.endswith('.hpp'))
    h = hashlib.sha256()
    for n in names:
        h.update(open(os.path.join(src, n), 'rb').read())
    h.update(open(os.path.join(_HERE, '..', 'include', 'mcgaze_hip.h'), 'rb').read())
    return h.hexdigest()[:16]


def check(rc, what):
    if rc != MCG_OK:
        msg = load().mcg_last_error().decode(errors='replace')
        raise McgError(f'{what} failed (code {rc}): {msg}')
```

Before: 3637 clips/s.

## Defer FPN P5 output conv to decoder, gated on coarse-level ROI demand

Stops computing the P5 output 3x3 conv in the trunk and keeps its lateral input in the deferred slot. During each decoder stage, the ROI mark kernel counts boxes that map to the coarsest level. A gated Winograd kernel then computes P5 only the first time any stage needs it. This removes P5 work when no ROI uses level 3, at the cost of an extra launch per stage and extra slot memory and counters.

```diff
diff --git a/include/mcgaze_hip.h b/include/mcgaze_hip.h
--- a/include/mcgaze_hip.h
+++ b/include/mcgaze_hip.h
@@ -176,6 +176,10 @@
 int mcg_deferred_pyramid_state(const mcg_engine* e, void* slot, int num_frames, int H, int W, void** inner, int** flags, int** counts,
                                int** lists, int* blocks, int* lateral_deferred);
 int mcg_inner_block_neighbours(int id, int H, int W, int out[9]);
+int mcg_deferred_pyramid_p5_state(const mcg_engine* e, void* slot, int num_frames, int H, int W, void** inner, int** counters, int* stages,
+                                  int* p5_deferred);
+int mcg_deferred_p5_region_bytes(int num_frames, int H, int W, int num_stages, size_t* inner_bytes, size_t* counter_bytes);
+int mcg_roi_level(float x1, float y1, float x2, float y2);
 int mcg_backbone_fpn_forward_deferred(mcg_engine* e, mcg_stream s, const float* img, int num_frames, int H, int W, int chunk_frames,
                                       void* slot, size_t slot_bytes, void* ws, size_t ws_bytes);
 int mcg_decoder_forward_deferred(mcg_engine* e, mcg_stream s, void* slot, size_t slot_bytes, int num_frames, int clip_length, int H, int W,
diff --git a/mcgaze_amd/csrc/check_resources.py b/mcgaze_amd/csrc/check_resources.py
--- a/mcgaze_amd/csrc/check_resources.py
+++ b/mcgaze_amd/csrc/check_resources.py
@@ -4,6 +4,7 @@
 
 RULES = {
     'wino_x3w_kernel': dict(scratch=0, vgpr_spill=0, unit='engine'),
+    'wino_x3w_gated_kernel': dict(scratch=0, vgpr_spill=0, unit='engine'),
     'wino_x3w_blocks_kernel': dict(scratch=0, vgpr_spill=0, unit='engine'),
     'gaze_targets_kernel': dict(scratch=0, vgpr_spill=0, unit='attend'),
     'gaze_targets_poly_kernel': dict(scratch=0, vgpr_spill=0, unit='attend'),
diff --git a/mcgaze_amd/csrc/engine.hip b/mcgaze_amd/csrc/engine.hip
--- a/mcgaze_amd/csrc/engine.hip
+++ b/mcgaze_amd/csrc/engine.hip
@@ -22,7 +22,7 @@
 bool roi_mark_supported(int H, int W);
 int launch_defer_clear(hipStream_t s, int* p, int n);
 int launch_roi_mark(hipStream_t s, const float* boxes, int num_boxes, int boxes_per_frame, int level, int H, int W, int stride, int* state,
-                    int* list, int* count);
+                    int* list, int* count, int* coarse_want);
 int launch_inner_mark(hipStream_t s, const int* out_list, const int* out_count, int H, int W, int nblk, int* state, int* list, int* count);
 
 struct mcg_engine {
@@ -38,6 +38,7 @@
   int wino_tile = -1;
   int fpn_deferred = 1;
   int fpn_lateral_deferred = 1;
+  int fpn_p5_deferred = 1;
   static constexpr int kAuditCap = 256;
   unsigned long long* audit_dev = nullptr;
   std::vector<std::string> audit_names;
@@ -187,6 +188,7 @@
   else if (!strcmp(name, "winograd")) { MCG_CHECK_ARG(value >= 0 && value <= 2, "winograd must be 0, 1 or 2"); e->winograd = value; }
   else if (!strcmp(name, "fpn_deferred")) e->fpn_deferred = value != 0;
   else if (!strcmp(name, "fpn_lateral_deferred")) e->fpn_lateral_deferred = value != 0;
+  else if (!strcmp(name, "fpn_p5_deferred")) e->fpn_p5_deferred = value != 0;
   else if (!strcmp(name, "wino_tile")) { MCG_CHECK_ARG(value >= -1 && value <= 3, "wino_tile must be -1 (by grid size) .. 3"); e->wino_tile = value; }
   else if (!strcmp(name, "range_audit")) {
     MCG_CHECK_ARG(!mcg_is16(e->dt) || !value, "range_audit: f32-storage engines only (MCG_F32, MCG_F16X3)");
@@ -479,9 +481,9 @@
   return MCG_OK;
 }
 
-struct TrunkKeep { char *inner, *c2, *l1; };
+struct TrunkKeep { char *inner, *c2, *l1, *l3; };
 static int trunk_chunk(mcg_engine* e, hipStream_t s, const float* img, int f0, int n, int H, int W, void* const pyr[4], char* wsbase,
-                       bool backbone_only = false, const TrunkKeep tk = TrunkKeep{nullptr, nullptr, nullptr}) {
+                       bool backbone_only = false, const TrunkKeep tk = TrunkKeep{nullptr, nullptr, nullptr, nullptr}) {
   const mcg_dtype dt = e->dt;
   const size_t es = esize(dt);
   TrunkWs t = trunk_layout(dt, n, H, W, wsbase);
@@ -492,6 +494,8 @@
     t.c[0] = tk.c2 + (size_t)f0 * (H / 4) * (W / 4) * 256 * es;
     t.l[1] = tk.l1 + (size_t)f0 * (H / 8) * (W / 8) * 256 * es;
   }
+  const bool p5_deferred = inner0 && tk.l3;
+  if (p5_deferred) t.l[3] = tk.l3 + (size_t)f0 * (H / 32) * (W / 32) * 256 * es;
   MCG_TRY(stem_forward_ctx(s, dt, img + (size_t)f0 * 3 * H * W, e->stem.w, e->stem.bias, t.x0, n, H, W, t.stem_ws, t.stem_bytes, e->ctx));
   AuditCursor au{e, s, 0, e->audit_dev != nullptr && e->audit_names.empty()};
   audit_tensor(au, t.x0, (long long)n * (H / 4) * (W / 4) * 64, "stem");
@@ -529,7 +533,7 @@
                       i == 3 ? 0 : hs[i + 1], i == 3 ? 0 : wsz[i + 1]));
     audit_tensor(au, t.l[i], (long long)n * hs[i] * wsz[i] * 256, "fpn.lateral%d (+ top-down)", i);
   }
-  for (int i = inner0 ? 1 : 0; i < 4; ++i) {
+  for (int i = inner0 ? 1 : 0; i < (p5_deferred ? 3 : 4); ++i) {
     char* dst = (char*)pyr[i] + (size_t)f0 * hs[i] * wsz[i] * 256 * es;
     MCG_TRY(conv_call(e, s, dt, e->fpn_out[i], t.l[i], n, hs[i], wsz[i], dst, 0, nullptr, MCG_RES_NONE, 0, 0));
     audit_tensor(au, dst, (long long)n * hs[i] * wsz[i] * 256, "fpn.P%d", i + 2);
@@ -586,6 +590,10 @@
   bool lateral;
   char *c2, *l1;
   int *istate, *icount, *ilist;
+  bool p5;
+  char* l3;
+  int* p5want;
+  int nclear;
   size_t total;
 };
 static bool fpn_deferred_on(const mcg_engine* e, int N, int H, int W) {
@@ -600,6 +608,16 @@
   return e->fpn_lateral_deferred && fpn_deferred_on(e, N, H, W) && e->pw_single && e->ctx.tile < 0 && cw.wf && cw.bias && cw.k == 1 && cw.stride == 1 &&
          cw.pad == 0 && h % 2 == 0 && w % 2 == 0 &&
          pw_single_x3_blocks_applicable(cw.cin, cw.cout, h, w, (long long)N * h * w, (long long)N * (h / 2) * (w / 2));
+}
+static bool fpn_p5_deferred_on(const mcg_engine* e, int N, int H, int W) {
+  return e->fpn_p5_deferred && fpn_deferred_on(e, N, H, W) && e->num_stages <= 30 &&
+         wino_kind(e, e->dt, e->fpn_out[3], N, H / 32, W / 32, MCG_RES_NONE) == 2;
+}
+extern "C" int mcg_deferred_p5_region_bytes(int N, int H, int W, int num_stages, size_t* inner_bytes, size_t* counter_bytes) {
+  MCG_CHECK_ARG(check_shape_ok(N, H, W) && num_stages > 0, "mcg_deferred_p5_region_bytes: bad shape");
+  if (inner_bytes) *inner_bytes = al256((size_t)N * (H / 32) * (W / 32) * 256 * 4);
+  if (counter_bytes) *counter_bytes = al256(sizeof(int) * ((size_t)num_stages + 1));
+  return MCG_OK;
 }
 static DeferSlot defer_layout(const mcg_engine* e, int N, int H, int W, char* base) {
   DeferSlot d;
@@ -613,8 +631,18 @@
     d.nblk = N * wino_x3_blocks_per_frame(H / 4, W / 4);
     d.lateral = fpn_lateral_deferred_on(e, N, H, W);
     const size_t per = (size_t)d.nblk + e->num_stages;
+    const size_t state_off = off;
     d.state = (int*)take(sizeof(int) * per * (d.lateral ? 2 : 1));
     d.count = d.state ? d.state + d.nblk : nullptr;
+    d.nclear = (int)(per * (d.lateral ? 2 : 1));
+    d.p5 = fpn_p5_deferred_on(e, N, H, W);
+    if (d.p5) {
+      size_t inner_bytes = 0, counter_bytes = 0;
+      (void)mcg_deferred_p5_region_bytes(N, H, W, e->num_stages, &inner_bytes, &counter_bytes);
+      d.nclear = (int)((off - state_off) / sizeof(int)) + e->num_stages + 1;
+      d.p5want = (int*)take(counter_bytes);
+      d.l3 = take(inner_bytes);
+    }
     d.list = (int*)take(sizeof(int) * (size_t)d.nblk * e->num_stages);
     if (d.lateral) {
       d.istate = d.state ? d.state + per : nullptr;
@@ -661,7 +689,8 @@
 }
 
 static int trunk_forward(mcg_engine* e, mcg_stream s_, const float* img, int N, int H, int W, int chunk,
-                         void* const pyramid[4], void* ws, size_t ws_bytes, bool backbone_only, const TrunkKeep tk = TrunkKeep{nullptr, nullptr, nullptr}) {
+                         void* const pyramid[4], void* ws, size_t ws_bytes, bool backbone_only,
+                         const TrunkKeep tk = TrunkKeep{nullptr, nullptr, nullptr, nullptr}) {
   MCG_CHECK_ARG(e && img && (pyramid || backbone_only) && ws, "mcg_backbone_fpn_forward: null pointer");
   MCG_TRY(check_shape(N, H, W));
   std::lock_guard<std::mutex> lock(e->mu);
@@ -793,7 +822,7 @@
 static int defer_stage_forward(const mcg_engine* e, hipStream_t s, const DeferSlot& d, int st, const float* boxes, int N, int h, int w) {
   const mcg_conv_weights& cw = e->fpn_out[0];
   int* list = d.list + (size_t)st * d.nblk;
-  MCG_TRY(launch_roi_mark(s, boxes, N * 3, 3, 0, h, w, 4, d.state, list, d.count + st));
+  MCG_TRY(launch_roi_mark(s, boxes, N * 3, 3, 0, h, w, 4, d.state, list, d.count + st, d.p5 ? d.p5want + st : nullptr));
   if (d.lateral) {
     const mcg_conv_weights& lw = e->lateral[0];
     int* ilist = d.ilist + (size_t)st * d.nblk;
@@ -810,7 +839,16 @@
     MCG_TRY(launch_done(lrec, s, launch_pw_single_x3_blocks(s, pp, ilist, d.icount + st, d.nblk), "pw_single_x3 block"));
   }
   ProfRec* rec = prof_begin_wino(e->ctx, s, cw, (long long)N * h * w, st == 0);
-  return launch_done(rec, s, launch_wino_x3_blocks(s, wino_params(cw, 2, d.inner, N, h, w, d.p[0], 0), list, d.count + st, d.nblk), "wino_x3 block");
+  MCG_TRY(launch_done(rec, s, launch_wino_x3_blocks(s, wino_params(cw, 2, d.inner, N, h, w, d.p[0], 0), list, d.count + st, d.nblk), "wino_x3 block"));
+  if (d.p5) {
+    const mcg_conv_weights& c5 = e->fpn_out[3];
+    const int h5 = h >> 3, w5 = w >> 3;
+    WinoParams wp = wino_params(c5, 2, d.l3, N, h5, w5, d.p[3], 0);
+    wp.gate = d.p5want; wp.gate_stage = st; wp.gate_stages = e->num_stages;
+    ProfRec* rec5 = prof_begin_wino(e->ctx, s, c5, (long long)N * h5 * w5, st == 0);
+    MCG_TRY(launch_done(rec5, s, launch_wino_x3(s, wp, e->wino_tile, 2), "wino_x3 gated"));
+  }
+  return MCG_OK;
 }
 
 static int decoder_forward(mcg_engine* e, hipStream_t s, const void* const pyramid[4], int pyramid_frames, const int32_t* frame_of, int N,
@@ -828,7 +866,7 @@
   char* obj_in = c.obj_a; char* obj_out = c.obj_b;
   float* b_in = c.boxes_a; float* b_out = c.boxes_b;
   const bool defer = d && d->deferred;
-  if (defer) MCG_TRY(launch_defer_clear(s, d->state, (d->nblk + e->num_stages) * (d->lateral ? 2 : 1)));
+  if (defer) MCG_TRY(launch_defer_clear(s, d->state, d->nclear));
   for (int st = 0; st < e->num_stages; ++st) {
     if (defer) MCG_TRY(defer_stage_forward(e, s, *d, st, b_in, N, fh[0], fw[0]));
     MCG_TRY(launch_roi_align(s, e->dt, pyramid, fh, fw, strides, 256, b_in, N * 3, 3, frame_of, pyramid_frames, c.roi, nullptr));
@@ -884,7 +922,7 @@
   const DeferSlot d = defer_layout(e, N, H, W, (char*)slot);
   if (slot_bytes < d.total) { mcg_set_error("mcg_backbone_fpn_forward_deferred: slot too small (%zu < %zu)", slot_bytes, d.total); return MCG_ERR_WORKSPACE; }
   return trunk_forward(e, s, img, N, H, W, chunk, d.p, ws, ws_bytes, false,
-                       TrunkKeep{d.deferred ? d.inner : nullptr, d.lateral ? d.c2 : nullptr, d.lateral ? d.l1 : nullptr});
+                       TrunkKeep{d.deferred ? d.inner : nullptr, d.lateral ? d.c2 : nullptr, d.lateral ? d.l1 : nullptr, d.p5 ? d.l3 : nullptr});
 }
 
 extern "C" int mcg_deferred_pyramid_state(const mcg_engine* e, void* slot, int N, int H, int W, void** inner, int** flags, int** counts, int** lists,
@@ -898,6 +936,18 @@
   if (lists) *lists = d.ilist;
   if (blocks) *blocks = d.nblk;
   if (lateral_deferred) *lateral_deferred = d.lateral ? 1 : 0;
+  return MCG_OK;
+}
+
+extern "C" int mcg_deferred_pyramid_p5_state(const mcg_engine* e, void* slot, int N, int H, int W, void** inner, int** counters, int* stages,
+                                             int* p5_deferred) {
+  MCG_CHECK_ARG(e && slot, "mcg_deferred_pyramid_p5_state: null pointer");
+  MCG_TRY(check_shape(N, H, W));
+  const DeferSlot d = defer_layout(e, N, H, W, (char*)slot);
+  if (inner) *inner = d.l3;
+  if (counters) *counters = d.p5want;
+  if (stages) *stages = e->num_stages;
+  if (p5_deferred) *p5_deferred = d.p5 ? 1 : 0;
   return MCG_OK;
 }
 
diff --git a/mcgaze_amd/csrc/roi_align.hip b/mcgaze_amd/csrc/roi_align.hip
--- a/mcgaze_amd/csrc/roi_align.hip
+++ b/mcgaze_amd/csrc/roi_align.hip
@@ -83,12 +83,14 @@
 constexpr int kMarkMaxBlocks = 64;
 __global__ __launch_bounds__(256) void roi_mark_kernel(const float* __restrict__ boxes, int boxes_per_frame, int level_deferred, int H, int W,
                                                        float ss, int* __restrict__ state, int* __restrict__ list, int* __restrict__ count,
-                                                       float finest_scale) {
+                                                       float finest_scale, int* __restrict__ coarse_want) {
   constexpr int P = 7, S = 2, NS = P * S;
   __shared__ int s_hit[2][kMarkMaxBlocks];
   const int box = blockIdx.x, tid = threadIdx.x;
   const float x1 = boxes[box * 4 + 0], y1 = boxes[box * 4 + 1], x2 = boxes[box * 4 + 2], y2 = boxes[box * 4 + 3];
-  if (roi_level(x1, y1, x2, y2, finest_scale) != level_deferred) return;
+  const int level = roi_level(x1, y1, x2, y2, finest_scale);
+  if (coarse_want && level == 3 && tid == 0) atomicAdd(coarse_want, 1);
+  if (level != level_deferred) return;
   const int by_n = (H + 7) / 8, bx_n = (W + 7) / 8;
   if (tid < 2 * kMarkMaxBlocks) s_hit[tid / kMarkMaxBlocks][tid % kMarkMaxBlocks] = 0;
   __syncthreads();
@@ -142,6 +144,7 @@
 __global__ void defer_clear_kernel(int* __restrict__ p, int n) {
   for (int i = blockIdx.x * blockDim.x + threadIdx.x; i < n; i += gridDim.x * blockDim.x) p[i] = 0;
 }
+extern "C" int mcg_roi_level(float x1, float y1, float x2, float y2) { return roi_level(x1, y1, x2, y2, 56.f); }
 bool roi_mark_supported(int H, int W) { return (H + 7) / 8 <= kMarkMaxBlocks && (W + 7) / 8 <= kMarkMaxBlocks; }
 int launch_defer_clear(hipStream_t s, int* p, int n) {
   const int blocks = (n + 255) / 256 < 1024 ? (n + 255) / 256 : 1024;
@@ -150,10 +153,10 @@
   return MCG_OK;
 }
 int launch_roi_mark(hipStream_t s, const float* boxes, int num_boxes, int boxes_per_frame, int level, int H, int W, int stride, int* state,
-                    int* list, int* count) {
+                    int* list, int* count, int* coarse_want) {
   MCG_CHECK_ARG(roi_mark_supported(H, W), "roi_mark: deferred level of %dx%d pixels exceeds %d blocks per axis", H, W, kMarkMaxBlocks);
   hipLaunchKernelGGL(roi_mark_kernel, dim3(num_boxes), dim3(256), 0, s, boxes, boxes_per_frame, level, H, W, 1.0f / (float)stride, state, list,
-                     count, 56.f);
+                     count, 56.f, coarse_want);
   MCG_CHECK_LAUNCH("roi_mark");
   return MCG_OK;
 }
diff --git a/mcgaze_amd/csrc/roi_sample.hpp b/mcgaze_amd/csrc/roi_sample.hpp
--- a/mcgaze_amd/csrc/roi_sample.hpp
+++ b/mcgaze_amd/csrc/roi_sample.hpp
@@ -1,6 +1,6 @@
 #pragma once
 
-__device__ __forceinline__ int roi_level(float x1, float y1, float x2, float y2, float finest_scale) {
+__host__ __device__ __forceinline__ int roi_level(float x1, float y1, float x2, float y2, float finest_scale) {
   const float sc = sqrtf((x2 - x1) * (y2 - y1));
   int level = (int)fminf(fmaxf(floorf(log2f(sc / finest_scale + 1e-6f)), 0.f), 3.f);
   if (!(sc == sc)) level = 0;
diff --git a/mcgaze_amd/csrc/wino_x3.hpp b/mcgaze_amd/csrc/wino_x3.hpp
--- a/mcgaze_amd/csrc/wino_x3.hpp
+++ b/mcgaze_amd/csrc/wino_x3.hpp
@@ -21,6 +21,8 @@
   const int* blk_list;
   const int* blk_count;
   int bxn, bpf;
+  int* gate;
+  int gate_stage, gate_stages;
 };
 
 namespace wnx {
@@ -115,10 +117,18 @@
     *(float4*)(yp + (long long)j * p.Cout) = o;
   }
 }
+__device__ __forceinline__ bool gate_open(const WinoParams& p) {
+  int earlier = 0;
+  for (int j = 0; j < p.gate_stage; ++j) earlier |= p.gate[j];
+  return __builtin_amdgcn_readfirstlane((earlier == 0 && p.gate[p.gate_stage] != 0) ? 1 : 0) != 0;
+}
+__device__ __forceinline__ void gate_done(const WinoParams& p) {
+  if (blockIdx.x == 0 && threadIdx.x == 0) p.gate[p.gate_stages] = p.gate[p.gate_stages] | (1 << p.gate_stage);
+}
 }
 
 template <int NB, int RH, int RT, int CT, int G>
-__global__ __launch_bounds__(64 * (G + 2) * RH, 1) void wino_x3_kernel(const WinoParams p) {
+__device__ __forceinline__ void wino_x3_tile(const WinoParams& p, const int logical) {
   using namespace wnx;
   constexpr int NV = G + 2, NW = NV * RH, NTHREADS = 64 * NW, MT = 32 * RH * RT, NT = 32 * CT;
   constexpr int ROWB = NB * 1024, WIN_CAP = wcap(G, CT), USTAGE = ustage(G);
@@ -133,7 +143,6 @@
   const int tid = threadIdx.x, lane = tid & 63;
   const int wave = __builtin_amdgcn_readfirstlane(tid >> 6);
   const int nu = wave % NV, rh = wave / NV;
-  const int logical = xcd_remap(blockIdx.x, gridDim.x);
   const int mt = logical / p.n_tiles, ntile = logical - mt * p.n_tiles;
   int q0, q_end;
   tile_range(p, mt, MT, q0, q_end);
@@ -341,6 +350,16 @@
     }
     __syncthreads();
   }
+}
+template <int NB, int RH, int RT, int CT, int G>
+__global__ __launch_bounds__(64 * (G + 2) * RH, 1) void wino_x3_kernel(const WinoParams p) {
+  wino_x3_tile<NB, RH, RT, CT, G>(p, xcd_remap(blockIdx.x, gridDim.x));
+}
+template <int NB, int RH, int RT, int CT, int G>
+__global__ __launch_bounds__(64 * (G + 2) * RH, 1) void wino_x3_gated_kernel(const WinoParams p) {
+  if (!wnx::gate_open(p)) return;
+  wino_x3_tile<NB, RH, RT, CT, G>(p, xcd_remap(blockIdx.x, gridDim.x));
+  wnx::gate_done(p);
 }
 
 typedef uint32_t u32x4v __attribute__((ext_vector_type(4)));
@@ -598,6 +617,12 @@
 __global__ __launch_bounds__(256, 1) void wino_x3w_kernel(const WinoParams p) {
   wino_x3w_tile<NB, false>(p, xcd_remap(blockIdx.x, gridDim.x));
 }
+template <int NB>
+__global__ __launch_bounds__(256, 1) void wino_x3w_gated_kernel(const WinoParams p) {
+  if (!wnx::gate_open(p)) return;
+  wino_x3w_tile<NB, false>(p, xcd_remap(blockIdx.x, gridDim.x));
+  wnx::gate_done(p);
+}
 __global__ __launch_bounds__(256, 1) void wino_x3w_blocks_kernel(const WinoParams p) {
   const int units = __builtin_amdgcn_readfirstlane(((*p.blk_count + 3) >> 2) * p.n_tiles);
   const int padded = p.n_tiles == 2 ? (units + 15) & ~15 : units;
@@ -641,12 +666,26 @@
 template <int NB, int RH, int RT, int CT, int G>
 static inline int launch_wino_x3_t(hipStream_t s, const WinoParams& p, int grid) {
   constexpr int kLds = 2 * wnx::wcap(G, CT) + 2 * ((G + 2) * CT * 2 * 1024);
+  if (p.gate) {
+    if constexpr (G == 2) {
+      if (kernel_ready<wino_x3_gated_kernel<NB, RH, RT, CT, G>>(kLds)) return 1;
+      hipLaunchKernelGGL((wino_x3_gated_kernel<NB, RH, RT, CT, G>), dim3(grid), dim3(64 * (G + 2) * RH), kLds, s, p);
+      return hipGetLastError() == hipSuccess ? 0 : 1;
+    } else {
+      return 1;
+    }
+  }
   if (kernel_ready<wino_x3_kernel<NB, RH, RT, CT, G>>(kLds)) return 1;
   hipLaunchKernelGGL((wino_x3_kernel<NB, RH, RT, CT, G>), dim3(grid), dim3(64 * (G + 2) * RH), kLds, s, p);
   return hipGetLastError() == hipSuccess ? 0 : 1;
 }
 template <int NB>
 static inline int launch_wino_x3w(hipStream_t s, const WinoParams& p, int grid) {
+  if (p.gate) {
+    if (kernel_ready<wino_x3w_gated_kernel<NB>>(wnx::W_LDS)) return 1;
+    hipLaunchKernelGGL((wino_x3w_gated_kernel<NB>), dim3(grid), dim3(256), wnx::W_LDS, s, p);
+    return hipGetLastError() == hipSuccess ? 0 : 1;
+  }
   if (kernel_ready<wino_x3w_kernel<NB>>(wnx::W_LDS)) return 1;
   hipLaunchKernelGGL((wino_x3w_kernel<NB>), dim3(grid), dim3(256), wnx::W_LDS, s, p);
   return hipGetLastError() == hipSuccess ? 0 : 1;
diff --git a/mcgaze_amd/lib.py b/mcgaze_amd/lib.py
--- a/mcgaze_amd/lib.py
+++ b/mcgaze_amd/lib.py
@@ -34,7 +34,7 @@
            'mcg_deferred_pyramid_state', 'mcg_inner_block_neighbours', 'mcg_gaze_targets', 'mcg_gaze_dwell', 'mcg_gaze_targets_poly',
            'mcg_pointwise_stream', 'mcg_pointwise_dyn', 'mcg_pointwise_pair', 'mcg_draw_attention', 'mcg_draw_attention_nv12',
            'mcg_format_labels', 'mcg_draw_labels', 'mcg_draw_labels_nv12', 'mcg_gaze_heat_add', 'mcg_draw_heat', 'mcg_draw_heat_nv12',
-           'mcg_anonymize_heads', 'mcg_anonymize_heads_nv12']
+           'mcg_anonymize_heads', 'mcg_anonymize_heads_nv12', 'mcg_deferred_pyramid_p5_state', 'mcg_deferred_p5_region_bytes', 'mcg_roi_level']
 LABEL_CHARS = 24
 LETTERBOX_U8, LETTERBOX_F16, LETTERBOX_F32 = 0, 1, 2
 
@@ -162,6 +162,9 @@
     lib.mcg_deferred_pyramid_bytes.argtypes = [vp, i, i, i]
     lib.mcg_deferred_pyramid_levels.argtypes = [vp, vp, i, i, i, C.POINTER(vp), C.POINTER(i)]
     lib.mcg_deferred_pyramid_state.argtypes = [vp, vp, i, i, i, C.POINTER(vp), C.POINTER(vp), C.POINTER(vp), C.POINTER(vp), C.POINTER(i), C.POINTER(i)]
+    lib.mcg_deferred_pyramid_p5_state.argtypes = [vp, vp, i, i, i, C.POINTER(vp), C.POINTER(vp), C.POINTER(i), C.POINTER(i)]
+    lib.mcg_deferred_p5_region_bytes.argtypes = [i, i, i, i, C.POINTER(sz), C.POINTER(sz)]
+    lib.mcg_roi_level.argtypes = [C.c_float] * 4
     lib.mcg_inner_block_neighbours.argtypes = [i, i, i, C.POINTER(i)]
     lib.mcg_backbone_fpn_forward_deferred.argtypes = [vp, vp, vp, i, i, i, i, vp, sz, vp, sz]
     lib.mcg_decoder_forward_deferred.argtypes = [vp, vp, vp, sz, i, i, i, i, vp, vp, vp, vp, vp, sz]
```

Result: no change. 3653 clips/s (median of 2 runs) (+0.4%).
